# ColinWine/Multi-modal-Multi-label-Facial-Action-Unit-Detection-with-Transformer

Measured on AMD Instinct MI355X. Metric: clips/sec (fwd+bwd) on synthetic (B,T,d) AV sequences, higher is better.
Workload: dtype bf16; 1 GPU; BASELINE.json configs[1]: avformer transformer stack d=512 L=6 H=8x64 mlp=1024, T_v=196+T_a=128 tokens, B=32/GPU; global_batch=32, seq_len=324, parallelism=dp1, step=zero_grad+fwd+AULoss+bwd+adam, optimizer=FusedAdam, residual_stream=bf16

## Files before the change

include/avformer_hip.h:

```cpp
#ifndef AVFORMER_HIP_H
#define AVFORMER_HIP_H

#include <stddef.h>
#include <stdint.h>

#ifdef __cplusplus
extern "C" {
#endif

#define AVF_F32 0
#define AVF_BF16 1

#define AVF_EPI_NONE 0
#define AVF_EPI_BIAS_RES 1
#define AVF_EPI_BIAS_GELU 2
#define AVF_EPI_DGELU 3

typedef struct avf_layer_cfg {
  int32_t batch;
  int32_t tokens;
  int32_t dim;
  int32_t heads;
  int32_t dim_head;
  int32_t mlp_dim;
// ... 240 lines not shown

size_t avf_layer_saved_bytes(const avf_layer_cfg* cfg);
size_t avf_layer_lowp_bytes(const avf_layer_cfg* cfg);
size_t avf_layer_workspace_bytes(const avf_layer_cfg* cfg);
size_t avf_layer_grad_stream_bytes(const avf_layer_cfg* cfg);
int avf_layer_prepare_weights(const avf_layer_cfg* cfg, const avf_layer_params* p, void* lowp, void* stream);

int avf_layer_adam_step(const avf_layer_cfg* cfg, const avf_layer_params* p, const avf_layer_grads* g,
                        const avf_layer_grads* exp_avg, const avf_layer_grads* exp_avg_sq, void* lowp, float lr,
                        float beta1, float beta2, float eps, float weight_decay, const float* step, void* stream);

int avf_stack_adam_step(const avf_layer_cfg* cfg, int layers, const avf_layer_params* p, const avf_layer_grads* g,
                        const avf_layer_grads* exp_avg, const avf_layer_grads* exp_avg_sq, void* const* lowp, float lr,
                        float beta1, float beta2, float eps, float weight_decay, const float* step, void* stream);

int avf_adam_step_tensors(int count, float* const* p, const float* const* g, float* const* exp_avg,
                          float* const* exp_avg_sq, const int64_t* numel, float lr, float beta1, float beta2, float eps,
                          float weight_decay, const float* step, void* stream);

int avf_adam_batch_begin(void);
int avf_adam_batch_end(void);
int avf_adam_batch_abort(void);
int avf_selftest_adam_table(void* stream);

size_t avf_grad_control_workspace_bytes(int count, const int64_t* numel);
int avf_grad_control(int count, const float* const* g, const int64_t* numel, float max_norm, int n_warmup_steps,
                     const float* step, float* ctl, void* ws, void* stream);

int avf_adam_batch_control(const float* ctl);

int avf_layer_fwd(const avf_layer_cfg* cfg, const avf_layer_params* p, const void* lowp, const void* x_in,
                  void* x_out, void* saved, void* workspace, void* stream);

int avf_layer_fwd_embed_ok(const avf_layer_cfg* cfg);
int avf_layernorm_fwd_embed(const float* clip, const float* audio, const float* pos, int batch, int t_video, int t_audio,
                            void* x0_bf16, const float* gamma, const float* beta, void* y_bf16, float* mean, float* rstd, int dim,
                            float eps, void* stream);
int avf_layernorm_bwd_pos_ok(int batch, int tokens, int dim);
size_t avf_layernorm_bwd_pos_workspace_bytes(int batch, int tokens, int dim);
int avf_layernorm_bwd_pos(const void* dy_bf16, const void* x_bf16, const float* gamma, const float* mean, const float* rstd,
                          const void* dres_bf16, float* d_pos, float* dgamma, float* dbeta, void* workspace, int batch, int tokens,
                          int dim, void* stream);
int avf_layer_fwd_embed(const avf_layer_cfg* cfg, const avf_layer_params* p, const void* lowp, const float* clip,
                        const float* audio, const float* pos, int t_video, void* x0, void* x_out, void* saved, void* workspace,
                        void* stream);
int avf_layer_bwd_pos_ok(const avf_layer_cfg* cfg);
int avf_layer_bwd_pos(const avf_layer_cfg* cfg, const avf_layer_params* p, const void* lowp, const void* x_in,
                      const void* saved, const float* dx_out, const void* dx_out_lo, const float* dx_out_colsum, float* d_pos,
                      const avf_layer_grads* g, void* workspace, void* stream);
int avf_layer_bwd_dx_pos(const avf_layer_cfg* cfg, const avf_layer_params* p, const void* lowp, const void* x_in,
                         const void* saved, const float* dx_out, const void* dx_out_lo, const float* dx_out_colsum, float* d_pos,
                         const avf_layer_grads* g, void* workspace, void* dw_block, void* dw_desc, void* stream);

int avf_layer_bwd(const avf_layer_cfg* cfg, const avf_layer_params* p, const void* lowp, const void* x_in,
                  const void* saved, const float* dx_out, const void* dx_out_lo, const float* dx_out_colsum,
                  float* dx_in, void* dx_in_lo, float* dx_in_colsum, const avf_layer_grads* g, void* workspace,
                  void* stream);

int avf_layer_dw_defer_ok(const avf_layer_cfg* cfg, int* tiles_per_layer, int* slots);
int avf_layers_dw_max(void);
size_t avf_layer_dw_block_bytes(const avf_layer_cfg* cfg);
size_t avf_layer_dw_desc_bytes(void);
int avf_layer_bwd_dx(const avf_layer_cfg* cfg, const avf_layer_params* p, const void* lowp, const void* x_in,
                     const void* saved, const float* dx_out, const void* dx_out_lo, const float* dx_out_colsum,
                     float* dx_in, void* dx_in_lo, float* dx_in_colsum, const avf_layer_grads* g, void* workspace,
                     void* dw_block, void* dw_desc, void* stream);
size_t avf_layers_dw_workspace_bytes(const avf_layer_cfg* cfgs, int n_layers);
int avf_layers_dw(const avf_layer_cfg* cfgs, int n_layers, const void* const* descs, void* workspace, size_t workspace_bytes,
                  void* stream);

int avf_conv_pack_weight(const float* w, const float* gamma, const float* beta, const float* running_mean,
                         const float* running_var, double eps, void* w_packed, float* scale, float* shift, int Cout, int Cin,
                         int k, void* stream);
int avf_conv2d_nhwc(const void* x, int x_dtype, const void* w_packed, const float* scale, const float* shift,
                    const void* residual, int res_dtype, int relu, int k, int stride, void* out, int out_dtype, int N, int H,
                    int W, int Cin, int Cout, void* stream);
int avf_conv_plan(int N, int H, int W, int Cin, int Cout, int k, int stride, int* tile, int* tile_m, int* tile_n);
int avf_avgpool_nhwc(const void* x, int x_dtype, float* out, int64_t N, int HW, int C, void* stream);

int avf_dropout_factors(uint32_t seed_lo, uint32_t seed_hi, int layer_index, int site, float p, int64_t rows, int cols,
                        float* out, void* stream);

int avf_set_f32_arith(int mode);
int avf_get_f32_arith(void);

int avf_hip_error_reset(void* stream);

int avf_crash_line_arm(const char* line, int fd);
int avf_crash_line_disarm(void);

int avf_timing_enable(int on);
int avf_timing_read(int cls, double* total_ms, int64_t* launches, double* flops, double* bytes);

int avf_selftest_mfma_bf16(const void* a_bf16_16x32, const void* b_bf16_32x16, float* c_16x16, void* stream);
int avf_selftest_mfma_f32(const float* a_16x4, const float* b_4x16, float* c_16x16, void* stream);
int avf_selftest_tr16(const void* tile_bf16_32x16, void* out_bf16_64x8, void* stream);

#ifdef __cplusplus
}
#endif
#endif
```

multi-modal-multi-label-facial-action-unit-detection-with-transformer_amd/_build.py:

```python
from __future__ import annotations

import concurrent.futures
import os
import shutil
import subprocess

HERE = os.path.dirname(os.path.abspath(__file__))
CSRC = os.path.join(HERE, "csrc")
LIBDIR = os.path.join(HERE, "lib")
LIBNAME = "libavformer_hip.so"
SOURCES = ["api.hip", "norm_elem.hip", "layernorm.hip", "gemm_f32.hip", "attn_f32.hip", "attn_f32_mfma.hip", "attn_f32x3.hip", "gemm_bf16.hip", "gemm_ws.hip", "gemm_mx8.hip", "attn_bf16.hip", "attn_bwd_merged.hip", "layer.hip", "optim.hip", "grad_control.hip", "layer_small.hip", "heads.hip", "task_loss.hip", "eval_metrics.hip", "mel.hip", "clip.hip", "augment.hip", "clip_bank.hip", "mel_bank.hip", "conv.hip"]
HEADERS = [os.path.join(CSRC, "common.hpp"), os.path.join(CSRC, "gemm_nt.hpp"), os.path.join(CSRC, "gemm_dispatch.hpp"), os.path.join(CSRC, "attn_dispatch.hpp"), os.path.join(CSRC, "clip_source.hpp"),
           os.path.join(CSRC, "clip_kernels.hpp"), os.path.join(CSRC, "augment_kernels.hpp"), os.path.join(CSRC, "mel_kernels.hpp"), os.path.join(os.path.dirname(HERE), "include", "avformer_hip.h")]
FLAGS = ["--offload-arch=gfx950", "-O3", "-std=c++17", "-fPIC"]
EXTRA_FLAGS = {"gemm_f32.hip": ["-mllvm", "-amdgpu-mfma-vgpr-form"], "attn_f32_mfma.hip": ["-mllvm", "-amdgpu-mfma-vgpr-form"], "attn_f32x3.hip": ["-mllvm", "-amdgpu-mfma-vgpr-form"],
               "attn_bwd_merged.hip": ["-mllvm", "-amdgpu-mfma-vgpr-form", "-Xclang", "-target-feature", "-Xclang", "-packed-fp32-ops"],
               "augment.hip": ["-ffp-contract=off"],
               "clip_bank.hip": ["-ffp-contract=off"]}


def out_wt() -> int:
    v = os.environ.get("AVF_OUT_WT", "1").strip() or "1"
    if v not in ("0", "1"):
        raise RuntimeError(f"AVF_OUT_WT={v!r}: 0 or 1")
    return int(v)


def _variant() -> str:
    return "" if out_wt() == 1 else "_wt0"


def built_lib_path() -> str:
    return os.path.join(LIBDIR, LIBNAME.replace(".so", _variant() + ".so"))


def lib_path() -> str:
    return os.environ.get("AVF_LIB_PATH") or built_lib_path()


def _hipcc() -> str:
    for cand in (os.environ.get("HIPCC"), "/opt/rocm/bin/hipcc", shutil.which("hipcc")):
        if cand and os.path.exists(cand):
            return cand
    raise RuntimeError("hipcc not found (set HIPCC or install ROCm under /opt/rocm)")


def _stale(target: str, deps) -> bool:
    if not os.path.exists(target):
        return True
    t = os.path.getmtime(target)
    return any(os.path.getmtime(d) > t for d in deps)


def build(force: bool = False, verbose: bool = False) -> str:
    import fcntl
    os.makedirs(LIBDIR, exist_ok=True)
    with open(os.path.join(LIBDIR, ".build.lock"), "w") as lock:
        fcntl.flock(lock, fcntl.LOCK_EX)
        try:
            return _build_locked(force, verbose)
        finally:
            fcntl.flock(lock, fcntl.LOCK_UN)


# ... 40 lines not shown
```

multi-modal-multi-label-facial-action-unit-detection-with-transformer_amd/_lib.py:

```python
from __future__ import annotations

import ctypes as C
import os
import threading

from . import _build

F32, BF16 = 0, 1
EPI_NONE, EPI_BIAS_RES, EPI_BIAS_GELU, EPI_DGELU = 0, 1, 2, 3
CLIP_CTHW, CLIP_TCHW = 0, 1
WAVE_F32, WAVE_I16 = 0, 1

_vp = C.c_void_p
_i64 = C.c_int64
_int = C.c_int
_f = C.c_float
_sz = C.c_size_t


class LayerCfg(C.Structure):
    _fields_ = [("batch", C.c_int32), ("tokens", C.c_int32), ("dim", C.c_int32), ("heads", C.c_int32),
                ("dim_head", C.c_int32), ("mlp_dim", C.c_int32), ("dtype", C.c_int32), ("project_out", C.c_int32),
                ("ln_eps", C.c_float), ("dropout_p", C.c_float), ("seed_lo", C.c_uint32), ("seed_hi", C.c_uint32),
                ("layer_index", C.c_int32), ("seed_dev", C.c_void_p), ("grad_stream_bf16", C.c_int32), ("mx8_fwd", C.c_int32),
# ... 88 lines not shown
    "avf_au_loss_sum": (_int, [_vp, _i64, _vp, _i64, _vp, _f, _int, _int, _vp, _vp, _vp]),
    "avf_au_loss_wide": (_int, [_vp, _i64, _vp, _i64, _vp, _f, _int, _int, _int, _int, _vp, _vp, _vp]),
    "avf_sizeof_task_loss_cfg": (_sz, []),
    "avf_task_loss": (_int, [_vp, _i64, _vp, _vp, _i64, _vp, _i64, _vp, _int, _int, _vp, _vp, _vp, _vp]),
    "avf_task_loss_bwd": (_int, [_vp, _vp, _vp, _vp, _vp, _int, _int, _vp, _vp]),
    "avf_sizeof_eval_cfg": (_sz, []),
    "avf_eval_update": (_int, [_vp, _i64, _vp, _vp, _i64, _vp, _i64, _vp, _vp, _int, _vp, _vp, _vp, _vp, _vp]),
    "avf_eval_scores": (_int, [_vp, _vp, _vp, _vp]),
    "avf_mel_power": (_int, [_vp, _i64, _i64, _vp, _int, _int, _int, _vp, _vp, _vp, _int, _int, _int, _vp, _vp, _vp]),
    "avf_mel_db_norm": (_int, [_vp, _vp, _i64, _int, _i64, _int, C.c_double, C.c_double, C.c_double, _vp]),
    "avf_mel_power_bank": (_int, [_vp, _int, _i64, _vp, _vp, _i64, _vp, _vp, _i64, _vp, _i64, _i64, _i64, _vp, _int, _int, _int, _vp, _vp,
                                  _vp, _int, _int, _vp, _vp, _vp]),
    "avf_wave_gather": (_int, [_vp, _int, _i64, _vp, _vp, _i64, _vp, _vp, _i64, _vp, _i64, _i64, _i64, _i64, _vp, _vp]),
    "avf_clip_normalize": (_int, [_vp, _i64, _i64, _i64, _i64, _int, _int, _vp, _vp, _vp, _int, _int, _vp]),
    "avf_clip_denormalize": (_int, [_vp, _int, _int, _i64, _i64, _i64, _i64, _int, _vp, _vp, _vp, _vp]),
    "avf_clip_autoaugment": (_int, [_vp, _vp, _i64, _i64, _i64, _i64, _int, _vp, _vp]),
    "avf_clip_autoaugment_max_pixels": (_i64, []),
    "avf_clip_autoaugment_normalize": (_int, [_vp, _i64, _i64, _i64, _i64, _int, _vp, _int, _vp, _vp, _vp, _int, _int, _vp]),
    "avf_clip_gather": (_int, [_vp, _vp, _vp, _vp, _i64, _i64, _i64, _i64, _i64, _i64, _int, _vp, _vp]),
    "avf_clip_gather_normalize": (_int, [_vp, _vp, _vp, _vp, _i64, _i64, _i64, _i64, _i64, _i64, _int, _int, _vp, _vp, _vp, _int, _int,
                                         _vp]),
    "avf_clip_gather_autoaugment": (_int, [_vp, _vp, _vp, _vp, _i64, _i64, _i64, _i64, _i64, _i64, _int, _vp, _vp, _vp]),
    "avf_clip_gather_autoaugment_normalize": (_int, [_vp, _vp, _vp, _vp, _i64, _i64, _i64, _i64, _i64, _i64, _int, _vp, _int, _vp, _vp,
                                                     _vp, _int, _int, _vp]),
    "avf_conv_pack_weight": (_int, [_vp, _vp, _vp, _vp, _vp, C.c_double, _vp, _vp, _vp, _int, _int, _int, _vp]),
    "avf_conv2d_nhwc": (_int, [_vp, _int, _vp, _vp, _vp, _vp, _int, _int, _int, _int, _vp, _int, _int, _int, _int, _int, _int, _vp]),
    "avf_conv_plan": (_int, [_int, _int, _int, _int, _int, _int, _int, C.POINTER(C.c_int), C.POINTER(C.c_int), C.POINTER(C.c_int)]),
    "avf_avgpool_nhwc": (_int, [_vp, _int, _vp, _i64, _int, _int, _vp]),
    "avf_layer_saved_bytes": (_sz, [C.POINTER(LayerCfg)]),
    "avf_layer_lowp_bytes": (_sz, [C.POINTER(LayerCfg)]),
    "avf_layernorm_bwd_mx8": (_int, [_vp, _vp, _vp, _vp, _vp, _vp, _vp, _vp, _vp, _vp, _vp, _vp, _vp, _i64, _int, _vp]),
    "avf_attn_fwd_mx8": (_int, [_vp, _vp, _vp, _vp, _vp, _int, _int, _int, _int, _vp]),
    "avf_attn_bwd_emits_mx8": (_int, [_int, _int]),
    "avf_attn_bwd_mx8": (_int, [_vp, _vp, _vp, _vp, _vp, _vp, _vp, _int, _int, _int, _int, _vp]),
    "avf_attn_fwd_masked": (_int, [_int, _vp, _vp, _vp, _vp, _int, _int, _int, _int, _vp]),
    "avf_attn_bwd_masked": (_int, [_int, _vp, _vp, _vp, _vp, _vp, _vp, _vp, _int, _int, _int, _int, _vp]),
    "avf_layer_workspace_bytes": (_sz, [C.POINTER(LayerCfg)]),
    "avf_layer_grad_stream_bytes": (_sz, [C.POINTER(LayerCfg)]),
    "avf_layer_prepare_weights": (_int, [C.POINTER(LayerCfg), C.POINTER(LayerPtrs), _vp, _vp]),
    "avf_layer_fwd": (_int, [C.POINTER(LayerCfg), C.POINTER(LayerPtrs), _vp, _vp, _vp, _vp, _vp, _vp]),
    "avf_layer_bwd": (_int, [C.POINTER(LayerCfg), C.POINTER(LayerPtrs), _vp, _vp, _vp, _vp, _vp, _vp, _vp, _vp, _vp,
                             C.POINTER(LayerPtrs), _vp, _vp]),
    "avf_layernorm_fwd_embed": (_int, [_vp, _vp, _vp, _int, _int, _int, _vp, _vp, _vp, _vp, _vp, _vp, _int, _f, _vp]),
    "avf_layernorm_bwd_pos_ok": (_int, [_int, _int, _int]),
    "avf_layernorm_bwd_pos_workspace_bytes": (_sz, [_int, _int, _int]),
    "avf_layernorm_bwd_pos": (_int, [_vp, _vp, _vp, _vp, _vp, _vp, _vp, _vp, _vp, _vp, _int, _int, _int, _vp]),
    "avf_layer_fwd_embed_ok": (_int, [C.POINTER(LayerCfg)]),
    "avf_layer_fwd_embed": (_int, [C.POINTER(LayerCfg), C.POINTER(LayerPtrs), _vp, _vp, _vp, _vp, _int, _vp, _vp, _vp, _vp, _vp]),
    "avf_layer_bwd_pos_ok": (_int, [C.POINTER(LayerCfg)]),
    "avf_layer_bwd_pos": (_int, [C.POINTER(LayerCfg), C.POINTER(LayerPtrs), _vp, _vp, _vp, _vp, _vp, _vp, _vp,
                                 C.POINTER(LayerPtrs), _vp, _vp]),
    "avf_layer_bwd_dx_pos": (_int, [C.POINTER(LayerCfg), C.POINTER(LayerPtrs), _vp, _vp, _vp, _vp, _vp, _vp, _vp,
                                    C.POINTER(LayerPtrs), _vp, _vp, _vp, _vp]),
    "avf_layer_dw_defer_ok": (_int, [C.POINTER(LayerCfg), C.POINTER(C.c_int), C.POINTER(C.c_int)]),
    "avf_layers_dw_max": (_int, []),
    "avf_layer_dw_block_bytes": (_sz, [C.POINTER(LayerCfg)]),
    "avf_layer_dw_desc_bytes": (_sz, []),
    "avf_layer_bwd_dx": (_int, [C.POINTER(LayerCfg), C.POINTER(LayerPtrs), _vp, _vp, _vp, _vp, _vp, _vp, _vp, _vp, _vp,
                                C.POINTER(LayerPtrs), _vp, _vp, _vp, _vp]),
    "avf_layers_dw_workspace_bytes": (_sz, [C.POINTER(LayerCfg), _int]),
    "avf_layers_dw": (_int, [C.POINTER(LayerCfg), _int, _vp, _vp, _sz, _vp]),
    "avf_layer_adam_step": (_int, [C.POINTER(LayerCfg), C.POINTER(LayerPtrs), C.POINTER(LayerPtrs), C.POINTER(LayerPtrs),
                                   C.POINTER(LayerPtrs), _vp, _f, _f, _f, _f, _f, _vp, _vp]),
    "avf_stack_adam_step": (_int, [C.POINTER(LayerCfg), _int, C.POINTER(LayerPtrs), C.POINTER(LayerPtrs), C.POINTER(LayerPtrs),
                                   C.POINTER(LayerPtrs), _vp, _f, _f, _f, _f, _f, _vp, _vp]),
    "avf_adam_step_tensors": (_int, [_int, _vp, _vp, _vp, _vp, _vp, _f, _f, _f, _f, _f, _vp, _vp]),
    "avf_adam_batch_begin": (_int, []),
    "avf_adam_batch_end": (_int, []),
    "avf_adam_batch_abort": (_int, []),
    "avf_selftest_adam_table": (_int, [_vp]),
    "avf_grad_control_workspace_bytes": (_sz, [_int, _vp]),
    "avf_grad_control": (_int, [_int, _vp, _vp, _f, _int, _vp, _vp, _vp, _vp]),
    "avf_adam_batch_control": (_int, [_vp]),
    "avf_dropout_factors": (_int, [C.c_uint32, C.c_uint32, _int, _int, _f, _i64, _int, _vp, _vp]),
    "avf_timing_enable": (_int, [_int]),
    "avf_timing_read": (_int, [_int, C.POINTER(C.c_double), C.POINTER(C.c_int64), C.POINTER(C.c_double),
                               C.POINTER(C.c_double)]),
    "avf_hip_error_reset": (_int, [_vp]),
    "avf_crash_line_arm": (_int, [C.c_char_p, _int]),
    "avf_crash_line_disarm": (_int, []),
    "avf_set_f32_arith": (_int, [_int]),
    "avf_get_f32_arith": (_int, []),
    "avf_selftest_mfma_bf16": (_int, [_vp, _vp, _vp, _vp]),
    "avf_selftest_mfma_f32": (_int, [_vp, _vp, _vp, _vp]),
    "avf_selftest_tr16": (_int, [_vp, _vp, _vp]),
}

_lock = threading.Lock()
_lib = None


class HipLibraryError(RuntimeError):
    pass


def load(build_if_missing: bool = True):
    global _lib
    if _lib is not None:
        return _lib
    with _lock:
        if _lib is not None:
            return _lib
        path = _build.lib_path()
        if not os.path.exists(path):
            err = None
            if build_if_missing:
# ... 68 lines not shown
```

multi-modal-multi-label-facial-action-unit-detection-with-transformer_amd/csrc/api.hip:

```cpp
#include <stdarg.h>

#include "common.hpp"

namespace avf {

static thread_local char g_err[512] = "";

void set_error(const char* fmt, ...) {
  va_list ap;
  va_start(ap, fmt);
  vsnprintf(g_err, sizeof(g_err), fmt, ap);
  va_end(ap);
}

int check_launch(const char* what) {
  hipError_t e = hipGetLastError();
  if (e != hipSuccess) {
    set_error("%s: %s", what, hipGetErrorString(e));
    return 2;
  }
  return 0;
}

namespace {
// ... 141 lines not shown
  return 1;
}

extern "C" int avf_layernorm_fwd(const float* x, const float* gamma, const float* beta, void* y, int y_dtype,
                                 float* mean, float* rstd, int64_t rows, int dim, float eps, void* stream) {
  AVF_REQUIRE(x && gamma && beta && y && mean && rstd, "layernorm_fwd: null pointer");
  return layernorm_fwd(x, gamma, beta, y, y_dtype, mean, rstd, rows, dim, eps, (hipStream_t)stream);
}
extern "C" size_t avf_layernorm_bwd_workspace_bytes(int64_t rows, int dim) { return layernorm_bwd_ws(rows, dim); }
extern "C" int avf_layernorm_bwd(const void* dy, int dy_dtype, const float* x, const float* gamma, const float* mean,
                                 const float* rstd, const float* dres, float* dx, void* dx_lo, float* dgamma,
                                 float* dbeta, float* dcolsum, void* workspace, int64_t rows, int dim, void* stream) {
  AVF_REQUIRE(dy && x && gamma && mean && rstd && dx && dgamma && dbeta && workspace, "layernorm_bwd: null pointer");
  return layernorm_bwd(dy, dy_dtype, x, gamma, mean, rstd, dres, dx, dx_lo, dgamma, dbeta, dcolsum, workspace, rows,
                       dim, (hipStream_t)stream);
}
extern "C" int avf_layernorm_fwd_ex(const void* x, int x_dtype, const float* gamma, const float* beta, void* y, int y_dtype,
                                    float* mean, float* rstd, int64_t rows, int dim, float eps, void* stream) {
  AVF_REQUIRE(x && gamma && beta && y && mean && rstd, "layernorm_fwd_ex: null pointer");
  AVF_REQUIRE(x_dtype == AVF_F32 || x_dtype == AVF_BF16, "layernorm_fwd_ex: bad x_dtype %d", x_dtype);
  return layernorm_fwd(x, gamma, beta, y, y_dtype, mean, rstd, rows, dim, eps, (hipStream_t)stream, nullptr, nullptr, x_dtype);
}
extern "C" int avf_layernorm_bwd_ex(const void* dy, int dy_dtype, const void* x, int x_dtype, const float* gamma,
                                    const float* mean, const float* rstd, const void* dres, int dres_dtype, float* dx,
                                    void* dx_lo, void* dx_m, float* dgamma, float* dbeta, float* dcolsum, void* workspace,
                                    int64_t rows, int dim, uint32_t seed_lo, uint32_t seed_hi, int layer_index, int site,
                                    float p, void* stream) {
  AVF_REQUIRE(dy && x && gamma && mean && rstd && dgamma && dbeta && workspace, "layernorm_bwd_ex: null pointer");
  AVF_REQUIRE((x_dtype == AVF_F32 || x_dtype == AVF_BF16) && (dres_dtype == AVF_F32 || dres_dtype == AVF_BF16),
              "layernorm_bwd_ex: bad x_dtype %d / dres_dtype %d", x_dtype, dres_dtype);
  AVF_REQUIRE(p >= 0.f && p < 1.f && (p == 0.f || (site >= 0 && site < 3)), "layernorm_bwd_ex: bad dropout site %d / p %g", site,
              (double)p);
  const DropCfg d = p > 0.f ? make_drop(p, ((uint64_t)seed_hi << 32) | seed_lo, layer_index, site) : kNoDrop;
  return layernorm_bwd(dy, dy_dtype, x, gamma, mean, rstd, dres, dx, dx_lo, dgamma, dbeta, dcolsum, workspace, rows, dim,
                       (hipStream_t)stream, d, nullptr, dres ? dres_dtype : AVF_F32, x_dtype, nullptr, nullptr, dx_m);
}
extern "C" int avf_layernorm_fwd_embed(const float* clip, const float* audio, const float* pos, int batch, int t_video, int t_audio,
                                       void* x0_bf16, const float* gamma, const float* beta, void* y_bf16, float* mean, float* rstd,
                                       int dim, float eps, void* stream) {
  AVF_REQUIRE(gamma && beta, "layernorm_fwd_embed: null pointer");
  return layernorm_fwd_embed(clip, audio, pos, batch, t_video, t_audio, x0_bf16, gamma, beta, y_bf16, mean, rstd, dim, eps,
                             (hipStream_t)stream);
}
extern "C" int avf_layernorm_bwd_pos_ok(int batch, int tokens, int dim) { return layernorm_bwd_tok_ok(batch, tokens, dim) ? 1 : 0; }
extern "C" size_t avf_layernorm_bwd_pos_workspace_bytes(int batch, int tokens, int dim) {
  return layernorm_bwd_ws((int64_t)batch * tokens, dim, tokens);
}
extern "C" int avf_layernorm_bwd_pos(const void* dy_bf16, const void* x_bf16, const float* gamma, const float* mean, const float* rstd,
                                     const void* dres_bf16, float* d_pos, float* dgamma, float* dbeta, void* workspace, int batch,
                                     int tokens, int dim, void* stream) {
  AVF_REQUIRE(dgamma && dbeta, "layernorm_bwd_pos: null pointer");
  return layernorm_bwd_tok(dy_bf16, x_bf16, gamma, mean, rstd, dres_bf16, d_pos, dgamma, dbeta, workspace, batch, tokens, dim,
                           (hipStream_t)stream);
}
extern "C" size_t avf_colsum_workspace_bytes(int64_t rows, int cols) { return colsum_ws(rows, cols); }
extern "C" int avf_colsum(const void* in, int in_dtype, int64_t rows, int cols, int64_t ld, float* out,
                          void* workspace, void* stream) {
  return colsum(in, in_dtype, rows, cols, ld, out, workspace, (hipStream_t)stream);
}
extern "C" int avf_cast_f32_to_bf16(const float* in, void* out, int64_t n, void* stream) {
  AVF_REQUIRE(in && out, "cast: null pointer");
  return cast_f32_to_bf16(in, out, n, (hipStream_t)stream);
}
extern "C" int avf_dropout_factors(uint32_t seed_lo, uint32_t seed_hi, int layer_index, int site, float p, int64_t rows,
                                   int cols, float* out, void* stream) {
  AVF_REQUIRE(out && rows > 0 && cols > 0 && cols % 4 == 0 && p > 0.f && p < 1.f && site >= 0 && site < 3,
              "dropout_factors: bad arguments");
  const DropCfg d = make_drop(p, ((uint64_t)seed_hi << 32) | seed_lo, layer_index, site);
  return dropout_factors(d, out, rows * cols, (hipStream_t)stream);
}
extern "C" int avf_prep_weight_bf16(const float* w, void* w_lo, void* w_t_lo, int rows, int cols, void* stream) {
  AVF_REQUIRE(w, "prep_weight: null pointer");
  return prep_weight_bf16(w, w_lo, w_t_lo, rows, cols, (hipStream_t)stream);
}

extern "C" size_t avf_gemm_workspace_bytes(int dtype, int transA, int transB, int64_t M, int64_t N, int64_t K) {
  return gemm_ws(dtype, transA, transB, M, N, K);
}
extern "C" int avf_gemm(int dtype, int transA, int transB, int64_t M, int64_t N, int64_t K, const void* A, int64_t lda,
                        const void* B, int64_t ldb, void* C, int64_t ldc, int c_dtype, int epilogue, const float* bias,
                        const float* residual, int64_t ldres, void* aux, int64_t ldaux, void* workspace, void* stream) {
  AVF_REQUIRE(A && B && C, "gemm: null pointer");
  GemmArgs a;
  a.dtype = dtype; a.transA = transA; a.transB = transB;
  a.M = M; a.N = N; a.K = K;
  a.A = A; a.lda = lda; a.B = B; a.ldb = ldb; a.C = C; a.ldc = ldc;
  a.c_dtype = c_dtype; a.epilogue = epilogue; a.bias = bias; a.residual = residual; a.ldres = ldres;
  a.aux = aux; a.ldaux = ldaux; a.workspace = workspace; a.colsum = nullptr; a.drop = kNoDrop; a.defer_fold = nullptr;
  return gemm(a, (hipStream_t)stream);
}

extern "C" int avf_pack_weight_ws_ok(int64_t rows, int64_t cols) { return pack_ws_ok(rows, cols) ? 1 : 0; }
extern "C" size_t avf_pack_weight_ws_bytes(int64_t rows, int64_t cols) { return pack_ws_ok(rows, cols) ? pack_ws_bytes(rows, cols) : 0; }
extern "C" size_t avf_gemm_nt_ws_workspace_bytes(int64_t M, int64_t N) { return gemm_nt_colsum_ws(M, N); }
extern "C" int avf_gemm_nt_ws_dispatch(int64_t M, int64_t N, int64_t K, int epilogue, int c_dtype) {
  GemmArgs a;
  a.dtype = AVF_BF16; a.transA = 0; a.transB = 1;
  a.M = M; a.N = N; a.K = K;
  void* aligned = (void*)(uintptr_t)256;
  a.A = aligned; a.lda = K; a.B = nullptr; a.ldb = K; a.C = aligned; a.ldc = N;
  a.c_dtype = c_dtype; a.epilogue = epilogue; a.bias = (epilogue == AVF_EPI_BIAS_RES || epilogue == AVF_EPI_BIAS_GELU) ? (const float*)aligned : nullptr;
  a.residual = epilogue == AVF_EPI_BIAS_RES ? aligned : nullptr; a.ldres = N;
  a.aux = (epilogue == AVF_EPI_BIAS_GELU || epilogue == AVF_EPI_DGELU) ? aligned : nullptr; a.ldaux = N;
  a.workspace = nullptr; a.colsum = nullptr; a.drop = kNoDrop; a.defer_fold = nullptr;
  a.Bp = aligned; a.ws_force = 0; a.mx_q = nullptr; a.mx_s = nullptr;
  return gemm_bf16_nt_ws_preferred(a) ? 1 : 0;
// ... 280 lines not shown
```

multi-modal-multi-label-facial-action-unit-detection-with-transformer_amd/csrc/common.hpp:

```cpp
#pragma once
#include <hip/hip_runtime.h>
#include <hip/hip_ext.h>
#include <stdint.h>
#include <stdio.h>
#include <stdlib.h>
#include <string.h>

#include <type_traits>

#include "../../include/avformer_hip.h"

namespace avf {

void set_error(const char* fmt, ...);
int check_launch(const char* what);
bool shape_log_on();
void shape_log(const char* fmt, ...);
inline const char* tuning_env(const char* name) {
  static const bool on = [] {
    const char* t = getenv("AVF_TUNING");
    return t && *t && atoi(t) != 0;
  }();
  return on ? getenv(name) : nullptr;
}
// ... 267 lines not shown
  d.scale = 1.0f / (1.0f - (float)d.thresh16 / 65536.0f);
  d.site_const = 0xD1B54A32D192ED03ULL * (uint64_t)(layer * 4 + site + 1);
  d.key = mix64(seed + d.site_const);
  d.seed_dev = seed_dev;
  return d;
}
static const DropCfg kNoDrop = {0, nullptr, 0, 0, 1.0f};
__device__ __forceinline__ uint64_t drop_key(const DropCfg& d) {
  return d.seed_dev ? mix64(*d.seed_dev + d.site_const) : d.key;
}
__device__ __forceinline__ float4 drop_factor4(const DropCfg& d, uint64_t key, uint64_t idx) {
  const uint64_t h = mix64(key + idx * 0x9E3779B97F4A7C15ULL);
  float4 f;
  f.x = ((uint32_t)(h) & 0xffffu) >= d.thresh16 ? d.scale : 0.f;
  f.y = ((uint32_t)(h >> 16) & 0xffffu) >= d.thresh16 ? d.scale : 0.f;
  f.z = ((uint32_t)(h >> 32) & 0xffffu) >= d.thresh16 ? d.scale : 0.f;
  f.w = ((uint32_t)(h >> 48) & 0xffffu) >= d.thresh16 ? d.scale : 0.f;
  return f;
}

__device__ __forceinline__ float drop_factor1(const DropCfg& d, uint64_t key, uint64_t idx) {
  const uint64_t h = mix64(key + (idx & ~3ULL) * 0x9E3779B97F4A7C15ULL);
  return ((uint32_t)(h >> (16 * (idx & 3))) & 0xffffu) >= d.thresh16 ? d.scale : 0.f;
}

static inline size_t align_up(size_t v, size_t a) { return (v + a - 1) / a * a; }

struct PerDeviceOnce {
  uint64_t done = 0;
  bool need() const {
    int dev = 0;
    (void)hipGetDevice(&dev);
    return ((__atomic_load_n(&done, __ATOMIC_ACQUIRE) >> (dev & 63)) & 1u) == 0;
  }
  void mark() {
    int dev = 0;
    (void)hipGetDevice(&dev);
    __atomic_fetch_or(&done, 1ull << (dev & 63), __ATOMIC_RELEASE);
  }
};

struct FoldJob;
int layernorm_fwd(const void* x, const float* gamma, const float* beta, void* y, int y_dtype, float* mean,
                  float* rstd, int64_t rows, int dim, float eps, hipStream_t s, void* mx_q = nullptr, void* mx_s = nullptr,
                  int x_dtype = AVF_F32);
size_t layernorm_bwd_ws(int64_t rows, int dim, int tokens = 0);
bool layernorm_fwd_embed_ok(int dim);
int layernorm_fwd_embed(const float* clip, const float* audio, const float* pos, int batch, int t_video, int t_audio, void* x0,
                        const float* gamma, const float* beta, void* y, float* mean, float* rstd, int dim, float eps, hipStream_t s);
bool layernorm_bwd_tok_ok(int batch, int tokens, int dim);
int layernorm_bwd_tok(const void* dy, const void* x, const float* gamma, const float* mean, const float* rstd, const void* dres,
                      float* dpos, float* dgamma, float* dbeta, void* ws, int batch, int tokens, int dim, hipStream_t s,
                      FoldJob* defer_fold = nullptr);
int layernorm_bwd(const void* dy, int dy_dtype, const void* x, const float* gamma, const float* mean,
                  const float* rstd, const void* dres, float* dx, void* dx_lo, float* dgamma, float* dbeta,
                  float* dcolsum, void* ws, int64_t rows, int dim, hipStream_t s, const DropCfg& drop = kNoDrop,
                  FoldJob* defer_fold = nullptr, int dres_dtype = AVF_F32, int x_dtype = AVF_F32, void* mx_q = nullptr,
                  void* mx_s = nullptr, void* dx_m = nullptr);
size_t colsum_ws(int64_t rows, int cols);
int colsum(const void* in, int in_dtype, int64_t rows, int cols, int64_t ld, float* out, void* ws, hipStream_t s);
int cast_f32_to_bf16(const float* in, void* out, int64_t n, hipStream_t s, const DropCfg& drop = kNoDrop);
int mask_copy_f32(const float* in, float* out, int64_t n, hipStream_t s, const DropCfg& drop);
int dropout_factors(const DropCfg& drop, float* out, int64_t n, hipStream_t s);
int fold_partials(const float* partial, int nb, int width, float* out, hipStream_t s);
struct FoldJob;
int fold_job(const FoldJob& job, hipStream_t s);

struct FoldJob {
  const float* partial;
  int nb, width, seg;
  float *o0, *o1, *o2;
};
constexpr int kFoldMax = 12;
struct FoldList {
  FoldJob job[kFoldMax];
  int count;
};
int fold_list(const FoldList& fl, hipStream_t s);
constexpr int FOLD_COLS = 16, FOLD_RG = 64;
__device__ __forceinline__ void fold_columns_vec(const FoldJob& j, int colgroup, float4 (*red)[FOLD_COLS / 4]) {
  const int cq = threadIdx.x & (FOLD_COLS / 4 - 1), grp = threadIdx.x / (FOLD_COLS / 4);
  const int col = colgroup * FOLD_COLS + cq * 4;
  float4 a[8];
#pragma unroll
  for (int u = 0; u < 8; ++u) a[u] = make_float4(0.f, 0.f, 0.f, 0.f);
  if (col < j.width) {
    int b = grp;
    for (; b + 7 * FOLD_RG < j.nb; b += 8 * FOLD_RG) {
      float4 t[8];
#pragma unroll
      for (int u = 0; u < 8; ++u) t[u] = *reinterpret_cast<const float4*>(j.partial + (int64_t)(b + FOLD_RG * u) * j.width + col);
#pragma unroll
      for (int u = 0; u < 8; ++u) { a[u].x += t[u].x; a[u].y += t[u].y; a[u].z += t[u].z; a[u].w += t[u].w; }
    }
    for (; b < j.nb; b += FOLD_RG) {
      const float4 t = *reinterpret_cast<const float4*>(j.partial + (int64_t)b * j.width + col);
      a[0].x += t.x; a[0].y += t.y; a[0].z += t.z; a[0].w += t.w;
    }
  }
  red[grp][cq] = make_float4(((a[0].x + a[1].x) + (a[2].x + a[3].x)) + ((a[4].x + a[5].x) + (a[6].x + a[7].x)),
                             ((a[0].y + a[1].y) + (a[2].y + a[3].y)) + ((a[4].y + a[5].y) + (a[6].y + a[7].y)),
                             ((a[0].z + a[1].z) + (a[2].z + a[3].z)) + ((a[4].z + a[5].z) + (a[6].z + a[7].z)),
                             ((a[0].w + a[1].w) + (a[2].w + a[3].w)) + ((a[4].w + a[5].w) + (a[6].w + a[7].w)));
  __syncthreads();
  if (threadIdx.x < FOLD_COLS) {
    const int q = threadIdx.x >> 2, comp = threadIdx.x & 3;
// ... 158 lines not shown
```

multi-modal-multi-label-facial-action-unit-detection-with-transformer_amd/csrc/layer.hip:

```cpp
#include <mutex>
#include <vector>

#include "common.hpp"

namespace avf {

namespace {

struct Dims {
  int64_t R;
  int D, H, dh, I, M, B, N;
  int dt;
  size_t es;
  float p;
  uint64_t seed;
  const uint64_t* seed_dev;
  int layer;
  bool gs16;
  bool gsd;
  bool mx;
  bool rs16;
  int xdt;
  float p0;
  const void* keep;
// ... 101 lines not shown
  }
  Carver c(base);
  LowP t;
  t.wqkv = c.take((size_t)3 * d.I * d.D * 2);
  t.wqkv_t = c.take((size_t)3 * d.I * d.D * 2);
  t.wo = c.take((size_t)d.D * d.I * 2);
  t.wo_t = c.take((size_t)d.D * d.I * 2);
  t.w1 = c.take((size_t)d.M * d.D * 2);
  t.w1_t = c.take((size_t)d.M * d.D * 2);
  t.w2 = c.take((size_t)d.D * d.M * 2);
  t.w2_t = c.take((size_t)d.D * d.M * 2);
  if (d.mx) {
    t.wqkv_q = c.take((size_t)3 * d.I * d.D); t.wqkv_s = c.take((size_t)3 * d.I * d.D / 32);
    t.w1_q = c.take((size_t)d.M * d.D);       t.w1_s = c.take((size_t)d.M * d.D / 32);
    t.w2_q = c.take((size_t)d.D * d.M);       t.w2_s = c.take((size_t)d.D * d.M / 32);
    t.wo_q = c.take((size_t)d.D * d.I);       t.wo_s = c.take((size_t)d.D * d.I / 32);
    t.w2t_q = c.take((size_t)d.D * d.M);      t.w2t_s = c.take((size_t)d.D * d.M / 32);
    t.w1t_q = c.take((size_t)d.D * d.M);      t.w1t_s = c.take((size_t)d.D * d.M / 32);
    t.wot_q = c.take((size_t)d.D * d.I);      t.wot_s = c.take((size_t)d.D * d.I / 32);
    t.wqkvt_q = c.take((size_t)3 * d.I * d.D); t.wqkvt_s = c.take((size_t)3 * d.I * d.D / 32);
  } else {
    t.wqkv_q = t.wqkv_s = t.w1_q = t.w1_s = t.w2_q = t.w2_s = nullptr;
    t.wo_q = t.wo_s = t.w2t_q = t.w2t_s = t.w1t_q = t.w1t_s = t.wot_q = t.wot_s = nullptr;
    t.wqkvt_q = t.wqkvt_s = nullptr;
  }
  t.ws.wqkv_p = pack_ws_ok(3 * d.I, d.D) ? c.take(pack_ws_bytes(3 * d.I, d.D)) : nullptr;
  t.ws.wo_p = pack_ws_ok(d.D, d.I) ? c.take(pack_ws_bytes(d.D, d.I)) : nullptr;
  t.ws.w1_p = pack_ws_ok(d.M, d.D) ? c.take(pack_ws_bytes(d.M, d.D)) : nullptr;
  t.ws.w2t_p = pack_ws_ok(d.M, d.D) ? c.take(pack_ws_bytes(d.M, d.D)) : nullptr;
  t.ws.wot_p = pack_ws_ok(d.I, d.D) ? c.take(pack_ws_bytes(d.I, d.D)) : nullptr;
  if (!base) t.ws = LowpWs{nullptr, nullptr, nullptr, nullptr, nullptr};
  if (l) *l = t;
  return c.off;
}

TnGroupArgs dw_group(const Dims& d, const void* gy, const void* g_act, const void* du, const void* h2, const void* gm,
                     const void* o, const void* dqkv, const void* h1, const avf_layer_grads* g) {
  TnGroupArgs a;
  memset(&a, 0, sizeof(a));
  a.count = 4;
  a.K = d.R;
  a.A[0] = dqkv; a.B[0] = h1; a.C[0] = g ? g->w_qkv : nullptr; a.M[0] = 3 * d.I; a.N[0] = d.D;
  a.A[1] = gm;   a.B[1] = o;  a.C[1] = g ? g->w_out : nullptr; a.M[1] = d.D;     a.N[1] = d.I;
  a.A[2] = du;   a.B[2] = h2; a.C[2] = g ? g->w1 : nullptr;    a.M[2] = d.M;     a.N[2] = d.D;
  a.A[3] = gy;   a.B[3] = g_act; a.C[3] = g ? g->w2 : nullptr; a.M[3] = d.D;     a.N[3] = d.M;
  for (int i = 0; i < 4; ++i) { a.lda[i] = a.M[i]; a.ldb[i] = a.N[i]; }
  return a;
}

size_t work_colsum_bytes(const Dims& d) {
  const int maxc = d.M > d.D ? d.M : d.D;
  size_t csb = colsum_ws(d.R, maxc);
  if (d.dt == AVF_BF16 && gemm_nt_colsum_ws(d.R, d.M) > csb) csb = gemm_nt_colsum_ws(d.R, d.M);
  return csb;
}

struct Work {
  void *du, *dh, *d_o, *dqkv, *dx_mid_lo, *dx_out_lo, *ln_ws, *ln_ws1, *cs_ws, *gemm_ws;
  float *dx_mid, *delta;
  void *hq, *hs, *gq, *gs;
  void *oq, *os;
  void *duq, *dus, *mq, *ms, *gyq, *gys;
  void *dqq, *dqs;
  void *dx_out_s, *dx_mid_m;
  float *gy_m, *gm_m;
  float* small_part;
};
size_t carve_work(const Dims& d, void* base, Work* w) {
  Carver c(base);
  Work t;
  t.du = c.take(d.R * d.M * d.es);
  t.dh = c.take(d.R * d.D * d.es);
  t.d_o = c.take(d.R * d.I * d.es);
  t.dqkv = c.take(d.R * 3 * d.I * d.es);
  t.dx_mid = (float*)c.take(d.R * d.D * 4);
  t.dx_mid_lo = c.take(d.dt == AVF_BF16 ? d.R * d.D * 2 : 0);
  t.dx_out_lo = c.take(d.dt == AVF_BF16 ? d.R * d.D * 2 : 0);
  t.delta = (float*)c.take((size_t)d.B * d.H * d.N * 4 * 2);
  t.ln_ws = c.take(layernorm_bwd_ws(d.R, d.D));
  t.ln_ws1 = c.take(layernorm_bwd_ws(d.R, d.D, d.N));
  t.cs_ws = c.take(work_colsum_bytes(d));
  size_t g = 0;
  if (d.dt == AVF_BF16) {
    size_t a = gemm_bf16_tn_ws(3 * d.I, d.D, d.R), b = gemm_bf16_tn_ws(d.D, d.I, d.R);
    size_t e = gemm_bf16_tn_ws(d.M, d.D, d.R), f = gemm_bf16_tn_ws(d.D, d.M, d.R);
    g = a > b ? a : b;
    g = g > e ? g : e;
    g = g > f ? g : f;
    TnGroupArgs ga = dw_group(d, nullptr, nullptr, nullptr, nullptr, nullptr, nullptr, nullptr, nullptr, nullptr);
    const size_t gg = gemm_bf16_tn_group_ws(ga);
    g = g > gg ? g : gg;
  } else {
    const size_t a = gemm_f32_ws(3 * d.I, d.D, d.R), b = gemm_f32_ws(d.D, d.I, d.R);
    const size_t e = gemm_f32_ws(d.M, d.D, d.R), f = gemm_f32_ws(d.D, d.M, d.R);
    g = a > b ? a : b;
    g = g > e ? g : e;
    g = g > f ? g : f;
    TnGroupArgs ga = dw_group(d, nullptr, nullptr, nullptr, nullptr, nullptr, nullptr, nullptr, nullptr, nullptr);
    const size_t gg = gemm_f32x3_tn_group_ws(ga);
    g = g > gg ? g : gg;
  }
  t.gemm_ws = c.take(g);
  t.small_part = (float*)c.take(small_layer_ok(d.dt, d.N, d.D, d.H, d.dh, d.M) ? small_bwd_partial_floats(d.B, d.D, d.M) * 4 : 0);
  if (d.mx) {
    t.hq = c.take(d.R * d.D); t.hs = c.take(d.R * d.D / 32);
    t.gq = c.take(d.R * d.M); t.gs = c.take(d.R * d.M / 32);
    t.oq = c.take(d.R * d.I); t.os = c.take(d.R * d.I / 32);
  } else {
    t.hq = t.hs = t.gq = t.gs = t.oq = t.os = nullptr;
  }
  if (d.mxb) {
    t.duq = c.take(d.R * d.M); t.dus = c.take(d.R * d.M / 32);
    t.mq = c.take(d.R * d.D);  t.ms = c.take(d.R * d.D / 32);
    t.gyq = c.take(d.R * d.D); t.gys = c.take(d.R * d.D / 32);
    t.dqq = c.take(d.R * 3 * d.I); t.dqs = c.take(d.R * 3 * d.I / 32);
  } else {
    t.duq = t.dus = t.mq = t.ms = t.gyq = t.gys = nullptr;
    t.dqq = t.dqs = nullptr;
  }
  t.dx_out_s = c.take(d.gsd ? d.R * d.D * 2 : 0);
  t.dx_mid_m = c.take(d.gsd ? d.R * d.D * 2 : 0);
  const bool f32_drop = d.dt == AVF_F32 && d.p > 0.f;
  t.gy_m = (float*)c.take(f32_drop ? d.R * d.D * 4 : 0);
  t.gm_m = (float*)c.take(f32_drop ? d.R * d.D * 4 : 0);
  if (w) *w = t;
  return c.off;
}

size_t carve_dw_block(const Dims& d, void* base, Work* w) {
  Carver c(base);
  void* du = c.take(d.R * d.M * 2);
  void* dqkv = c.take(d.R * 3 * d.I * 2);
  void* dx_mid_lo = c.take(d.R * d.D * 2);
  void* dx_out_lo = c.take(d.R * d.D * 2);
  void* ln_ws = c.take(layernorm_bwd_ws(d.R, d.D));
  void* ln_ws1 = c.take(layernorm_bwd_ws(d.R, d.D, d.N));
  void* cs_ws = c.take(work_colsum_bytes(d));
  if (w) {
    w->du = du; w->dqkv = dqkv; w->dx_mid_lo = dx_mid_lo; w->dx_out_lo = dx_out_lo;
    w->ln_ws = ln_ws; w->ln_ws1 = ln_ws1; w->cs_ws = cs_ws;
  }
  return c.off;
}
constexpr uint32_t kDwDescMagic = 0x64574431u;
struct DwDeferred {
  uint32_t magic;
  TnGroupArgs grp;
  FoldJob folds[3];
};
bool dw_defer_mode_ok(const Dims& d) {
  return d.dt == AVF_BF16 && !d.gsd && d.p == 0.f && !d.mx && !d.mxb && !d.keep && !small_layer_ok(d.dt, d.N, d.D, d.H, d.dh, d.M);
}

int linear_fwd(const Dims& d, const void* A, int in, const void* W, int out, void* C, int c_dtype, int epi,
               const float* bias, const void* res, void* aux, hipStream_t s, const DropCfg& drop = kNoDrop,
               const void* Wp = nullptr) {
  GemmArgs a;
  a.dtype = d.dt; a.transA = 0; a.transB = 1;
  a.M = d.R; a.N = out; a.K = in;
  a.A = A; a.lda = in; a.B = W; a.ldb = in;
  a.C = C; a.ldc = out; a.c_dtype = c_dtype; a.epilogue = epi;
  a.bias = bias; a.residual = res; a.ldres = out; a.aux = aux; a.ldaux = out; a.workspace = nullptr; a.colsum = nullptr;
  a.drop = drop; a.defer_fold = nullptr;
  a.Bp = Wp;
  return gemm(a, s);
}

int linear_fwd_mx(const Dims& d, const void* Aq, const void* As, int in, const void* Wq, const void* Ws, int out, void* C,
                  int c_dtype, int epi, const float* bias, const void* res, void* aux, hipStream_t s, const DropCfg& drop,
                  void* mx_q = nullptr, void* mx_s = nullptr) {
  GemmArgs a;
  a.dtype = AVF_BF16; a.transA = 0; a.transB = 1;
  a.M = d.R; a.N = out; a.K = in;
  a.A = Aq; a.lda = in; a.B = Wq; a.ldb = in;
  a.C = C; a.ldc = out; a.c_dtype = c_dtype; a.epilogue = epi;
  a.bias = bias; a.residual = res; a.ldres = out; a.aux = aux; a.ldaux = out; a.workspace = nullptr; a.colsum = nullptr;
  a.drop = drop; a.defer_fold = nullptr;
// ... 98 lines not shown
  AVF_TRY(make_dims(cfg, &d));
  if (d.dt != AVF_BF16) return 0;
  AVF_REQUIRE(p && lowp, "prepare_weights: null pointer");
  hipStream_t s = (hipStream_t)stream;
  LowP l;
  carve_lowp(d, lowp, &l);
  PrepBatch b;
  b.d[0] = PrepDesc{p->w_qkv, (bf16*)l.wqkv, (bf16*)l.wqkv_t, 3 * d.I, d.D, attn_q_prescale(d.dh), d.I, l.ws.wqkv_p, nullptr};
  b.d[1] = PrepDesc{p->w_out, (bf16*)l.wo, (bf16*)l.wo_t, d.D, d.I, 1.0f, 0, l.ws.wo_p, l.ws.wot_p};
  b.d[2] = PrepDesc{p->w1, (bf16*)l.w1, (bf16*)l.w1_t, d.M, d.D, 1.0f, 0, l.ws.w1_p, nullptr};
  b.d[3] = PrepDesc{p->w2, (bf16*)l.w2, (bf16*)l.w2_t, d.D, d.M, 1.0f, 0, nullptr, l.ws.w2t_p};
  AVF_TRY(prep_weights_multi(b, 4, s));
  return 0;
}

extern "C" int avf_stack_quant_weights_mx8(const avf_layer_cfg* cfg, int layers, void* const* lowp, void* stream) {
  Dims d;
  AVF_TRY(make_dims(cfg, &d));
  AVF_REQUIRE(d.mx, "stack_quant_weights_mx8: cfg.mx8_fwd is not set");
  AVF_REQUIRE(layers > 0 && layers <= 64 && lowp, "stack_quant_weights_mx8: bad arguments");
  MxQuantJob jobs[64 * 8];
  int n = 0;
  for (int i = 0; i < layers; ++i) {
    AVF_REQUIRE(lowp[i], "stack_quant_weights_mx8: null image buffer (layer %d)", i);
    LowP l;
    carve_lowp(d, lowp[i], &l);
    jobs[n++] = MxQuantJob{l.wqkv, l.wqkv_q, l.wqkv_s, 3 * d.I, d.D};
    jobs[n++] = MxQuantJob{l.w1, l.w1_q, l.w1_s, d.M, d.D};
    jobs[n++] = MxQuantJob{l.w2, l.w2_q, l.w2_s, d.D, d.M};
    if (d.I % 128 == 0) jobs[n++] = MxQuantJob{l.wo, l.wo_q, l.wo_s, d.D, d.I};
    if (d.mxb) {
      jobs[n++] = MxQuantJob{l.w2_t, l.w2t_q, l.w2t_s, d.M, d.D};
      jobs[n++] = MxQuantJob{l.w1_t, l.w1t_q, l.w1t_s, d.D, d.M};
      jobs[n++] = MxQuantJob{l.wo_t, l.wot_q, l.wot_s, d.I, d.D};
      if ((3 * d.I) % 128 == 0) jobs[n++] = MxQuantJob{l.wqkv_t, l.wqkvt_q, l.wqkvt_s, d.D, 3 * d.I};
    }
  }
  return quant_mx8_multi(jobs, n, (hipStream_t)stream);
}

static bool stack_ends_mode_ok(const Dims& d) {
  return d.dt == AVF_BF16 && d.rs16 && d.gs16 && !d.gsd && d.p == 0.f && !d.mx && !d.mxb &&
         !d.keep && d.D % 8 == 0 && d.D <= 1536;
}
extern "C" int avf_layer_fwd_embed_ok(const avf_layer_cfg* cfg) {
  Dims d;
  return !make_dims(cfg, &d) && stack_ends_mode_ok(d) && layernorm_fwd_embed_ok(d.D);
}
extern "C" int avf_layer_bwd_pos_ok(const avf_layer_cfg* cfg) {
  Dims d;
  return !make_dims(cfg, &d) && stack_ends_mode_ok(d) && layernorm_bwd_tok_ok(d.B, d.N, d.D);
}

struct EmbedSrc {
  const float *clip, *audio, *pos;
  int t_video;
  void* x0;
};
static int layer_fwd_impl(const avf_layer_cfg* cfg, const avf_layer_params* p, const void* lowp, const void* x_in, void* x_out,
                          void* saved, void* workspace, void* stream, const EmbedSrc* emb) {
  Dims d;
  AVF_TRY(make_dims(cfg, &d));
  if (emb) {
    AVF_REQUIRE(stack_ends_mode_ok(d) && layernorm_fwd_embed_ok(d.D) && emb->x0 && emb->t_video > 0 && emb->t_video < d.N,
                "layer_fwd_embed: needs the all-bf16 streams without dropout, fp8 or mask, and both token groups (ask "
                "avf_layer_fwd_embed_ok first)");
    x_in = emb->x0;
  }
  AVF_REQUIRE(p && x_in && x_out && saved, "layer_fwd: null pointer");
  AVF_REQUIRE(d.dt == AVF_F32 || lowp, "layer_fwd(bf16): lowp weights missing");
  hipStream_t s = (hipStream_t)stream;
  Saved sv;
  carve_saved(d, saved, &sv);
  LowP l;
  carve_lowp(d, (void*)lowp, &l);
  const bool lo = d.dt == AVF_BF16;
  const void* wqkv = lo ? l.wqkv : (const void*)p->w_qkv;
  const void* wo = lo ? l.wo : (const void*)p->w_out;
  const void* w1 = lo ? l.w1 : (const void*)p->w1;
  const void* w2 = lo ? l.w2 : (const void*)p->w2;

  if (d.mx) {
    AVF_REQUIRE(workspace, "layer_fwd(mx8): workspace missing");
    Work w;
    carve_work(d, workspace, &w);
    const DropCfg dr0 = make_drop(d.p0, d.seed, d.layer, 0, d.seed_dev), dr1 = make_drop(d.p, d.seed, d.layer, 1, d.seed_dev),
                  dr2 = make_drop(d.p, d.seed, d.layer, 2, d.seed_dev);
    AVF_TRY(layernorm_fwd(x_in, p->ln1_w, p->ln1_b, sv.h1, d.dt, sv.mean1, sv.rstd1, d.R, d.D, cfg->ln_eps, s, w.hq, w.hs, d.xdt));
    AVF_TRY(linear_fwd_mx(d, w.hq, w.hs, d.D, l.wqkv_q, l.wqkv_s, 3 * d.I, sv.qkv, d.dt, AVF_EPI_NONE, nullptr, nullptr,
                          nullptr, s, kNoDrop));
    static const int o_mx_on = tuning_int("AVF_MX8_OUTPROJ", 1);
    const bool o_mx = o_mx_on && !d.keep && attn_fwd_emits_mx8(d.N, d.dh) && d.I % 128 == 0;
    if (d.keep)
      AVF_TRY(attn_fwd_vec(AVF_BF16, sv.qkv, sv.o, sv.lse2, d.B, d.N, d.H, d.dh, s, d.keep, attn_q_prescale_on()));
    else
      AVF_TRY(attn_fwd_bf16((const bf16*)sv.qkv, (bf16*)sv.o, sv.lse2, d.B, d.N, d.H, d.dh, s, attn_q_prescale_on(),
                            o_mx ? w.oq : nullptr, o_mx ? w.os : nullptr));
    if (o_mx)
      AVF_TRY(linear_fwd_mx(d, w.oq, w.os, d.I, l.wo_q, l.wo_s, d.D, sv.x_mid, d.xdt, AVF_EPI_BIAS_RES, p->b_out, x_in, nullptr,
                            s, dr0));
    else
      AVF_TRY(linear_fwd(d, sv.o, d.I, wo, d.D, sv.x_mid, d.xdt, AVF_EPI_BIAS_RES, p->b_out, x_in, nullptr, s, dr0, l.ws.wo_p));
    AVF_TRY(layernorm_fwd(sv.x_mid, p->ln2_w, p->ln2_b, sv.h2, d.dt, sv.mean2, sv.rstd2, d.R, d.D, cfg->ln_eps, s, w.hq, w.hs, d.xdt));
    AVF_TRY(linear_fwd_mx(d, w.hq, w.hs, d.D, l.w1_q, l.w1_s, d.M, sv.g, d.dt, AVF_EPI_BIAS_GELU, p->b1, nullptr, sv.u, s, dr1,
                          w.gq, w.gs));
    AVF_TRY(linear_fwd_mx(d, w.gq, w.gs, d.M, l.w2_q, l.w2_s, d.D, x_out, d.xdt, AVF_EPI_BIAS_RES, p->b2, sv.x_mid, nullptr,
                          s, dr2));
    return 0;
  }
  if (!d.rs16 && !d.keep && small_layer_ok(d.dt, d.N, d.D, d.H, d.dh, d.M)) {
    const float sc = attn_q_prescale_on() ? 1.0f : 1.4426950408889634f / sqrtf((float)d.dh);
    return layer_fwd_small(d.B, d.N, d.D, d.H, d.M, cfg->ln_eps, sc, p, wqkv, wo, w1, w2, (const float*)x_in, (float*)x_out, sv.h1,
                           sv.mean1, sv.rstd1, sv.qkv, sv.o, sv.lse2, (float*)sv.x_mid, sv.h2, sv.mean2, sv.rstd2, sv.u, sv.g,
                           make_drop(d.p0, d.seed, d.layer, 0, d.seed_dev), make_drop(d.p, d.seed, d.layer, 1, d.seed_dev),
                           make_drop(d.p, d.seed, d.layer, 2, d.seed_dev), s);
  }
  if (emb)
    AVF_TRY(layernorm_fwd_embed(emb->clip, emb->audio, emb->pos, d.B, emb->t_video, d.N - emb->t_video, emb->x0, p->ln1_w, p->ln1_b,
                                sv.h1, sv.mean1, sv.rstd1, d.D, cfg->ln_eps, s));
  else
    AVF_TRY(layernorm_fwd(x_in, p->ln1_w, p->ln1_b, sv.h1, d.dt, sv.mean1, sv.rstd1, d.R, d.D, cfg->ln_eps, s, nullptr, nullptr, d.xdt));
  AVF_TRY(linear_fwd(d, sv.h1, d.D, wqkv, 3 * d.I, sv.qkv, d.dt, AVF_EPI_NONE, nullptr, nullptr, nullptr, s, kNoDrop, l.ws.wqkv_p));
  if (d.keep && lo) AVF_TRY(attn_fwd_masked_bf16(sv.qkv, sv.o, sv.lse2, d.keep, d.B, d.N, d.H, d.dh, s, attn_q_prescale_on()));
  else if (d.keep) AVF_TRY(attn_fwd_vec(d.dt, sv.qkv, sv.o, sv.lse2, d.B, d.N, d.H, d.dh, s, d.keep, false));
  else if (lo) AVF_TRY(attn_fwd_bf16((const bf16*)sv.qkv, (bf16*)sv.o, sv.lse2, d.B, d.N, d.H, d.dh, s, attn_q_prescale_on()));
  else AVF_TRY(attn_fwd_f32((const float*)sv.qkv, (float*)sv.o, sv.lse2, d.B, d.N, d.H, d.dh, s));
  const DropCfg dr0 = make_drop(d.p0, d.seed, d.layer, 0, d.seed_dev), dr1 = make_drop(d.p, d.seed, d.layer, 1, d.seed_dev),
                dr2 = make_drop(d.p, d.seed, d.layer, 2, d.seed_dev);
  AVF_TRY(linear_fwd(d, sv.o, d.I, wo, d.D, sv.x_mid, d.xdt, AVF_EPI_BIAS_RES, p->b_out, x_in, nullptr, s, dr0, l.ws.wo_p));
  AVF_TRY(layernorm_fwd(sv.x_mid, p->ln2_w, p->ln2_b, sv.h2, d.dt, sv.mean2, sv.rstd2, d.R, d.D, cfg->ln_eps, s, nullptr, nullptr, d.xdt));
  AVF_TRY(linear_fwd(d, sv.h2, d.D, w1, d.M, sv.g, d.dt, AVF_EPI_BIAS_GELU, p->b1, nullptr, sv.u, s, dr1, l.ws.w1_p));
  AVF_TRY(linear_fwd(d, sv.g, d.M, w2, d.D, x_out, d.xdt, AVF_EPI_BIAS_RES, p->b2, sv.x_mid, nullptr, s, dr2));
  return 0;
}

extern "C" int avf_layer_fwd(const avf_layer_cfg* cfg, const avf_layer_params* p, const void* lowp, const void* x_in,
                             void* x_out, void* saved, void* workspace, void* stream) {
  return layer_fwd_impl(cfg, p, lowp, x_in, x_out, saved, workspace, stream, nullptr);
}

extern "C" int avf_layer_fwd_embed(const avf_layer_cfg* cfg, const avf_layer_params* p, const void* lowp, const float* clip,
                                   const float* audio, const float* pos, int t_video, void* x0, void* x_out, void* saved,
                                   void* workspace, void* stream) {
  const EmbedSrc emb{clip, audio, pos, t_video, x0};
  return layer_fwd_impl(cfg, p, lowp, nullptr, x_out, saved, workspace, stream, &emb);
}

static int layer_bwd_impl(const avf_layer_cfg* cfg, const avf_layer_params* p, const void* lowp, const void* x_in,
                          const void* saved, const float* dx_out, const void* dx_out_lo,
                          const float* dx_out_colsum, float* dx_in, void* dx_in_lo, float* dx_in_colsum,
                          const avf_layer_grads* g, void* workspace, void* stream, void* dw_block, DwDeferred* dw_desc,
                          float* d_pos = nullptr) {
  Dims d;
  AVF_TRY(make_dims(cfg, &d));
  AVF_REQUIRE(!d_pos || (stack_ends_mode_ok(d) && layernorm_bwd_tok_ok(d.B, d.N, d.D) && !dx_in && !dx_in_lo && !dx_in_colsum),
              "layer_bwd_pos: needs the all-bf16 streams without dropout, fp8 or mask, a batch within the token-major rule (ask "
              "avf_layer_bwd_pos_ok first) and no dx_in outputs");
  AVF_REQUIRE(!dw_desc || (dw_block && dw_defer_mode_ok(d) && ((uintptr_t)dw_block & 255) == 0),
              "layer_bwd_dx: this mode keeps its weight gradients in the layer (ask avf_layer_dw_defer_ok first), or the "
              "operand block is missing / not 256-byte aligned");
  AVF_REQUIRE(p && x_in && saved && g && workspace, "layer_bwd: null pointer");
  AVF_REQUIRE(d.gs16 ? (dx_out || dx_out_lo) && (dx_in || dx_in_lo || d_pos) : (dx_out && dx_in), "layer_bwd: null gradient pointer");
  AVF_REQUIRE(!d.gs16 || dx_in_lo || d_pos, "layer_bwd(grad_stream_bf16): dx_in_lo missing");
  AVF_REQUIRE(d.dt == AVF_F32 || lowp, "layer_bwd(bf16): lowp weights missing");
  hipStream_t s = (hipStream_t)stream;
  Saved sv;
  carve_saved(d, (void*)saved, &sv);
  LowP l;
  carve_lowp(d, (void*)lowp, &l);
  const bool lo = d.dt == AVF_BF16;
  Work w;
  carve_work(d, workspace, &w);
  if (dw_desc) carve_dw_block(d, dw_block, &w);

  const DropCfg dr0 = make_drop(d.p0, d.seed, d.layer, 0, d.seed_dev), dr1 = make_drop(d.p, d.seed, d.layer, 1, d.seed_dev),
                dr2 = make_drop(d.p, d.seed, d.layer, 2, d.seed_dev);
  const DropCfg dr_prev2 = d.layer > 0 ? make_drop(d.p, d.seed, d.layer - 1, 2, d.seed_dev) : kNoDrop;
  static const int small_bwd_on = tuning_int("AVF_LAYER_SMALL_BWD", 1);
  const bool small_bwd = lo && !d.rs16 && !d.mx && !d.keep && small_bwd_on && small_layer_ok(d.dt, d.N, d.D, d.H, d.dh, d.M);
  const void* gy = dx_out;
  const void* gy_stream = nullptr;
  bool own_copy = false;
  if (lo) {
    if (dx_out_lo && d.gsd) {
      gy_stream = dx_out_lo;
      gy = (const char*)dx_out_lo + grad_q_off(d.R, d.D);
    } else if (dx_out_lo) gy = dx_out_lo;
    else if (small_bwd) gy = w.dx_out_lo;
    else {
      AVF_TRY(cast_f32_to_bf16(dx_out, w.dx_out_lo, d.R * d.D, s, dr2));
      gy = w.dx_out_lo;
      own_copy = true;
      if (d.gsd) {
        AVF_TRY(cast_f32_to_bf16(dx_out, w.dx_out_s, d.R * d.D, s, kNoDrop));
        gy_stream = w.dx_out_s;
      }
    }
  }
  AVF_REQUIRE(!d.gsd || !small_bwd, "layer_bwd: grad_stream_bf16 with dropout on a short-sequence layer (internal error)");
  const bool gm_masked = d.gsd && d.p0 > 0.f;
  const bool f32_drop = !lo && d.p > 0.f;
  if (f32_drop) {
    AVF_TRY(mask_copy_f32(dx_out, w.gy_m, d.R * d.D, s, dr2));
    gy = w.gy_m;
    own_copy = true;
  }
  const bool f32_drop0 = f32_drop && d.p0 > 0.f;
  const void* gm = lo ? (gm_masked ? (const void*)w.dx_mid_m : (const void*)w.dx_mid_lo)
                      : (f32_drop0 ? (const void*)w.gm_m : (const void*)w.dx_mid);
  TnGroupArgs grp = dw_group(d, gy, sv.g, w.du, sv.h2, gm, sv.o, w.dqkv, sv.h1, g);
  grp.workspace = w.gemm_ws;
  const bool grouped32 = !lo && !small_bwd && gemm_f32x3_tn_group_ok(grp);
  const bool grouped = lo && gemm_bf16_tn_group_ok(grp);
  FoldList folds;
  memset(&folds, 0, sizeof(folds));
  folds.count = 3;
  AVF_REQUIRE(!dw_desc || (grouped && !small_bwd), "layer_bwd_dx: the layer's weight gradients do not form a grouped launch "
              "(rows %% 64, widths %% 8, 16-byte aligned operands)");

  if (small_bwd) {
    float* pb1 = w.small_part;
    float* pln2 = pb1 + (size_t)d.B * d.M;
    float* pln1 = pln2 + (size_t)d.B * 3 * d.D;
    SmallBwdAHost ha;
    ha.dx_out = dx_out; ha.dx_out_lo = dx_out_lo; ha.gy_store = dx_out_lo ? nullptr : w.dx_out_lo; ha.x_mid = (const float*)sv.x_mid;
    ha.u = sv.u; ha.ln2_w = p->ln2_w; ha.mean2 = sv.mean2; ha.rstd2 = sv.rstd2;
    ha.w2_t = l.w2_t; ha.w1_t = l.w1_t; ha.wo_t = l.wo_t; ha.du = w.du; ha.dx_mid = d.gs16 ? nullptr : w.dx_mid;
    ha.dx_mid_lo = w.dx_mid_lo; ha.d_o = w.d_o; ha.pb1 = pb1; ha.pln2 = pln2; ha.gs16 = d.gs16 ? 1 : 0;
    ha.dr0 = dr0; ha.dr1 = dr1; ha.dr2 = dr2;
    AVF_TRY(layer_bwd_small_a(d.B, d.N, d.D, d.I, d.M, ha, s));
    if (dx_out_colsum && dx_out_colsum != g->b2)
      AVF_REQUIRE(hipMemcpyAsync(g->b2, dx_out_colsum, (size_t)d.D * 4, hipMemcpyDeviceToDevice, s) == hipSuccess,
                  "layer_bwd: memcpy failed");
    else if (!dx_out_colsum) {
      if (d.p > 0.f || !dx_out) AVF_TRY(colsum(gy, AVF_BF16, d.R, d.D, d.D, g->b2, w.cs_ws, s));
      else AVF_TRY(colsum(dx_out, AVF_F32, d.R, d.D, d.D, g->b2, w.cs_ws, s));
    }
    static const int small_att_on = tuning_int("AVF_LAYER_SMALL_ATT", 1);
    const bool fuse_att = small_att_on && d.H <= 16;
    if (!fuse_att)
      AVF_TRY(attn_bwd_bf16((const bf16*)sv.qkv, (const bf16*)sv.o, (const bf16*)w.d_o, sv.lse2, (bf16*)w.dqkv, w.delta,
                            d.B, d.N, d.H, d.dh, s, attn_q_prescale_on(), w.delta + (size_t)d.B * d.H * d.N));
    SmallBwdBHost hb;
    hb.attention = fuse_att ? 1 : 0;
    hb.qkv = sv.qkv; hb.o = sv.o; hb.d_o = w.d_o; hb.lse2 = sv.lse2; hb.H = d.H;
    {
      const float scale = 1.0f / sqrtf((float)d.dh), log2e = 1.4426950408889634f;
      hb.score_scale = attn_q_prescale_on() ? 1.0f : log2e * scale;
      hb.dq_scale = scale;
      hb.dk_scale = attn_q_prescale_on() ? 1.0f / log2e : scale;
    }
    hb.dqkv = w.dqkv; hb.wqkv_t = l.wqkv_t; hb.x_in = (const float*)x_in; hb.ln1_w = p->ln1_w; hb.mean1 = sv.mean1; hb.rstd1 = sv.rstd1;
    hb.dx_mid = d.gs16 ? nullptr : w.dx_mid; hb.dx_mid_lo = w.dx_mid_lo; hb.dx_in = dx_in; hb.dx_in_lo = dx_in_lo; hb.pln1 = pln1;
    hb.gs16 = d.gs16 ? 1 : 0; hb.dr_prev2 = dr_prev2;
    AVF_TRY(layer_bwd_small_b(d.B, d.N, d.D, d.I, hb, s));
    folds.job[0] = FoldJob{pb1, d.B, d.M, d.M, g->b1, nullptr, nullptr};
    folds.job[1] = FoldJob{pln2, d.B, 3 * d.D, d.D, g->ln2_w, g->ln2_b, g->b_out};
    folds.job[2] = FoldJob{pln1, d.B, 3 * d.D, d.D, g->ln1_w, g->ln1_b, dx_in_colsum};
    if (grouped) return gemm_bf16_tn_group(grp, s, &folds);
    AVF_TRY(linear_dw(d, gy, d.D, sv.g, d.M, g->w2, w.gemm_ws, s));
    AVF_TRY(linear_dw(d, w.du, d.M, sv.h2, d.D, g->w1, w.gemm_ws, s));
    AVF_TRY(linear_dw(d, gm, d.D, sv.o, d.I, g->w_out, w.gemm_ws, s));
    AVF_TRY(linear_dw(d, w.dqkv, 3 * d.I, sv.h1, d.D, g->w_qkv, w.gemm_ws, s));
    for (int j = 0; j < 3; ++j) AVF_TRY(fold_job(folds.job[j], s));
    return 0;
  }

  if (dx_out_colsum && dx_out_colsum != g->b2)
    AVF_REQUIRE(hipMemcpyAsync(g->b2, dx_out_colsum, (size_t)d.D * 4, hipMemcpyDeviceToDevice, s) == hipSuccess,
                "layer_bwd: memcpy failed");
  else if (!dx_out_colsum) {
    if (d.p > 0.f) {
      AVF_REQUIRE(own_copy, "layer_bwd: with dropout pass dx_out_colsum together with dx_out_lo");
      AVF_TRY(colsum(gy, d.dt, d.R, d.D, d.D, g->b2, w.cs_ws, s));
    } else if (dx_out) {
      AVF_TRY(colsum(dx_out, AVF_F32, d.R, d.D, d.D, g->b2, w.cs_ws, s));
    } else {
      AVF_TRY(colsum(gy, AVF_BF16, d.R, d.D, d.D, g->b2, w.cs_ws, s));
    }
  }
  if (!grouped && !grouped32) AVF_TRY(linear_dw(d, gy, d.D, sv.g, d.M, g->w2, w.gemm_ws, s));
  const void *gyq = nullptr, *gys = nullptr;
  void *inq = nullptr, *ins = nullptr;
  if (d.mxb) {
    if (d.gy_mx && dx_out_lo) {
      gyq = (const char*)dx_out_lo + grad_q_off(d.R, d.D);
      gys = (const char*)dx_out_lo + grad_s_off(d.R, d.D);
    } else {
      AVF_TRY(quant_mx8(gy, AVF_BF16, d.D, d.R, d.D, w.gyq, d.D, w.gys, s));
      gyq = w.gyq; gys = w.gys;
    }
    if (dx_in_lo) {
      inq = (char*)dx_in_lo + grad_q_off(d.R, d.D);
      ins = (char*)dx_in_lo + grad_s_off(d.R, d.D);
    }
  }
  if (d.mxb) {
    GemmArgs a;
    a.dtype = AVF_BF16; a.transA = 0; a.transB = 1;
    a.M = d.R; a.N = d.M; a.K = d.D;
    a.A = gy; a.lda = d.D; a.B = l.w2_t; a.ldb = d.D;
    a.C = w.du; a.ldc = d.M; a.c_dtype = AVF_BF16; a.epilogue = AVF_EPI_DGELU;
    a.bias = nullptr; a.residual = nullptr; a.ldres = 0; a.aux = (void*)sv.u; a.ldaux = d.M; a.workspace = w.cs_ws; a.colsum = g->b1;
    a.drop = dr1; a.defer_fold = grouped ? &folds.job[0] : nullptr;
    a.Bp = l.ws.w2t_p; a.mx_q = w.duq; a.mx_s = w.dus;
    static const int dgelu_ws = tuning_int("AVF_MX8_DGELU_WS", 1);
    if (dgelu_ws && gemm_bf16_nt_ws_ok(a)) AVF_TRY(gemm(a, s));
    else
      AVF_TRY(linear_dx_mx(d, gyq, gys, d.D, l.w2t_q, l.w2t_s, d.M, w.du, AVF_EPI_DGELU, sv.u, s, g->b1, w.cs_ws, dr1,
                           grouped ? &folds.job[0] : nullptr, w.duq, w.dus));
  } else if (lo) {
    AVF_TRY(linear_dx(d, gy, d.D, p->w2, l.w2_t, d.M, w.du, AVF_EPI_DGELU, sv.u, s, g->b1, w.cs_ws, dr1,
                      grouped ? &folds.job[0] : nullptr, l.ws.w2t_p));
  } else {
    AVF_TRY(linear_dx(d, gy, d.D, p->w2, l.w2_t, d.M, w.du, AVF_EPI_DGELU, sv.u, s, nullptr, nullptr, dr1));
    AVF_TRY(colsum(w.du, d.dt, d.R, d.M, d.M, g->b1, w.cs_ws, s));
  }
  if (d.mxb)
    AVF_TRY(linear_dx_mx(d, w.duq, w.dus, d.M, l.w1t_q, l.w1t_s, d.D, w.dh, AVF_EPI_NONE, nullptr, s, nullptr, nullptr, kNoDrop,
                         nullptr));
  else
    AVF_TRY(linear_dx(d, w.du, d.M, p->w1, l.w1_t, d.D, w.dh, AVF_EPI_NONE, nullptr, s));
  if (d.gs16)
    AVF_TRY(layernorm_bwd(w.dh, d.dt, sv.x_mid, p->ln2_w, sv.mean2, sv.rstd2, d.gsd ? gy_stream : gy, nullptr, w.dx_mid_lo,
                          g->ln2_w, g->ln2_b, g->b_out, w.ln_ws, d.R, d.D, s, dr0, grouped ? &folds.job[1] : nullptr, AVF_BF16,
                          d.xdt, w.mq, w.ms, gm_masked ? w.dx_mid_m : nullptr));
  else
    AVF_TRY(layernorm_bwd(w.dh, d.dt, sv.x_mid, p->ln2_w, sv.mean2, sv.rstd2, dx_out, w.dx_mid,
                          lo ? w.dx_mid_lo : nullptr, g->ln2_w, g->ln2_b, g->b_out, w.ln_ws, d.R, d.D, s, dr0,
                          (grouped || grouped32) ? &folds.job[1] : nullptr, AVF_F32, d.xdt, w.mq, w.ms));
  if (!grouped && !grouped32) AVF_TRY(linear_dw(d, w.du, d.M, sv.h2, d.D, g->w1, w.gemm_ws, s));
  if (f32_drop0) AVF_TRY(mask_copy_f32(w.dx_mid, w.gm_m, d.R * d.D, s, dr0));
  if (!grouped && !grouped32) AVF_TRY(linear_dw(d, gm, d.D, sv.o, d.I, g->w_out, w.gemm_ws, s));
  if (d.mxb)
    AVF_TRY(linear_dx_mx(d, w.mq, w.ms, d.D, l.wot_q, l.wot_s, d.I, w.d_o, AVF_EPI_NONE, nullptr, s, nullptr, nullptr, kNoDrop,
                         nullptr));
  else
    AVF_TRY(linear_dx(d, gm, d.D, p->w_out, l.wo_t, d.I, w.d_o, AVF_EPI_NONE, nullptr, s, nullptr, nullptr, kNoDrop, nullptr,
                      l.ws.wot_p));
  const int dq_mx_on = tuning_int("AVF_MX8_DQKV", 0);
  const bool dq_mx = d.mxb && dq_mx_on && !d.keep && (3 * d.I) % 128 == 0 && d.D % 128 == 0 &&
                     attn_bwd_emits_mx8(d.N, d.dh, attn_q_prescale_on());
  if (d.keep && lo && !d.mx)
    AVF_TRY(attn_bwd_masked_bf16(sv.qkv, sv.o, w.d_o, sv.lse2, w.dqkv, w.delta, w.delta + (size_t)d.B * d.H * d.N, d.keep, d.B,
                                 d.N, d.H, d.dh, s, attn_q_prescale_on()));
  else if (d.keep)
    AVF_TRY(attn_bwd_vec(d.dt, sv.qkv, sv.o, w.d_o, sv.lse2, w.dqkv, w.delta, d.B, d.N, d.H, d.dh, s, d.keep,
                         lo && attn_q_prescale_on()));
  else if (lo)
    AVF_TRY(attn_bwd_bf16((const bf16*)sv.qkv, (const bf16*)sv.o, (const bf16*)w.d_o, sv.lse2, (bf16*)w.dqkv, w.delta,
                          d.B, d.N, d.H, d.dh, s, attn_q_prescale_on(), w.delta + (size_t)d.B * d.H * d.N, nullptr,
                          dq_mx ? w.dqq : nullptr, dq_mx ? w.dqs : nullptr));
  else
    AVF_TRY(attn_bwd_f32((const float*)sv.qkv, (const float*)sv.o, (const float*)w.d_o, sv.lse2, (float*)w.dqkv,
                         w.delta, d.B, d.N, d.H, d.dh, s));
  if (grouped32) AVF_TRY(gemm_f32x3_tn_group(grp, s));
  if (dq_mx)
    AVF_TRY(linear_dx_mx(d, w.dqq, w.dqs, 3 * d.I, l.wqkvt_q, l.wqkvt_s, d.D, w.dh, AVF_EPI_NONE, nullptr, s, nullptr, nullptr,
                         kNoDrop, nullptr));
  else
    AVF_TRY(linear_dx(d, w.dqkv, 3 * d.I, p->w_qkv, l.wqkv_t, d.D, w.dh, AVF_EPI_NONE, nullptr, s));
  if (d_pos)
    AVF_TRY(layernorm_bwd_tok(w.dh, x_in, p->ln1_w, sv.mean1, sv.rstd1, w.dx_mid_lo, d_pos, g->ln1_w, g->ln1_b, w.ln_ws1, d.B, d.N,
                              d.D, s, grouped ? &folds.job[2] : nullptr));
  else if (d.gs16)
    AVF_TRY(layernorm_bwd(w.dh, d.dt, x_in, p->ln1_w, sv.mean1, sv.rstd1, w.dx_mid_lo, dx_in, dx_in_lo, g->ln1_w, g->ln1_b,
                          dx_in_colsum, w.ln_ws1, d.R, d.D, s, dr_prev2, grouped ? &folds.job[2] : nullptr, AVF_BF16, d.xdt,
                          inq, ins, (d.gsd && dr_prev2.thresh16) ? (char*)dx_in_lo + grad_q_off(d.R, d.D) : nullptr));
  else
    AVF_TRY(layernorm_bwd(w.dh, d.dt, x_in, p->ln1_w, sv.mean1, sv.rstd1, w.dx_mid, dx_in, lo ? dx_in_lo : nullptr,
                          g->ln1_w, g->ln1_b, dx_in_colsum, w.ln_ws1, d.R, d.D, s, dr_prev2,
                          (grouped || grouped32) ? &folds.job[2] : nullptr, AVF_F32, d.xdt, inq, ins));
  if (!grouped && !grouped32) AVF_TRY(linear_dw(d, w.dqkv, 3 * d.I, sv.h1, d.D, g->w_qkv, w.gemm_ws, s));
  if (dw_desc) {
    dw_desc->magic = kDwDescMagic;
    dw_desc->grp = grp;
// ... 1 lines not shown
    for (int j = 0; j < 3; ++j) dw_desc->folds[j] = folds.job[j];
    return 0;
  }
  if (grouped) {
    AVF_TRY(gemm_bf16_tn_group(grp, s, &folds));
  }
  if (grouped32) AVF_TRY(fold_list(folds, s));
  return 0;
}

extern "C" int avf_layer_bwd(const avf_layer_cfg* cfg, const avf_layer_params* p, const void* lowp, const void* x_in,
                             const void* saved, const float* dx_out, const void* dx_out_lo,
                             const float* dx_out_colsum, float* dx_in, void* dx_in_lo, float* dx_in_colsum,
                             const avf_layer_grads* g, void* workspace, void* stream) {
  return layer_bwd_impl(cfg, p, lowp, x_in, saved, dx_out, dx_out_lo, dx_out_colsum, dx_in, dx_in_lo, dx_in_colsum, g, workspace,
                        stream, nullptr, nullptr);
}

extern "C" int avf_layer_dw_defer_ok(const avf_layer_cfg* cfg, int* tiles_per_layer, int* slots) {
  Dims d;
  if (make_dims(cfg, &d) || !dw_defer_mode_ok(d) || d.R % 64 != 0) return 0;
  TnGroupArgs ga = dw_group(d, nullptr, nullptr, nullptr, nullptr, nullptr, nullptr, nullptr, nullptr, nullptr);
  if (!gemm_bf16_tn_group_ok(ga)) return 0;
  int t = 0, sl = 0;
  gemm_bf16_tn_group_plan(ga, &t, &sl);
  if (tiles_per_layer) *tiles_per_layer = t;
  if (slots) *slots = sl;
  return 1;
}
extern "C" int avf_layers_dw_max(void) { return kTnGroupMax / 4; }
extern "C" size_t avf_layer_dw_block_bytes(const avf_layer_cfg* cfg) {
  Dims d;
  if (make_dims(cfg, &d) || !dw_defer_mode_ok(d)) return 0;
  return align_up(carve_dw_block(d, nullptr, nullptr), 256);
}
extern "C" size_t avf_layer_dw_desc_bytes(void) { return sizeof(DwDeferred); }

extern "C" int avf_layer_bwd_pos(const avf_layer_cfg* cfg, const avf_layer_params* p, const void* lowp, const void* x_in,
                                 const void* saved, const float* dx_out, const void* dx_out_lo, const float* dx_out_colsum,
                                 float* d_pos, const avf_layer_grads* g, void* workspace, void* stream) {
  AVF_REQUIRE(d_pos, "layer_bwd_pos: null d_pos");
  return layer_bwd_impl(cfg, p, lowp, x_in, saved, dx_out, dx_out_lo, dx_out_colsum, nullptr, nullptr, nullptr, g, workspace, stream,
                        nullptr, nullptr, d_pos);
}
extern "C" int avf_layer_bwd_dx_pos(const avf_layer_cfg* cfg, const avf_layer_params* p, const void* lowp, const void* x_in,
                                    const void* saved, const float* dx_out, const void* dx_out_lo, const float* dx_out_colsum,
                                    float* d_pos, const avf_layer_grads* g, void* workspace, void* dw_block, void* dw_desc,
                                    void* stream) {
  AVF_REQUIRE(d_pos && dw_block && dw_desc, "layer_bwd_dx_pos: null d_pos / operand block / descriptor");
  return layer_bwd_impl(cfg, p, lowp, x_in, saved, dx_out, dx_out_lo, dx_out_colsum, nullptr, nullptr, nullptr, g, workspace, stream,
                        dw_block, (DwDeferred*)dw_desc, d_pos);
}

extern "C" int avf_layer_bwd_dx(const avf_layer_cfg* cfg, const avf_layer_params* p, const void* lowp, const void* x_in,
                                const void* saved, const float* dx_out, const void* dx_out_lo,
                                const float* dx_out_colsum, float* dx_in, void* dx_in_lo, float* dx_in_colsum,
                                const avf_layer_grads* g, void* workspace, void* dw_block, void* dw_desc, void* stream) {
  AVF_REQUIRE(dw_block && dw_desc, "layer_bwd_dx: null operand block / descriptor");
  return layer_bwd_impl(cfg, p, lowp, x_in, saved, dx_out, dx_out_lo, dx_out_colsum, dx_in, dx_in_lo, dx_in_colsum, g, workspace,
                        stream, dw_block, (DwDeferred*)dw_desc);
}

static int layers_dw_group(const avf_layer_cfg* cfgs, int n_layers, const void* const* descs, TnGroupArgs* grp, FoldList* fl) {
  AVF_REQUIRE(cfgs && n_layers >= 1 && n_layers <= kTnGroupMax / 4, "layers_dw: 1..%d layers per group", kTnGroupMax / 4);
  memset(grp, 0, sizeof(*grp));
  if (fl) memset(fl, 0, sizeof(*fl));
  for (int l = 0; l < n_layers; ++l) {
    Dims d;
    AVF_TRY(make_dims(&cfgs[l], &d));
    AVF_REQUIRE(dw_defer_mode_ok(d), "layers_dw: layer %d is in a mode that keeps its weight gradients in the layer", l);
    TnGroupArgs one;
    if (descs) {
      const DwDeferred* dd = (const DwDeferred*)descs[l];
      AVF_REQUIRE(dd && dd->magic == kDwDescMagic, "layers_dw: descriptor %d was not written by avf_layer_bwd_dx", l);
      one = dd->grp;
      AVF_REQUIRE(one.K == d.R, "layers_dw: descriptor %d belongs to another configuration", l);
      for (int j = 0; j < 3; ++j) fl->job[3 * l + j] = dd->folds[j];
    } else {
      one = dw_group(d, nullptr, nullptr, nullptr, nullptr, nullptr, nullptr, nullptr, nullptr, nullptr);
    }
    AVF_REQUIRE(l == 0 || one.K == grp->K, "layers_dw: the layers of a group share their token rows");
    grp->K = one.K;
    for (int i = 0; i < 4; ++i) {
      const int q = 4 * l + i;
      grp->A[q] = one.A[i]; grp->B[q] = one.B[i]; grp->C[q] = one.C[i];
      grp->M[q] = one.M[i]; grp->N[q] = one.N[i]; grp->lda[q] = one.lda[i]; grp->ldb[q] = one.ldb[i];
    }
  }
  grp->count = 4 * n_layers;
  if (fl) fl->count = 3 * n_layers;
  return 0;
}
extern "C" size_t avf_layers_dw_workspace_bytes(const avf_layer_cfg* cfgs, int n_layers) {
  TnGroupArgs grp;
  if (layers_dw_group(cfgs, n_layers, nullptr, &grp, nullptr)) return 0;
  return gemm_bf16_tn_group_ws(grp);
}
extern "C" int avf_layers_dw(const avf_layer_cfg* cfgs, int n_layers, const void* const* descs, void* workspace,
                             size_t workspace_bytes, void* stream) {
  AVF_REQUIRE(descs, "layers_dw: null descriptors");
  TnGroupArgs grp;
  FoldList fl;
  AVF_TRY(layers_dw_group(cfgs, n_layers, descs, &grp, &fl));
  AVF_REQUIRE(gemm_bf16_tn_group_ok(grp), "layers_dw: the group does not fit the grouped launch");
  const size_t need = gemm_bf16_tn_group_ws(grp);
  AVF_REQUIRE(need == 0 || (workspace && ((uintptr_t)workspace & 15) == 0 && workspace_bytes >= need),
              "layers_dw: split-K workspace missing or too small (%zu bytes given, %zu needed)", workspace_bytes, need);
  grp.workspace = workspace;
  return gemm_bf16_tn_group(grp, (hipStream_t)stream, &fl);
}
```

multi-modal-multi-label-facial-action-unit-detection-with-transformer_amd/csrc/layernorm.hip:

```cpp
#include <algorithm>
#include <type_traits>

#include "common.hpp"

namespace avf {

template <typename F>
static int ln_nv(int dim, F&& f) {
  switch ((dim + 255) / 256) {
    case 1: return f(int_c<1>{});
    case 2: return f(int_c<2>{});
    case 3: return f(int_c<3>{});
    case 4: return f(int_c<4>{});
    default: return f(int_c<6>{});
  }
}
template <typename F>
static int ln_nv8(int dim, F&& f) {
  switch ((dim + 511) / 512) {
    case 1: return f(int_c<1>{}, int_c<4>{});
    case 2: return f(int_c<2>{}, int_c<2>{});
    default: return f(int_c<3>{}, int_c<1>{});
  }
}
// ... 446 lines not shown
        xh[i] = make_float4((v.x - mu) * rs, (v.y - mu) * rs, (v.z - mu) * rs, (v.w - mu) * rs);
      }
      const float g0 = d[i].x * g[i].x, g1 = d[i].y * g[i].y, g2 = d[i].z * g[i].z, g3 = d[i].w * g[i].w;
      s1 += (g0 + g1) + (g2 + g3);
      s2 += (g0 * xh[i].x + g1 * xh[i].y) + (g2 * xh[i].z + g3 * xh[i].w);
    }
    s1 = wave_sum(s1) * invD;
    s2 = wave_sum(s2) * invD;
#pragma unroll
    for (int i = 0; i < NV; ++i) {
      if (!act[i]) continue;
      const int c = lane * 4 + 256 * i;
      float4 r = make_float4(0.f, 0.f, 0.f, 0.f);
      if (dres) r = load4<ResT>(dres + row * D + c);
      float4 o;
      o.x = rs * (d[i].x * g[i].x - s1 - xh[i].x * s2) + r.x;
      o.y = rs * (d[i].y * g[i].y - s1 - xh[i].y * s2) + r.y;
      o.z = rs * (d[i].z * g[i].z - s1 - xh[i].z * s2) + r.z;
      o.w = rs * (d[i].w * g[i].w - s1 - xh[i].w * s2) + r.w;
      if (dx) *reinterpret_cast<float4*>(dx + row * D + c) = o;
      if (drop.thresh16) {
        const float4 f = drop_factor4(drop, dkey, (uint64_t)row * D + c);
        o.x *= f.x; o.y *= f.y; o.z *= f.z; o.w *= f.w;
      }
      if (dx_lo) store4<bf16>(dx_lo + row * D + c, o);
      if (dxq) {
        const float ov[4] = {o.x, o.y, o.z, o.w};
        uint32_t sb;
        const uint32_t qw = mx8_encode4(ov, &sb);
        *reinterpret_cast<uint32_t*>(dxq + row * D + c) = qw;
        if ((lane & 7) == 0) dxs[row * (D >> 5) + (c >> 5)] = (uint8_t)sb;
      }
      adg[i].x += d[i].x * xh[i].x; adg[i].y += d[i].y * xh[i].y; adg[i].z += d[i].z * xh[i].z; adg[i].w += d[i].w * xh[i].w;
      adb[i].x += d[i].x; adb[i].y += d[i].y; adb[i].z += d[i].z; adb[i].w += d[i].w;
      acs[i].x += o.x; acs[i].y += o.y; acs[i].z += o.z; acs[i].w += o.w;
    }
  }
  float* mine = lds + wave * 3 * D;
#pragma unroll
  for (int i = 0; i < NV; ++i) {
    if (!act[i]) continue;
    const int c = lane * 4 + 256 * i;
    *reinterpret_cast<float4*>(mine + c) = adg[i];
    *reinterpret_cast<float4*>(mine + D + c) = adb[i];
    *reinterpret_cast<float4*>(mine + 2 * D + c) = acs[i];
  }
  __syncthreads();
  float* out = partial + (int64_t)blockIdx.x * 3 * D;
  const int n = want_colsum ? 3 * D : 2 * D;
  for (int i = threadIdx.x; i < n; i += 256)
    out[i] = (lds[i] + lds[3 * D + i]) + (lds[6 * D + i] + lds[9 * D + i]);
}

template <int NV8, int RU, bool DROP = false, bool TOK = false>
__global__ __launch_bounds__(256) void ln_bwd_row8_kernel(const bf16* __restrict__ dy, const bf16* __restrict__ x,
                                                          const float* __restrict__ gamma, const float* __restrict__ mean,
                                                          const float* __restrict__ rstd, const bf16* __restrict__ dres,
                                                          bf16* __restrict__ dx_lo, float* __restrict__ partial, int64_t rows,
                                                          int D, int want_colsum, uint8_t* __restrict__ dxq = nullptr,
                                                          uint8_t* __restrict__ dxs = nullptr, float* __restrict__ dx = nullptr,
                                                          DropCfg drop = kNoDrop, bf16* __restrict__ dx_m = nullptr,
                                                          int rpb = LNR_ROWS_PER_BLOCK, int tokN = 0,
                                                          float* __restrict__ dpos = nullptr) {
  uint64_t dkey = 0;
  if constexpr (DROP) dkey = drop_key(drop);
  extern __shared__ __attribute__((aligned(16))) float lds[];
  const int lane = threadIdx.x & 63, wave = threadIdx.x >> 6;
  float gm[NV8][8];
#pragma unroll
  for (int i = 0; i < NV8; ++i) {
    const int c = lane * 8 + 512 * i;
#pragma unroll
    for (int k = 0; k < 8; ++k) gm[i][k] = 0.f;
    if (c < D) load8f(gamma + c, gm[i]);
  }
  float adg[NV8][8], adb[NV8][8], acs[NV8][8];
#pragma unroll
  for (int i = 0; i < NV8; ++i)
#pragma unroll
    for (int k = 0; k < 8; ++k) adg[i][k] = adb[i][k] = acs[i][k] = 0.f;
  const float invD = 1.0f / (float)D;
#pragma unroll 1
  for (int batch = 0; batch < rpb / 4 / RU; ++batch) {
  const int64_t i0 = TOK ? (int64_t)(batch * 4 + wave) * RU : (int64_t)blockIdx.x * rpb + wave * (rpb / 4) + batch * RU;
  const int64_t iend = TOK ? rows / tokN : rows;
  const auto row_of = [&](int64_t i) { return TOK ? i * tokN + blockIdx.x : i; };
  uint4 rd[RU][NV8], rx[RU][NV8], rr[RU][NV8];
  float mu[RU], rs[RU];
#pragma unroll
  for (int r = 0; r < RU; ++r) {
    const int64_t row = row_of(i0 + r < iend ? i0 + r : iend - 1);
#pragma unroll
    for (int i = 0; i < NV8; ++i) {
      const int c = lane * 8 + 512 * i;
      const bool ok = c < D;
      rd[r][i] = ok ? *reinterpret_cast<const uint4*>(dy + row * D + c) : make_uint4(0u, 0u, 0u, 0u);
      typedef uint32_t u32x4_nt __attribute__((ext_vector_type(4)));
      u32x4_nt xv = {0u, 0u, 0u, 0u};
      if (ok) xv = __builtin_nontemporal_load(reinterpret_cast<const u32x4_nt*>(x + row * D + c));
      rx[r][i] = make_uint4(xv[0], xv[1], xv[2], xv[3]);
      rr[r][i] = (ok && dres) ? *reinterpret_cast<const uint4*>(dres + row * D + c) : make_uint4(0u, 0u, 0u, 0u);
    }
    mu[r] = mean[row];
    rs[r] = rstd[row];
  }
  float s1[RU], s2[RU];
#pragma unroll
  for (int r = 0; r < RU; ++r) {
    float a = 0.f, b = 0.f;
#pragma unroll
    for (int i = 0; i < NV8; ++i) {
      float d[8], v[8];
      unpack8(rd[r][i], d);
      unpack8(rx[r][i], v);
#pragma unroll
      for (int k = 0; k < 8; ++k) {
        const float g = d[k] * gm[i][k];
        a += g;
        b = fmaf(g, (v[k] - mu[r]) * rs[r], b);
      }
    }
    s1[r] = a;
    s2[r] = b;
  }
#pragma unroll
  for (int r = 0; r < RU; ++r) {
    s1[r] = wave_sum(s1[r]) * invD;
    s2[r] = wave_sum(s2[r]) * invD;
  }
#pragma unroll
  for (int r = 0; r < RU; ++r) {
    if (i0 + r >= iend) break;
    const int64_t row = row_of(i0 + r);
#pragma unroll
    for (int i = 0; i < NV8; ++i) {
      const int c = lane * 8 + 512 * i;
      if (c >= D) continue;
      float d[8], v[8], e[8], o[8];
      unpack8(rd[r][i], d);
      unpack8(rx[r][i], v);
      unpack8(rr[r][i], e);
#pragma unroll
      for (int k = 0; k < 8; ++k) {
        const float xh = (v[k] - mu[r]) * rs[r];
        o[k] = rs[r] * (d[k] * gm[i][k] - s1[r] - xh * s2[r]) + e[k];
        adg[i][k] = fmaf(d[k], xh, adg[i][k]);
        adb[i][k] += d[k];
        if constexpr (!DROP) acs[i][k] += o[k];
      }
      if constexpr (TOK) continue;
      *reinterpret_cast<uint4*>(dx_lo + row * D + c) = pack8(o);
      if (dx) {
        *reinterpret_cast<float4*>(dx + row * D + c) = make_float4(o[0], o[1], o[2], o[3]);
        *reinterpret_cast<float4*>(dx + row * D + c + 4) = make_float4(o[4], o[5], o[6], o[7]);
      }
      if constexpr (DROP) {
        const uint64_t e0 = (uint64_t)row * D + c;
        const float4 f0 = drop_factor4(drop, dkey, e0), f1 = drop_factor4(drop, dkey, e0 + 4);
        o[0] *= f0.x; o[1] *= f0.y; o[2] *= f0.z; o[3] *= f0.w;
        o[4] *= f1.x; o[5] *= f1.y; o[6] *= f1.z; o[7] *= f1.w;
#pragma unroll
        for (int k = 0; k < 8; ++k) acs[i][k] += o[k];
        *reinterpret_cast<uint4*>(dx_m + row * D + c) = pack8(o);
      }
      if (dxq) {
        const MxBlock mb = mx8_encode(o);
        *reinterpret_cast<uint2*>(dxq + row * D + c) = mb.q;
        if ((lane & 3) == 0) dxs[row * (D >> 5) + (c >> 5)] = (uint8_t)mb.scale;
      }
    }
  }
  }
  float* mine = lds + wave * 3 * D;
#pragma unroll
  for (int i = 0; i < NV8; ++i) {
    const int c = lane * 8 + 512 * i;
    if (c >= D) continue;
#pragma unroll
    for (int h = 0; h < 2; ++h) {
      *reinterpret_cast<float4*>(mine + c + 4 * h) = make_float4(adg[i][4 * h], adg[i][4 * h + 1], adg[i][4 * h + 2], adg[i][4 * h + 3]);
      *reinterpret_cast<float4*>(mine + D + c + 4 * h) = make_float4(adb[i][4 * h], adb[i][4 * h + 1], adb[i][4 * h + 2], adb[i][4 * h + 3]);
      *reinterpret_cast<float4*>(mine + 2 * D + c + 4 * h) = make_float4(acs[i][4 * h], acs[i][4 * h + 1], acs[i][4 * h + 2], acs[i][4 * h + 3]);
    }
  }
  __syncthreads();
  float4* out = reinterpret_cast<float4*>(partial + (int64_t)blockIdx.x * 3 * D);
  const float4* l4 = reinterpret_cast<const float4*>(lds);
  const int n4 = (want_colsum ? 3 * D : 2 * D) >> 2, w4 = (3 * D) >> 2;
  for (int i = threadIdx.x; i < n4; i += 256) {
    const float4 a = l4[i], b = l4[w4 + i], c = l4[2 * w4 + i], d = l4[3 * w4 + i];
    const float4 v = make_float4((a.x + b.x) + (c.x + d.x), (a.y + b.y) + (c.y + d.y), (a.z + b.z) + (c.z + d.z), (a.w + b.w) + (c.w + d.w));
    if (TOK && i >= (2 * D) >> 2) reinterpret_cast<float4*>(dpos + (int64_t)blockIdx.x * D)[i - ((2 * D) >> 2)] = v;
    else out[i] = v;
  }
// ... 10 lines not shown
}
static inline int64_t ln_bwd_blocks(LnBwdFamily f, int64_t rows) { return ceil_div(rows, ln_bwd_rows_per_block(f, rows)); }

constexpr int LNR8_TOK_MAX_BATCH = 256;
bool layernorm_bwd_tok_ok(int batch, int tokens, int dim) {
  return batch > 0 && tokens > 0 && dim % 8 == 0 && dim <= 1536 && ln_row8_on() && batch <= LNR8_TOK_MAX_BATCH;
}

size_t layernorm_bwd_ws(int64_t rows, int dim, int tokens) {
  const int64_t nb = std::max({ln_bwd_blocks(LN_BWD_GENERAL, rows), ln_bwd_blocks(LN_BWD_REG, rows), ln_bwd_blocks(LN_BWD_ROW8, rows),
                               (int64_t)tokens});
  return (size_t)nb * 3 * dim * sizeof(float);
}

template <bool VEC, typename DyT>
static int launch_ln_bwd(const TimingScope* ts, hipStream_t s, const DyT* dy, const float* x, const float* gamma, const float* mean,
                         const float* rstd, const float* dres, float* dx, bf16* dx_lo, float* partial, int64_t rows, int D, int wc) {
  const size_t lds = (size_t)3 * D * sizeof(float);
  launch_in_scope(ts, ln_bwd_kernel<DyT, VEC>, dim3((unsigned)ln_bwd_blocks(LN_BWD_GENERAL, rows)), dim3(256), (uint32_t)lds, s, dy, x,
                  gamma, mean, rstd, dres, dx, dx_lo, partial, rows, D, wc);
  return check_launch("ln_bwd_kernel");
}

template <int NV, typename DyT, typename XT, typename ResT>
static int launch_ln_bwd_reg(const TimingScope* ts, hipStream_t s, const DyT* dy, const XT* x, const float* gamma, const float* mean,
                             const float* rstd, const ResT* dres, float* dx, bf16* dx_lo, float* partial, int64_t rows, int D, int wc,
                             const DropCfg& drop, uint8_t* dxq, uint8_t* dxs) {
  const size_t lds = (size_t)4 * 3 * D * sizeof(float);
  static PerDeviceOnce raised;
  if (lds > 64 * 1024 && raised.need()) {
    hipError_t e = hipFuncSetAttribute((const void*)ln_bwd_reg_kernel<DyT, NV, ResT, XT>, hipFuncAttributeMaxDynamicSharedMemorySize,
                                       4 * 3 * 256 * NV * (int)sizeof(float));
    AVF_REQUIRE(e == hipSuccess, "layernorm_bwd: cannot raise dynamic LDS limit");
    raised.mark();
  }
  launch_in_scope(ts, ln_bwd_reg_kernel<DyT, NV, ResT, XT>, dim3((unsigned)ln_bwd_blocks(LN_BWD_REG, rows)), dim3(256), (uint32_t)lds, s,
                  dy, x, gamma, mean, rstd, dres, dx, dx_lo, partial, rows, D, wc, drop, dxq, dxs, ln_bwd_rows_per_block(LN_BWD_REG, rows));
  return check_launch("ln_bwd_reg_kernel");
}

template <int NV8, int RU, bool DROP>
static int launch_ln_bwd_row8(const TimingScope* ts, hipStream_t s, const bf16* dy, const bf16* x, const float* gamma,
                              const float* mean, const float* rstd, const bf16* dres, bf16* dx_lo, float* partial, int64_t rows, int D,
                              int wc, uint8_t* dxq, uint8_t* dxs, float* dx, const DropCfg& drop, bf16* dx_m) {
  const size_t lds = (size_t)4 * 3 * D * sizeof(float);
  static PerDeviceOnce raised;
  if (lds > 64 * 1024 && raised.need()) {
    hipError_t e = hipFuncSetAttribute((const void*)ln_bwd_row8_kernel<NV8, RU, DROP>, hipFuncAttributeMaxDynamicSharedMemorySize,
                                       4 * 3 * 512 * NV8 * (int)sizeof(float));
    AVF_REQUIRE(e == hipSuccess, "layernorm_bwd: cannot raise dynamic LDS limit");
    raised.mark();
  }
  launch_in_scope(ts, ln_bwd_row8_kernel<NV8, RU, DROP>, dim3((unsigned)ln_bwd_blocks(LN_BWD_ROW8, rows)), dim3(256), (uint32_t)lds, s,
                  dy, x, gamma, mean, rstd, dres, dx_lo, partial, rows, D, wc, dxq, dxs, dx, drop, dx_m,
                  ln_bwd_rows_per_block(LN_BWD_ROW8, rows), 0, (float*)nullptr);
  return check_launch("ln_bwd_row8_kernel");
}

template <int NV8, int RU>
static int launch_ln_bwd_row8_tok(const TimingScope* ts, hipStream_t s, const bf16* dy, const bf16* x, const float* gamma,
                                  const float* mean, const float* rstd, const bf16* dres, float* dpos, float* partial, int batch,
                                  int tokens, int D) {
  const size_t lds = (size_t)4 * 3 * D * sizeof(float);
  static PerDeviceOnce raised;
  if (lds > 64 * 1024 && raised.need()) {
    hipError_t e = hipFuncSetAttribute((const void*)ln_bwd_row8_kernel<NV8, RU, false, true>, hipFuncAttributeMaxDynamicSharedMemorySize,
                                       4 * 3 * 512 * NV8 * (int)sizeof(float));
    AVF_REQUIRE(e == hipSuccess, "layernorm_bwd_tok: cannot raise dynamic LDS limit");
    raised.mark();
  }
  const int nbatch = (int)ceil_div((int64_t)batch, 4 * RU);
  launch_in_scope(ts, ln_bwd_row8_kernel<NV8, RU, false, true>, dim3((unsigned)tokens), dim3(256), (uint32_t)lds, s, dy, x, gamma, mean,
                  rstd, dres, (bf16*)nullptr, partial, (int64_t)batch * tokens, D, 1, (uint8_t*)nullptr, (uint8_t*)nullptr,
                  (float*)nullptr, kNoDrop, (bf16*)nullptr, nbatch * 4 * RU, tokens, dpos);
  return check_launch("ln_bwd_row8_kernel(tok)");
}

int layernorm_bwd_tok(const void* dy, const void* x, const float* gamma, const float* mean, const float* rstd, const void* dres,
                      float* dpos, float* dgamma, float* dbeta, void* ws, int batch, int tokens, int dim, hipStream_t s,
                      FoldJob* defer_fold) {
  AVF_REQUIRE(dy && x && gamma && mean && rstd && dpos && ws, "layernorm_bwd_tok: null pointer");
  AVF_REQUIRE(layernorm_bwd_tok_ok(batch, tokens, dim), "layernorm_bwd_tok: shape outside the token-major rule (batch=%d dim=%d)", batch, dim);
  AVF_REQUIRE((((uintptr_t)dy | (uintptr_t)x | (uintptr_t)dres | (uintptr_t)dpos | (uintptr_t)ws) & 15) == 0,
              "layernorm_bwd_tok: pointers must be 16-byte aligned");
  const int64_t rows = (int64_t)batch * tokens;
  TimingScope ts(KC_LAYERNORM, 0.0, (double)rows * dim * (2.0 + 2.0 + (dres ? 2.0 : 0.0)) + (double)tokens * dim * 4.0, s, true);
  float* partial = (float*)ws;
  AVF_TRY(ln_nv8(dim, [&](auto nv8, auto ru) {
    return launch_ln_bwd_row8_tok<decltype(nv8)::value, decltype(ru)::value>(&ts, s, (const bf16*)dy, (const bf16*)x, gamma, mean, rstd,
                                                                             (const bf16*)dres, dpos, partial, batch, tokens, dim);
  }));
  const FoldJob job{partial, tokens, 3 * dim, dim, dgamma, dbeta, nullptr};
  if (defer_fold) {
    *defer_fold = job;
    return 0;
  }
  return fold_job(job, s);
}

int layernorm_bwd(const void* dy, int dy_dtype, const void* xv, const float* gamma, const float* mean,
                  const float* rstd, const void* dres, float* dx, void* dx_lo, float* dgamma, float* dbeta,
                  float* dcolsum, void* ws, int64_t rows, int dim, hipStream_t s, const DropCfg& drop,
                  FoldJob* defer_fold, int dres_dtype, int x_dtype, void* mx_q, void* mx_s, void* dx_m) {
  AVF_REQUIRE(!dx_m || (drop.thresh16 && dx_lo && dy_dtype == AVF_BF16 && x_dtype == AVF_BF16 && (!dres || dres_dtype == AVF_BF16) &&
                        dim % 8 == 0 && dim <= 1536 && !mx_q),
              "layernorm_bwd: a separate masked image needs live dropout on the all-bf16 streams (dim %% 8 == 0, no MX-FP8 image)");
  AVF_REQUIRE(rows > 0 && dim > 0 && ws, "layernorm_bwd: bad arguments");
  AVF_REQUIRE(!mx_q || (mx_s && dy_dtype == AVF_BF16 && dim % 32 == 0 && dim <= 1536 && ((uintptr_t)mx_q & 3) == 0),
              "layernorm_bwd: the MX-FP8 image of dx needs bf16 dy, dim %% 32 == 0 and dim <= 1536 (dim=%d)", dim);
  AVF_REQUIRE(x_dtype == AVF_F32 || (x_dtype == AVF_BF16 && dy_dtype == AVF_BF16 && dim % 4 == 0 && dim <= 1536),
              "layernorm_bwd: a bf16 LayerNorm input needs bf16 dy, dim %% 4 == 0 and dim <= 1536");
  AVF_REQUIRE(dres_dtype == AVF_F32 || (dres_dtype == AVF_BF16 && dy_dtype == AVF_BF16 && dim % 4 == 0 && dim <= 1536 &&
                                         (!drop.thresh16 || dx_m) && dx_lo),
              "layernorm_bwd: a bf16 residual gradient needs bf16 dy, a bf16 output, dim %% 4 == 0, dim <= 1536, and with dropout a "
              "separate masked image");
  AVF_REQUIRE(dx || dx_lo, "layernorm_bwd: no output");
  AVF_REQUIRE(dx || (dim % 4 == 0 && dim <= 1536), "layernorm_bwd: dim %d runs the general kernel, which needs the fp32 dx", dim);
  AVF_REQUIRE(!drop.thresh16 || (dim % 4 == 0 && dim <= 1536), "layernorm_bwd: dropout needs dim %% 4 == 0 and dim <= 1536");
  AVF_REQUIRE((size_t)3 * dim * sizeof(float) <= 64 * 1024, "layernorm_bwd: dim %d too large", dim);
  TimingScope ts(KC_LAYERNORM, 0.0,
                 (double)rows * dim * ((dy_dtype == AVF_BF16 ? 2.0 : 4.0) + (x_dtype == AVF_BF16 ? 2.0 : 4.0) + (dres ? (dres_dtype == AVF_BF16 ? 2.0 : 4.0) : 0.0) +
                                       (dx ? 4.0 : 0.0) + (dx_lo ? 2.0 : 0.0)), s, true);
  float* partial = (float*)ws;
  const int wc = dcolsum ? 1 : 0;
  const float *x = (const float*)xv, *drf = (const float*)dres;
  const bf16 *dyb = (const bf16*)dy, *xb = (const bf16*)xv, *drb = (const bf16*)dres;
  uint8_t *dxq = (uint8_t*)mx_q, *dxs = (uint8_t*)mx_s;
  const bool fast = (dim % 4 == 0) && dim <= 1536 && (dy_dtype == AVF_F32 || dy_dtype == AVF_BF16);
  const bool row8 = fast && x_dtype == AVF_BF16 && dy_dtype == AVF_BF16 && (!dres || dres_dtype == AVF_BF16) && dx_lo &&
                    (!drop.thresh16 || dx_m) && (!mx_q || dim % 32 == 0) && dim % 8 == 0 && (ln_row8_on() || dx_m);
  const int nb = (int)ln_bwd_blocks(row8 ? LN_BWD_ROW8 : fast ? LN_BWD_REG : LN_BWD_GENERAL, rows);
  if (row8) {
    AVF_TRY(ln_nv8(dim, [&](auto nv8, auto ru) {
      constexpr int NV8 = decltype(nv8)::value, RU = decltype(ru)::value;
      if (dx_m)
        return launch_ln_bwd_row8<NV8, RU, true>(&ts, s, dyb, xb, gamma, mean, rstd, drb, (bf16*)dx_lo, partial, rows, dim, wc, nullptr,
                                                 nullptr, dx, drop, (bf16*)dx_m);
      return launch_ln_bwd_row8<NV8, RU, false>(&ts, s, dyb, xb, gamma, mean, rstd, drb, (bf16*)dx_lo, partial, rows, dim, wc, dxq, dxs,
                                                dx, kNoDrop, nullptr);
    }));
  } else if (fast) {
    auto reg = [&](auto* dyp, auto* xp, auto* drp) {
      return ln_nv(dim, [&](auto nv) {
        return launch_ln_bwd_reg<decltype(nv)::value>(&ts, s, dyp, xp, gamma, mean, rstd, drp, dx, (bf16*)dx_lo, partial, rows, dim, wc,
                                                      drop, dxq, dxs);
// ... 28 lines not shown
```

multi-modal-multi-label-facial-action-unit-detection-with-transformer_amd/ops.py:

```python
from __future__ import annotations

import ctypes as C
from typing import Optional, Tuple

import torch

from . import _lib
from ._lib import BF16, EPI_BIAS_GELU, EPI_BIAS_RES, EPI_DGELU, EPI_NONE, F32

_TORCH2AVF = {torch.float32: F32, torch.bfloat16: BF16}
_AVF2TORCH = {F32: torch.float32, BF16: torch.bfloat16}


def avf_dtype(dt) -> int:
    if isinstance(dt, int):
        return dt
    if isinstance(dt, str):
        return {"f32": F32, "fp32": F32, "float32": F32, "bf16": BF16, "bfloat16": BF16}[dt.lower()]
    return _TORCH2AVF[dt]


def torch_dtype(dt) -> torch.dtype:
    return _AVF2TORCH[avf_dtype(dt)]

# ... 941 lines not shown
def clip_gather_autoaugment_normalize(bank: torch.Tensor, video_db_nr: torch.Tensor, present: Optional[torch.Tensor],
                                      index: torch.Tensor, T: int, d: int, plan: torch.Tensor, lut: torch.Tensor,
                                      k: Optional[int] = None, flip: Optional[torch.Tensor] = None, layout: str = "cthw",
                                      out_dtype=torch.float32) -> torch.Tensor:
    F, B = _bank_args(bank, video_db_nr, present, index)
    _need_cuda(plan, lut, flip)
    _, H, W, Cn = bank.shape
    T = int(T)
    assert plan.dtype == torch.int32 and plan.is_contiguous() and tuple(plan.shape) == (B, T, 2, 8)
    k, dt, lay, out = _planes_out(B, T, H, W, Cn, lut, k, flip, layout, out_dtype, bank.device)
    _lib.check(_lib.load().avf_clip_gather_autoaugment_normalize(_ptr(bank), _ptr(video_db_nr), _ptr(present), _ptr(index), F, B, T,
                                                                 int(d), H, W, Cn, _ptr(plan), k, _ptr(lut), _ptr(flip), _ptr(out),
                                                                 dt, lay, _stream()), "clip_gather_autoaugment_normalize")
    return out


def fuse_tokens(clip: torch.Tensor, audio: torch.Tensor, pos: Optional[torch.Tensor], out_bf16: bool = False) -> torch.Tensor:
    _need_cuda(clip, audio)
    clip, audio = clip.contiguous(), audio.contiguous()
    B, Tv, D = clip.shape
    Ta = audio.shape[1]
    assert audio.shape[0] == B and audio.shape[2] == D and clip.dtype == audio.dtype == torch.float32
    if pos is not None:
        pos = pos.contiguous()
        assert pos.numel() == (Tv + Ta) * D and pos.dtype == torch.float32
    out = torch.empty((B, Tv + Ta, D), dtype=torch.bfloat16 if out_bf16 else torch.float32, device=clip.device)
    fn = _lib.load().avf_fuse_tokens_bf16 if out_bf16 else _lib.load().avf_fuse_tokens
    _lib.check(fn(_ptr(clip), _ptr(audio), _ptr(pos), _ptr(out), B, Tv, Ta, D, _stream()), "fuse_tokens")
    return out


def token_mean_fwd(y: torch.Tensor) -> torch.Tensor:
    _need_cuda(y)
    y = y.contiguous()
    B, T, D = y.shape
    out = torch.empty((B, D), dtype=torch.float32, device=y.device)
    fn = _lib.load().avf_token_mean_fwd_bf16 if y.dtype == torch.bfloat16 else _lib.load().avf_token_mean_fwd
    _lib.check(fn(_ptr(y), _ptr(out), B, T, D, _stream()), "token_mean_fwd")
    return out


def token_mean_bwd(g: torch.Tensor, tokens: int, want_bf16: bool = False, want_colsum: bool = False):
    _need_cuda(g)
    g = g.contiguous().to(torch.float32)
    B, D = g.shape
    dy = torch.empty((B, tokens, D), dtype=torch.float32, device=g.device)
    lo = torch.empty((B, tokens, D), dtype=torch.bfloat16, device=g.device) if want_bf16 else None
    cs = torch.empty(D, dtype=torch.float32, device=g.device) if want_colsum else None
    _lib.check(_lib.load().avf_token_mean_bwd(_ptr(g), _ptr(dy), _ptr(lo), _ptr(cs), B, tokens, D, _stream()),
               "token_mean_bwd")
    return dy, lo, cs


def conv_pack_weight(w: torch.Tensor, gamma: torch.Tensor, beta: torch.Tensor, running_mean: torch.Tensor,
                     running_var: torch.Tensor, eps: float = 1e-5):
    _need_cuda(w, gamma, beta, running_mean, running_var)
    ts = [t.detach().contiguous() for t in (w, gamma, beta, running_mean, running_var)]
    assert all(t.dtype == torch.float32 for t in ts) and ts[0].dim() == 4 and ts[0].shape[2] == ts[0].shape[3]
    Cout, Cin, k, _ = ts[0].shape
    assert all(t.numel() == Cout for t in ts[1:])
    wp = torch.empty((Cout, k * k * Cin), dtype=torch.bfloat16, device=w.device)
    scale = torch.empty(Cout, dtype=torch.float32, device=w.device)
    shift = torch.empty(Cout, dtype=torch.float32, device=w.device)
    _lib.check(_lib.load().avf_conv_pack_weight(*[_ptr(t) for t in ts], float(eps), _ptr(wp), _ptr(scale), _ptr(shift), Cout, Cin, k,
                                                _stream()), "conv_pack_weight")
    return wp, scale, shift


def conv_out_hw(H: int, W: int, k: int, stride: int) -> Tuple[int, int]:
    pad = 1 if k == 3 else 0
    return (H + 2 * pad - k) // stride + 1, (W + 2 * pad - k) // stride + 1


def conv_plan(N: int, H: int, W: int, Cin: int, Cout: int, k: int, stride: int = 1) -> dict:
    out = [C.c_int(-1) for _ in range(3)]
    _lib.check(_lib.load().avf_conv_plan(int(N), int(H), int(W), int(Cin), int(Cout), int(k), int(stride), *[C.byref(o) for o in out]),
               "conv_plan")
    return dict(tile=out[0].value, tile_m=out[1].value, tile_n=out[2].value)


def conv2d_nhwc(x: torch.Tensor, w_packed: torch.Tensor, scale: torch.Tensor, shift: torch.Tensor, k: int, stride: int = 1,
                residual: Optional[torch.Tensor] = None, relu: bool = False, out: Optional[torch.Tensor] = None,
                out_dtype=torch.bfloat16) -> torch.Tensor:
    _need_cuda(x, w_packed, scale, shift, residual, out)
    N, H, W, Cin = x.shape
    Cout = w_packed.shape[0]
    Ho, Wo = conv_out_hw(H, W, k, stride)
    if out is None:
        out = torch.empty((N, Ho, Wo, Cout), dtype=torch_dtype(out_dtype), device=x.device)
    for name, t, shape in (("x", x, (N, H, W, Cin)), ("w_packed", w_packed, (Cout, k * k * Cin)), ("scale", scale, (Cout,)),
                           ("shift", shift, (Cout,)), ("residual", residual, (N, Ho, Wo, Cout)), ("out", out, (N, Ho, Wo, Cout))):
        if t is not None and (tuple(t.shape) != shape or not t.is_contiguous()):
            raise ValueError(f"conv2d_nhwc: {name} must be a contiguous {shape} tensor (got {tuple(t.shape)}, strides {t.stride()})")
    assert w_packed.dtype == torch.bfloat16 and scale.dtype == shift.dtype == torch.float32
    _lib.check(_lib.load().avf_conv2d_nhwc(_ptr(x), avf_dtype(x.dtype), _ptr(w_packed), _ptr(scale), _ptr(shift), _ptr(residual),
                                           avf_dtype(residual.dtype) if residual is not None else F32, int(bool(relu)), int(k),
                                           int(stride), _ptr(out), avf_dtype(out.dtype), N, H, W, Cin, Cout, _stream()), "conv2d_nhwc")
    return out


def avgpool_nhwc(x: torch.Tensor, out: Optional[torch.Tensor] = None) -> torch.Tensor:
    _need_cuda(x, out)
    if not x.is_contiguous():
        raise ValueError("avgpool_nhwc: x must be contiguous")
    N, Cn = x.shape[0], x.shape[-1]
    HW = x.numel() // (N * Cn)
# ... 31 lines not shown
```

multi-modal-multi-label-facial-action-unit-detection-with-transformer_amd/transformer.py:

```python
from __future__ import annotations

import ctypes as C
import os
from typing import Callable, List, Optional

import torch
from torch import nn

from . import _lib, ops
from .ops import avf_dtype

PARAMS_PER_LAYER = 11

import os as _os

_CANARY = 4096 if _os.environ.get("AVF_DEBUG_CANARY") == "1" else 0
_guarded: list = []


def _alloc_bytes(nbytes: int, dev) -> torch.Tensor:
    t = torch.empty(max(int(nbytes), 16) + _CANARY, dtype=torch.uint8, device=dev)
    if _CANARY:
        import weakref
        t[-_CANARY:].fill_(0xA5)
# ... 16 lines not shown
    _guarded[:] = alive


class _Holder(nn.Module):

    def forward(self, *a, **k):
        raise RuntimeError("parameter holder: the computation runs in the enclosing Transformer")


def _make_layer(dim: int, heads: int, dim_head: int, mlp_dim: int, dropout: float) -> nn.ModuleList:
    inner = heads * dim_head
    project_out = not (heads == 1 and dim_head == dim)
    attn = _Holder()
    attn.to_qkv = nn.Linear(dim, inner * 3, bias=False)
    attn.to_out = nn.Sequential(nn.Linear(inner, dim), nn.Dropout(dropout)) if project_out else nn.Identity()
    pre_a = _Holder()
    pre_a.norm = nn.LayerNorm(dim)
    pre_a.fn = attn
    res_a = _Holder()
    res_a.fn = pre_a
    ff = _Holder()
    ff.net = nn.Sequential(nn.Linear(dim, mlp_dim), nn.Identity(), nn.Dropout(dropout), nn.Linear(mlp_dim, dim),
                           nn.Dropout(dropout))
    pre_f = _Holder()
    pre_f.norm = nn.LayerNorm(dim)
    pre_f.fn = ff
    res_f = _Holder()
    res_f.fn = pre_f
    return nn.ModuleList([res_a, res_f])


def _ptr(t):
    return None if t is None else C.c_void_p(t.data_ptr())


def plan_dw_groups(n_layers: int, tiles_per_layer: int, slots: int, max_group: int = 4, force: int = 0) -> List[int]:
    if n_layers <= 0:
        return []
    g = force if force > 0 else slots // max(1, tiles_per_layer)
    g = max(1, min(g, max_group, n_layers))
    out = [g] * (n_layers // g)
    if n_layers % g:
        out.append(n_layers % g)
    return out


class _DwGroup:
    __slots__ = ("cfgs", "ws_bytes", "blocks", "descs", "desc_ptrs", "ws")


def _stack_ends_on(part: str) -> bool:
    v = os.environ.get("AVF_STACK_ENDS", "1").strip()
    return v != "0" and (v in ("", "1") or part in v.split(","))


class _StackFn(torch.autograd.Function):

    @staticmethod
    def forward(ctx, x, audio, pos, mod, pool, keep, *params):
        lib = _lib.load()
        ctx.fused = audio is not None
        embed = None
        if ctx.fused:
            T = x.shape[1] + audio.shape[1]
            if pos.shape[-2] < T or pos.shape[-1] != x.shape[-1]:
                raise ValueError(f"pos_embedding {tuple(pos.shape)} does not cover {T} tokens of width {x.shape[-1]}")
            ctx.tv, ctx.shape_pos = x.shape[1], pos.shape
            pos_rows = pos.detach().reshape(pos.shape[-2], pos.shape[-1])[:T]
            if (mod.resid_bf16 and keep is None and x.shape[1] > 0 and audio.shape[1] > 0 and _stack_ends_on("embed")
                    and lib.avf_layer_fwd_embed_ok(C.byref(mod._cfg(x.shape[0], T, 0, None, None)))):
                embed = (x.detach().float().contiguous(), audio.detach().float().contiguous(), pos_rows.float().contiguous())
                x = torch.empty((x.shape[0], T, x.shape[2]), dtype=torch.bfloat16, device=x.device)
            else:
                x = ops.fuse_tokens(x.detach().float(), audio.detach().float(), pos_rows, out_bf16=mod.resid_bf16)
        B, N, D = x.shape
        dev = x.device
        stream = C.c_void_p(torch.cuda.current_stream().cuda_stream)
        L = mod.depth
        seed_t = mod._advance_seed(dev)
        if keep is not None and keep.shape != (B, N):
            raise ValueError(f"mask has incorrect dimensions: {tuple(keep.shape)} after the leading True, tokens {(B, N)}")
        ctx.keep = keep
        ckey = (B, N, mod.training, mod.dropout, None if seed_t is None else seed_t.data_ptr(),
                None if keep is None else keep.data_ptr(), mod.compute_dtype, mod.mx8, mod.mx8_bwd, mod.resid_bf16)
        chit = mod.__dict__.get("_cfg_cache")
        if chit is not None and chit[0] == ckey:
            cfgs = chit[1]
        else:
            cfgs = [mod._cfg(B, N, l, seed_t, keep) for l in range(L)]
            mod.__dict__["_cfg_cache"] = (ckey, cfgs)
        cfg = cfgs[0]
        params = list(params)
        need_grad = any(ctx.needs_input_grad)
        ctx.grad_in = ctx.needs_input_grad[:3]
        saved_bytes = lib.avf_layer_saved_bytes(C.byref(cfg))
        if saved_bytes == 0:
            _lib.check(1, "layer configuration")
        ws = mod._workspace(lib, cfg, dev)
        lowps = mod._lowp(lib, cfg, params, dev, stream)
        rs16 = bool(cfg.resid_bf16)
        x0 = x.detach().contiguous().view(B * N, D)
        if rs16 and x0.dtype != torch.bfloat16:
            xb = torch.empty((B * N, D), dtype=torch.bfloat16, device=dev)
            _lib.check(lib.avf_cast_f32_to_bf16(_ptr(x0), _ptr(xb), B * N * D, stream), "cast")
            x0 = xb
        xs = [x0]
        saved = []
        shared = None
        for l in range(L):
            pp = mod._param_struct(params, l)
            if need_grad:
                sv = _alloc_bytes(saved_bytes, dev)
            else:
                shared = shared if shared is not None else _alloc_bytes(saved_bytes, dev)
                sv = shared
            x_out = torch.empty((B * N, D), dtype=torch.bfloat16 if rs16 else torch.float32, device=dev)
            if l == 0 and embed is not None:
                _lib.check(lib.avf_layer_fwd_embed(C.byref(cfgs[0]), C.byref(pp), _ptr(lowps[0]), _ptr(embed[0]), _ptr(embed[1]),
                                                   _ptr(embed[2]), ctx.tv, _ptr(x0), _ptr(x_out), _ptr(sv), _ptr(ws), stream),
                           "layer_fwd_embed[0]")
            else:
                _lib.check(lib.avf_layer_fwd(C.byref(cfgs[l]), C.byref(pp), _ptr(lowps[l]), _ptr(xs[-1]), _ptr(x_out), _ptr(sv),
                                             _ptr(ws), stream), f"layer_fwd[{l}]")
            saved.append(sv)
            xs.append(x_out)
        ctx.mod = mod
        ctx.cfgs = cfgs
        ctx.seed_t = seed_t
        ctx.shape = (B, N, D)
        ctx.xs = xs[:-1] if need_grad else None
        ctx.saved_bufs = saved if need_grad else None
        ctx.params = params
        ctx.lowps = lowps
        ctx.pool = pool
        _check_canaries()
        if pool:
            pooled = torch.empty((B, D), dtype=torch.float32, device=dev)
            fn = lib.avf_token_mean_fwd_bf16 if rs16 else lib.avf_token_mean_fwd
            _lib.check(fn(_ptr(xs[-1]), _ptr(pooled), B, N, D, stream), "token_mean_fwd")
            return pooled
        out = xs[-1].view(B, N, D)
        return out.float() if rs16 else out

    @staticmethod
    def backward(ctx, dy):
        with torch.cuda.device(dy.device):
            return _StackFn._backward(ctx, dy)

    @staticmethod
    def _backward(ctx, dy):
        if ctx.saved_bufs is None:
            raise RuntimeError("Transformer (HIP): backward through the stack a second time - its saved activations are released "
                               "after the first backward (retain_graph=True is not supported; run the forward again)")
        lib = _lib.load()
        mod = ctx.mod
        cfgs = ctx.cfgs
        cfg = cfgs[0]
        B, N, D = ctx.shape
        dev = dy.device
        stream = C.c_void_p(torch.cuda.current_stream().cuda_stream)
        L = mod.depth
        ws = mod._workspace(lib, cfg, dev)
        bf16 = cfg.dtype == _lib.BF16
        lo_bytes = lib.avf_layer_grad_stream_bytes(C.byref(cfg)) if bf16 else 0
        lo_a = torch.empty(lo_bytes, dtype=torch.uint8, device=dev) if bf16 else None
        lo_b = torch.empty(lo_bytes, dtype=torch.uint8, device=dev) if bf16 else None
        have_lo = False
        top_colsum = False
        d_pos = None
        if (ctx.fused and ctx.grad_in[2] and not ctx.grad_in[0] and not ctx.grad_in[1] and cfg.grad_stream_bf16
                and _stack_ends_on("pos") and lib.avf_layer_bwd_pos_ok(C.byref(cfg))):
            d_pos = torch.empty((N, D), dtype=torch.float32, device=dev)
        if ctx.pool:
            g = dy.contiguous().to(torch.float32)
            have_lo = top_colsum = bf16 and cfg.dropout_p == 0.0
            dx = None if (have_lo and d_pos is not None) else torch.empty((B * N, D), dtype=torch.float32, device=dev)
        else:
            dx = dy.contiguous().view(B * N, D).to(torch.float32)
            if dx.data_ptr() == dy.data_ptr():
                dx = dx.clone()
        live = mod.flat_parameters()
        sizes = [p.numel() for p in ctx.params[:PARAMS_PER_LAYER]]
        hook = mod._grad_hook
        groups = mod._dw_plan(lib, cfgs) if (bf16 and hook is None and L > 1) else [1] * L
        per_layer = sum(sizes)
        flat_all = torch.empty(L * per_layer, dtype=torch.float32, device=dev)
        shapes = [p.shape for p in ctx.params[:PARAMS_PER_LAYER]]
        parts = flat_all.split_with_sizes(sizes * L)
        views = [[parts[l * PARAMS_PER_LAYER + i] if len(shapes[i]) == 1 else parts[l * PARAMS_PER_LAYER + i].view(shapes[i])
                  for i in range(PARAMS_PER_LAYER)] for l in range(L)]
        flats = list(flat_all.split(per_layer))
        offs, acc = [], 0
        for n in sizes:
            offs.append(4 * acc)
            acc += n
        base = flat_all.data_ptr()
        B2 = PARAMS_PER_LAYER - 1
        gs16 = bool(cfg.grad_stream_bf16)
        if ctx.pool:
            _lib.check(lib.avf_token_mean_bwd(_ptr(g), None if (gs16 and have_lo) else _ptr(dx),
                                              _ptr(lo_a) if have_lo else None,
                                              _ptr(views[L - 1][B2]) if top_colsum else None, B, N, D, stream),
                       "token_mean_bwd")
        def hand_over(l):
            waiter = hook(l, flats[l]) if hook is not None else None
            for p, v in zip(live[l * PARAMS_PER_LAYER:(l + 1) * PARAMS_PER_LAYER], views[l]):
                if not p.requires_grad:
                    continue
                if p.grad is None:
                    p.grad = v
                else:
                    if waiter is not None:
                        waiter()
                    p.grad.add_(v)

        top = L
        for gsize in groups:
            dw = mod._dw_buffers(lib, cfgs, top, gsize, dev) if gsize > 1 else None
            held = []
            for k, l in enumerate(range(top - 1, top - 1 - gsize, -1)):
                gp = _lib.LayerPtrs(*[base + 4 * l * per_layer + o for o in offs])
                pp = mod._param_struct(ctx.params, l)
                dx_out_p = None if (gs16 and have_lo) else _ptr(dx)
                dx_in_p = None if (gs16 and l > 0) else _ptr(dx)
                lead = (C.byref(cfgs[l]), C.byref(pp), _ptr(ctx.lowps[l]), _ptr(ctx.xs[l]),
                        _ptr(ctx.saved_bufs[l]), dx_out_p, _ptr(lo_a) if have_lo else None,
                        _ptr(views[l][B2]) if (l < L - 1 or top_colsum) else None)
                if l == 0 and d_pos is not None:
                    args = lead + (_ptr(d_pos), C.byref(gp), _ptr(ws))
                    fn, fn_dx, what = lib.avf_layer_bwd_pos, lib.avf_layer_bwd_dx_pos, "layer_bwd_pos"
                else:
                    args = lead + (dx_in_p, _ptr(lo_b), _ptr(views[l - 1][B2]) if l > 0 else None, C.byref(gp), _ptr(ws))
                    fn, fn_dx, what = lib.avf_layer_bwd, lib.avf_layer_bwd_dx, "layer_bwd"
                if dw is None:
                    _lib.check(fn(*args, stream), f"{what}[{l}]")
                    lo_a, lo_b = lo_b, lo_a
                else:
                    _lib.check(fn_dx(*args, _ptr(dw.blocks[k]), dw.descs[k], stream), f"{what}_dx[{l}]")
                    held.append(lo_a)
                    lo_a, lo_b = lo_b, torch.empty(lo_bytes, dtype=torch.uint8, device=dev)
                have_lo = bf16
            if dw is not None:
                _lib.check(lib.avf_layers_dw(dw.cfgs, gsize, dw.desc_ptrs, _ptr(dw.ws), dw.ws_bytes, stream), f"layers_dw[{top - gsize}:{top}]")
            del held
            for l in range(top - 1, top - 1 - gsize, -1):
                hand_over(l)
            top -= gsize
        _check_canaries()
        ctx.saved_bufs = None
        ctx.xs = None
        tail = (None, None, None, *([None] * (L * PARAMS_PER_LAYER)))
        dx = None if dx is None else dx.view(B, N, D)
        if not ctx.fused:
            return (dx, None, None) + tail
        d_clip = dx[:, :ctx.tv] if ctx.grad_in[0] else None
        d_audio = dx[:, ctx.tv:] if ctx.grad_in[1] else None
        if ctx.grad_in[2]:
            if d_pos is None:
                d_pos = ops.colsum(dx.view(B, N * D)).view(N, D)
            if ctx.shape_pos[-2] > N:
                d_pos = torch.nn.functional.pad(d_pos, (0, 0, 0, ctx.shape_pos[-2] - N))
            d_pos = d_pos.view(ctx.shape_pos)
        return (d_clip, d_audio, d_pos) + tail


class Transformer(nn.Module):
    _instances = 0

    def __init__(self, dim, depth, heads, dim_head, mlp_dim, dropout=0., compute_dtype="bf16", residual_dtype="f32"):
        super().__init__()
        self.dim, self.depth, self.heads, self.dim_head, self.mlp_dim = dim, depth, heads, dim_head, mlp_dim
        self.dropout = float(dropout)
        cd = compute_dtype.lower().replace("_", "-") if isinstance(compute_dtype, str) else ""
        self.mx8 = cd in ("mx8", "fp8", "mxfp8", "mx8-fwd")
        self.mx8_bwd = self.mx8 and cd != "mx8-fwd"
        if self.mx8 and (dim % 128 or mlp_dim % 128 or dim > 1536):
            raise ValueError(f"compute_dtype='mx8' needs dim and mlp_dim to be multiples of 128 and dim <= 1536 "
                             f"(dim={dim}, mlp_dim={mlp_dim})")
        self.compute_dtype = _lib.BF16 if self.mx8 else avf_dtype(compute_dtype)
        rd = str(residual_dtype).lower()
        if rd not in ("f32", "fp32", "float32", "bf16", "bfloat16"):
# ... 224 lines not shown
```

Baseline: 19100 clips/s.

## Fold final token-mean pool into top layer's second MLP linear, fwd and bwd

The last transformer layer's output is only consumed through a token mean. So the forward pass now sums GELU activations and residuals over tokens and applies W2 to the per-batch sums, instead of running the full W2 GEMM and a separate pooling pass. The backward pass mirrors this. It computes dW2/db2 from pooled sums, builds the dGELU input by broadcasting W2^T·d_pooled across tokens, and uses a layernorm backward that adds the broadcast pooled gradient as the residual. This removes one large (B·T × M × D) GEMM in each direction plus the pooled-output materialisation, at the cost of new reduction kernels and more top-layer-specific code paths.

Result: no change. 19110 clips/s (median of 5 runs) (+0.1%).

```diff
diff --git a/include/avformer_hip.h b/include/avformer_hip.h
--- a/include/avformer_hip.h
+++ b/include/avformer_hip.h
@@ -316,6 +316,29 @@
                          const void* saved, const float* dx_out, const void* dx_out_lo, const float* dx_out_colsum, float* d_pos,
                          const avf_layer_grads* g, void* workspace, void* dw_block, void* dw_desc, void* stream);
 
+int avf_layer_top_ok(const avf_layer_cfg* cfg);
+int avf_top_pooled(const void* g_bf16, const void* x_mid_bf16, const void* w2_bf16, const float* b2, float* pooled, float* gsum,
+                   float* xsum, int batch, int tokens, int dim, int mlp_dim, void* stream);
+size_t avf_top_dgelu_workspace_bytes(int64_t rows, int mlp_dim);
+int avf_top_dgelu(const float* d_pooled, const void* w2t_bf16, const void* u_bf16, float* r, void* du_bf16, float* db1,
+                  void* workspace, int batch, int tokens, int dim, int mlp_dim, void* stream);
+int avf_top_dw2(const float* d_pooled, const float* gsum, float* dw2, float* db2, int batch, int tokens, int dim, int mlp_dim,
+                void* stream);
+int avf_layernorm_bwd_clipres_ok(int dim);
+int avf_layernorm_bwd_clipres(const void* dy_bf16, const void* x_bf16, const float* gamma, const float* mean, const float* rstd,
+                              const float* d_pooled, int tokens, void* dx_bf16, float* dgamma, float* dbeta, float* dcolsum,
+                              void* workspace, int64_t rows, int dim, void* stream);
+int avf_layer_fwd_top(const avf_layer_cfg* cfg, const avf_layer_params* p, const void* lowp, const void* x_in, float* pooled,
+                      float* gsum, void* saved, void* workspace, void* stream);
+int avf_layer_top_gsum(const avf_layer_cfg* cfg, const void* saved, float* gsum, void* stream);
+int avf_layer_bwd_top(const avf_layer_cfg* cfg, const avf_layer_params* p, const void* lowp, const void* x_in, const void* saved,
+                      const float* d_pooled, const float* gsum, float* dx_in, void* dx_in_lo, float* dx_in_colsum,
+                      const avf_layer_grads* g, void* workspace, void* stream);
+int avf_layer_bwd_dx_top(const avf_layer_cfg* cfg, const avf_layer_params* p, const void* lowp, const void* x_in,
+                         const void* saved, const float* d_pooled, const float* gsum, float* dx_in, void* dx_in_lo,
+                         float* dx_in_colsum, const avf_layer_grads* g, void* workspace, void* dw_block, void* dw_desc,
+                         void* stream);
+
 int avf_layer_bwd(const avf_layer_cfg* cfg, const avf_layer_params* p, const void* lowp, const void* x_in,
                   const void* saved, const float* dx_out, const void* dx_out_lo, const float* dx_out_colsum,
                   float* dx_in, void* dx_in_lo, float* dx_in_colsum, const avf_layer_grads* g, void* workspace,
diff --git a/multi-modal-multi-label-facial-action-unit-detection-with-transformer_amd/_build.py b/multi-modal-multi-label-facial-action-unit-detection-with-transformer_amd/_build.py
--- a/multi-modal-multi-label-facial-action-unit-detection-with-transformer_amd/_build.py
+++ b/multi-modal-multi-label-facial-action-unit-detection-with-transformer_amd/_build.py
@@ -9,7 +9,7 @@
 CSRC = os.path.join(HERE, "csrc")
 LIBDIR = os.path.join(HERE, "lib")
 LIBNAME = "libavformer_hip.so"
-SOURCES = ["api.hip", "norm_elem.hip", "layernorm.hip", "gemm_f32.hip", "attn_f32.hip", "attn_f32_mfma.hip", "attn_f32x3.hip", "gemm_bf16.hip", "gemm_ws.hip", "gemm_mx8.hip", "attn_bf16.hip", "attn_bwd_merged.hip", "layer.hip", "optim.hip", "grad_control.hip", "layer_small.hip", "heads.hip", "task_loss.hip", "eval_metrics.hip", "mel.hip", "clip.hip", "augment.hip", "clip_bank.hip", "mel_bank.hip", "conv.hip"]
+SOURCES = ["api.hip", "norm_elem.hip", "layernorm.hip", "gemm_f32.hip", "attn_f32.hip", "attn_f32_mfma.hip", "attn_f32x3.hip", "gemm_bf16.hip", "gemm_ws.hip", "gemm_mx8.hip", "attn_bf16.hip", "attn_bwd_merged.hip", "layer.hip", "stack_top.hip", "optim.hip", "grad_control.hip", "layer_small.hip", "heads.hip", "task_loss.hip", "eval_metrics.hip", "mel.hip", "clip.hip", "augment.hip", "clip_bank.hip", "mel_bank.hip", "conv.hip"]
 HEADERS = [os.path.join(CSRC, "common.hpp"), os.path.join(CSRC, "gemm_nt.hpp"), os.path.join(CSRC, "gemm_dispatch.hpp"), os.path.join(CSRC, "attn_dispatch.hpp"), os.path.join(CSRC, "clip_source.hpp"),
            os.path.join(CSRC, "clip_kernels.hpp"), os.path.join(CSRC, "augment_kernels.hpp"), os.path.join(CSRC, "mel_kernels.hpp"), os.path.join(os.path.dirname(HERE), "include", "avformer_hip.h")]
 FLAGS = ["--offload-arch=gfx950", "-O3", "-std=c++17", "-fPIC"]
diff --git a/multi-modal-multi-label-facial-action-unit-detection-with-transformer_amd/_lib.py b/multi-modal-multi-label-facial-action-unit-detection-with-transformer_amd/_lib.py
--- a/multi-modal-multi-label-facial-action-unit-detection-with-transformer_amd/_lib.py
+++ b/multi-modal-multi-label-facial-action-unit-detection-with-transformer_amd/_lib.py
@@ -164,6 +164,19 @@
                                  C.POINTER(LayerPtrs), _vp, _vp]),
     "avf_layer_bwd_dx_pos": (_int, [C.POINTER(LayerCfg), C.POINTER(LayerPtrs), _vp, _vp, _vp, _vp, _vp, _vp, _vp,
                                     C.POINTER(LayerPtrs), _vp, _vp, _vp, _vp]),
+    "avf_top_pooled": (_int, [_vp, _vp, _vp, _vp, _vp, _vp, _vp, _int, _int, _int, _int, _vp]),
+    "avf_top_dgelu_workspace_bytes": (_sz, [_i64, _int]),
+    "avf_top_dgelu": (_int, [_vp, _vp, _vp, _vp, _vp, _vp, _vp, _int, _int, _int, _int, _vp]),
+    "avf_top_dw2": (_int, [_vp, _vp, _vp, _vp, _int, _int, _int, _int, _vp]),
+    "avf_layernorm_bwd_clipres_ok": (_int, [_int]),
+    "avf_layernorm_bwd_clipres": (_int, [_vp, _vp, _vp, _vp, _vp, _vp, _int, _vp, _vp, _vp, _vp, _vp, _i64, _int, _vp]),
+    "avf_layer_top_ok": (_int, [C.POINTER(LayerCfg)]),
+    "avf_layer_fwd_top": (_int, [C.POINTER(LayerCfg), C.POINTER(LayerPtrs), _vp, _vp, _vp, _vp, _vp, _vp, _vp]),
+    "avf_layer_top_gsum": (_int, [C.POINTER(LayerCfg), _vp, _vp, _vp]),
+    "avf_layer_bwd_top": (_int, [C.POINTER(LayerCfg), C.POINTER(LayerPtrs), _vp, _vp, _vp, _vp, _vp, _vp, _vp, _vp,
+                                 C.POINTER(LayerPtrs), _vp, _vp]),
+    "avf_layer_bwd_dx_top": (_int, [C.POINTER(LayerCfg), C.POINTER(LayerPtrs), _vp, _vp, _vp, _vp, _vp, _vp, _vp, _vp,
+                                    C.POINTER(LayerPtrs), _vp, _vp, _vp, _vp]),
     "avf_layer_dw_defer_ok": (_int, [C.POINTER(LayerCfg), C.POINTER(C.c_int), C.POINTER(C.c_int)]),
     "avf_layers_dw_max": (_int, []),
     "avf_layer_dw_block_bytes": (_sz, [C.POINTER(LayerCfg)]),
diff --git a/multi-modal-multi-label-facial-action-unit-detection-with-transformer_amd/csrc/api.hip b/multi-modal-multi-label-facial-action-unit-detection-with-transformer_amd/csrc/api.hip
--- a/multi-modal-multi-label-facial-action-unit-detection-with-transformer_amd/csrc/api.hip
+++ b/multi-modal-multi-label-facial-action-unit-detection-with-transformer_amd/csrc/api.hip
@@ -217,6 +217,35 @@
   AVF_REQUIRE(dgamma && dbeta, "layernorm_bwd_pos: null pointer");
   return layernorm_bwd_tok(dy_bf16, x_bf16, gamma, mean, rstd, dres_bf16, d_pos, dgamma, dbeta, workspace, batch, tokens, dim,
                            (hipStream_t)stream);
+}
+extern "C" int avf_top_pooled(const void* g_bf16, const void* x_mid_bf16, const void* w2_bf16, const float* b2, float* pooled,
+                              float* gsum, float* xsum, int batch, int tokens, int dim, int mlp_dim, void* stream) {
+  AVF_REQUIRE(pooled && gsum && xsum && x_mid_bf16, "top_pooled: null pointer");
+  AVF_TRY(token_sums_bf16(g_bf16, gsum, mlp_dim, x_mid_bf16, xsum, dim, batch, tokens, (hipStream_t)stream));
+  return rows_linear_bf16w(gsum, w2_bf16, xsum, b2, pooled, batch, dim, mlp_dim, 1.0f / (float)tokens, (hipStream_t)stream);
+}
+extern "C" size_t avf_top_dgelu_workspace_bytes(int64_t rows, int mlp_dim) { return top_dgelu_ws(rows, mlp_dim); }
+extern "C" int avf_top_dgelu(const float* d_pooled, const void* w2t_bf16, const void* u_bf16, float* r, void* du_bf16, float* db1,
+                             void* workspace, int batch, int tokens, int dim, int mlp_dim, void* stream) {
+  AVF_REQUIRE(r && db1, "top_dgelu: null pointer");
+  AVF_TRY(rows_linear_bf16w(d_pooled, w2t_bf16, nullptr, nullptr, r, batch, mlp_dim, dim, 1.0f, (hipStream_t)stream, 1.0f / (float)tokens,
+                            true));
+  FoldJob fj;
+  AVF_TRY(top_dgelu(r, u_bf16, du_bf16, workspace, (int64_t)batch * tokens, tokens, mlp_dim, db1, &fj, (hipStream_t)stream));
+  return fold_job(fj, (hipStream_t)stream);
+}
+extern "C" int avf_top_dw2(const float* d_pooled, const float* gsum, float* dw2, float* db2, int batch, int tokens, int dim,
+                           int mlp_dim, void* stream) {
+  AVF_REQUIRE(tokens > 0, "top_dw2: bad arguments");
+  return top_dw2(d_pooled, gsum, dw2, db2, batch, dim, mlp_dim, 1.0f / (float)tokens, (hipStream_t)stream);
+}
+extern "C" int avf_layernorm_bwd_clipres_ok(int dim) { return layernorm_bwd_clipres_ok(dim) ? 1 : 0; }
+extern "C" int avf_layernorm_bwd_clipres(const void* dy_bf16, const void* x_bf16, const float* gamma, const float* mean,
+                                         const float* rstd, const float* d_pooled, int tokens, void* dx_bf16, float* dgamma,
+                                         float* dbeta, float* dcolsum, void* workspace, int64_t rows, int dim, void* stream) {
+  AVF_REQUIRE(dgamma && dbeta && tokens > 0, "layernorm_bwd_clipres: null pointer");
+  return layernorm_bwd_clipres(dy_bf16, x_bf16, gamma, mean, rstd, d_pooled, 1.0f / (float)tokens, tokens, dx_bf16, dgamma, dbeta,
+                               dcolsum, workspace, rows, dim, (hipStream_t)stream);
 }
 extern "C" size_t avf_colsum_workspace_bytes(int64_t rows, int cols) { return colsum_ws(rows, cols); }
 extern "C" int avf_colsum(const void* in, int in_dtype, int64_t rows, int cols, int64_t ld, float* out,
diff --git a/multi-modal-multi-label-facial-action-unit-detection-with-transformer_amd/csrc/common.hpp b/multi-modal-multi-label-facial-action-unit-detection-with-transformer_amd/csrc/common.hpp
--- a/multi-modal-multi-label-facial-action-unit-detection-with-transformer_amd/csrc/common.hpp
+++ b/multi-modal-multi-label-facial-action-unit-detection-with-transformer_amd/csrc/common.hpp
@@ -343,6 +343,16 @@
 int layernorm_bwd_tok(const void* dy, const void* x, const float* gamma, const float* mean, const float* rstd, const void* dres,
                       float* dpos, float* dgamma, float* dbeta, void* ws, int batch, int tokens, int dim, hipStream_t s,
                       FoldJob* defer_fold = nullptr);
+int token_sums_bf16(const void* src0, float* out0, int W0, const void* src1, float* out1, int W1, int batch, int tokens, hipStream_t s);
+int rows_linear_bf16w(const float* a, const void* W, const float* add, const float* bias, float* out, int B, int J, int K, float scale,
+                      hipStream_t s, float a_scale = 1.0f, bool round_a = false);
+size_t top_dgelu_ws(int64_t rows, int M);
+int top_dgelu(const float* r, const void* u, void* du, void* ws, int64_t rows, int tokens, int M, float* db1, FoldJob* fold, hipStream_t s);
+int top_dw2(const float* dp, const float* gsum, float* dW2, float* db2, int B, int D, int M, float inv, hipStream_t s);
+bool layernorm_bwd_clipres_ok(int dim);
+int layernorm_bwd_clipres(const void* dy, const void* x, const float* gamma, const float* mean, const float* rstd, const float* dp,
+                          float inv, int tokens, void* dx_lo, float* dgamma, float* dbeta, float* dcolsum, void* ws, int64_t rows,
+                          int dim, hipStream_t s, FoldJob* defer_fold = nullptr);
 int layernorm_bwd(const void* dy, int dy_dtype, const void* x, const float* gamma, const float* mean,
                   const float* rstd, const void* dres, float* dx, void* dx_lo, float* dgamma, float* dbeta,
                   float* dcolsum, void* ws, int64_t rows, int dim, hipStream_t s, const DropCfg& drop = kNoDrop,
diff --git a/multi-modal-multi-label-facial-action-unit-detection-with-transformer_amd/csrc/layer.hip b/multi-modal-multi-label-facial-action-unit-detection-with-transformer_amd/csrc/layer.hip
--- a/multi-modal-multi-label-facial-action-unit-detection-with-transformer_amd/csrc/layer.hip
+++ b/multi-modal-multi-label-facial-action-unit-detection-with-transformer_amd/csrc/layer.hip
@@ -177,6 +177,7 @@
   const int maxc = d.M > d.D ? d.M : d.D;
   size_t csb = colsum_ws(d.R, maxc);
   if (d.dt == AVF_BF16 && gemm_nt_colsum_ws(d.R, d.M) > csb) csb = gemm_nt_colsum_ws(d.R, d.M);
+  if (d.dt == AVF_BF16 && top_dgelu_ws(d.R, d.M) > csb) csb = top_dgelu_ws(d.R, d.M);
   return csb;
 }
 
@@ -190,6 +191,7 @@
   void *dx_out_s, *dx_mid_m;
   float *gy_m, *gm_m;
   float* small_part;
+  float *top_xsum, *top_r;
 };
 size_t carve_work(const Dims& d, void* base, Work* w) {
   Carver c(base);
@@ -215,6 +217,9 @@
     TnGroupArgs ga = dw_group(d, nullptr, nullptr, nullptr, nullptr, nullptr, nullptr, nullptr, nullptr, nullptr);
     const size_t gg = gemm_bf16_tn_group_ws(ga);
     g = g > gg ? g : gg;
+    ga.count = 3;
+    const size_t g3 = gemm_bf16_tn_group_ws(ga);
+    g = g > g3 ? g : g3;
   } else {
     const size_t a = gemm_f32_ws(3 * d.I, d.D, d.R), b = gemm_f32_ws(d.D, d.I, d.R);
     const size_t e = gemm_f32_ws(d.M, d.D, d.R), f = gemm_f32_ws(d.D, d.M, d.R);
@@ -248,6 +253,8 @@
   const bool f32_drop = d.dt == AVF_F32 && d.p > 0.f;
   t.gy_m = (float*)c.take(f32_drop ? d.R * d.D * 4 : 0);
   t.gm_m = (float*)c.take(f32_drop ? d.R * d.D * 4 : 0);
+  t.top_xsum = (float*)c.take(d.dt == AVF_BF16 ? (size_t)d.B * d.D * 4 : 0);
+  t.top_r = (float*)c.take(d.dt == AVF_BF16 ? (size_t)d.B * d.M * 4 : 0);
   if (w) *w = t;
   return c.off;
 }
@@ -452,22 +459,37 @@
   return !make_dims(cfg, &d) && stack_ends_mode_ok(d) && layernorm_bwd_tok_ok(d.B, d.N, d.D);
 }
 
+static bool stack_top_mode_ok(const Dims& d) { return stack_ends_mode_ok(d) && layernorm_bwd_clipres_ok(d.D); }
+extern "C" int avf_layer_top_ok(const avf_layer_cfg* cfg) {
+  Dims d;
+  return !make_dims(cfg, &d) && stack_top_mode_ok(d);
+}
+struct TopOut {
+  float *pooled, *gsum;
+};
+struct TopGrad {
+  const float *d_pooled, *gsum;
+};
+
 struct EmbedSrc {
   const float *clip, *audio, *pos;
   int t_video;
   void* x0;
 };
 static int layer_fwd_impl(const avf_layer_cfg* cfg, const avf_layer_params* p, const void* lowp, const void* x_in, void* x_out,
-                          void* saved, void* workspace, void* stream, const EmbedSrc* emb) {
+                          void* saved, void* workspace, void* stream, const EmbedSrc* emb, const TopOut* top = nullptr) {
   Dims d;
   AVF_TRY(make_dims(cfg, &d));
+  AVF_REQUIRE(!top || (stack_top_mode_ok(d) && top->pooled && top->gsum && workspace && !emb && !x_out),
+              "layer_fwd_top: needs the all-bf16 streams without dropout, fp8 or mask (ask avf_layer_top_ok first), the two outputs "
+              "and the workspace");
   if (emb) {
     AVF_REQUIRE(stack_ends_mode_ok(d) && layernorm_fwd_embed_ok(d.D) && emb->x0 && emb->t_video > 0 && emb->t_video < d.N,
                 "layer_fwd_embed: needs the all-bf16 streams without dropout, fp8 or mask, and both token groups (ask "
                 "avf_layer_fwd_embed_ok first)");
     x_in = emb->x0;
   }
-  AVF_REQUIRE(p && x_in && x_out && saved, "layer_fwd: null pointer");
+  AVF_REQUIRE(p && x_in && (x_out || top) && saved, "layer_fwd: null pointer");
   AVF_REQUIRE(d.dt == AVF_F32 || lowp, "layer_fwd(bf16): lowp weights missing");
   hipStream_t s = (hipStream_t)stream;
   Saved sv;
@@ -530,6 +552,12 @@
   AVF_TRY(linear_fwd(d, sv.o, d.I, wo, d.D, sv.x_mid, d.xdt, AVF_EPI_BIAS_RES, p->b_out, x_in, nullptr, s, dr0, l.ws.wo_p));
   AVF_TRY(layernorm_fwd(sv.x_mid, p->ln2_w, p->ln2_b, sv.h2, d.dt, sv.mean2, sv.rstd2, d.R, d.D, cfg->ln_eps, s, nullptr, nullptr, d.xdt));
   AVF_TRY(linear_fwd(d, sv.h2, d.D, w1, d.M, sv.g, d.dt, AVF_EPI_BIAS_GELU, p->b1, nullptr, sv.u, s, dr1, l.ws.w1_p));
+  if (top) {
+    Work w;
+    carve_work(d, workspace, &w);
+    AVF_TRY(token_sums_bf16(sv.g, top->gsum, d.M, sv.x_mid, w.top_xsum, d.D, d.B, d.N, s));
+    return rows_linear_bf16w(top->gsum, w2, w.top_xsum, p->b2, top->pooled, d.B, d.D, d.M, 1.0f / (float)d.N, s);
+  }
   AVF_TRY(linear_fwd(d, sv.g, d.M, w2, d.D, x_out, d.xdt, AVF_EPI_BIAS_RES, p->b2, sv.x_mid, nullptr, s, dr2));
   return 0;
 }
@@ -546,11 +574,25 @@
   return layer_fwd_impl(cfg, p, lowp, nullptr, x_out, saved, workspace, stream, &emb);
 }
 
+extern "C" int avf_layer_fwd_top(const avf_layer_cfg* cfg, const avf_layer_params* p, const void* lowp, const void* x_in,
+                                 float* pooled, float* gsum, void* saved, void* workspace, void* stream) {
+  const TopOut top{pooled, gsum};
+  return layer_fwd_impl(cfg, p, lowp, x_in, nullptr, saved, workspace, stream, nullptr, &top);
+}
+extern "C" int avf_layer_top_gsum(const avf_layer_cfg* cfg, const void* saved, float* gsum, void* stream) {
+  Dims d;
+  AVF_TRY(make_dims(cfg, &d));
+  AVF_REQUIRE(stack_top_mode_ok(d) && saved && gsum, "layer_top_gsum: bad arguments (ask avf_layer_top_ok first)");
+  Saved sv;
+  carve_saved(d, (void*)saved, &sv);
+  return token_sums_bf16(sv.g, gsum, d.M, nullptr, nullptr, 0, d.B, d.N, (hipStream_t)stream);
+}
+
 static int layer_bwd_impl(const avf_layer_cfg* cfg, const avf_layer_params* p, const void* lowp, const void* x_in,
                           const void* saved, const float* dx_out, const void* dx_out_lo,
                           const float* dx_out_colsum, float* dx_in, void* dx_in_lo, float* dx_in_colsum,
                           const avf_layer_grads* g, void* workspace, void* stream, void* dw_block, DwDeferred* dw_desc,
-                          float* d_pos = nullptr) {
+                          float* d_pos = nullptr, const TopGrad* top = nullptr) {
   Dims d;
   AVF_TRY(make_dims(cfg, &d));
   AVF_REQUIRE(!d_pos || (stack_ends_mode_ok(d) && layernorm_bwd_tok_ok(d.B, d.N, d.D) && !dx_in && !dx_in_lo && !dx_in_colsum),
@@ -560,7 +602,9 @@
               "layer_bwd_dx: this mode keeps its weight gradients in the layer (ask avf_layer_dw_defer_ok first), or the "
               "operand block is missing / not 256-byte aligned");
   AVF_REQUIRE(p && x_in && saved && g && workspace, "layer_bwd: null pointer");
-  AVF_REQUIRE(d.gs16 ? (dx_out || dx_out_lo) && (dx_in || dx_in_lo || d_pos) : (dx_out && dx_in), "layer_bwd: null gradient pointer");
+  AVF_REQUIRE(!top || (stack_top_mode_ok(d) && top->d_pooled && top->gsum && !dx_out && !dx_out_lo && !dx_out_colsum && !d_pos),
+              "layer_bwd_top: needs the all-bf16 streams without dropout, fp8 or mask (ask avf_layer_top_ok first), d_pooled and gsum");
+  AVF_REQUIRE(d.gs16 ? (dx_out || dx_out_lo || top) && (dx_in || dx_in_lo || d_pos) : (dx_out && dx_in), "layer_bwd: null gradient pointer");
   AVF_REQUIRE(!d.gs16 || dx_in_lo || d_pos, "layer_bwd(grad_stream_bf16): dx_in_lo missing");
   AVF_REQUIRE(d.dt == AVF_F32 || lowp, "layer_bwd(bf16): lowp weights missing");
   hipStream_t s = (hipStream_t)stream;
@@ -581,7 +625,8 @@
   const void* gy = dx_out;
   const void* gy_stream = nullptr;
   bool own_copy = false;
-  if (lo) {
+  if (top) gy = nullptr;
+  else if (lo) {
     if (dx_out_lo && d.gsd) {
       gy_stream = dx_out_lo;
       gy = (const char*)dx_out_lo + grad_q_off(d.R, d.D);
@@ -609,6 +654,7 @@
   const void* gm = lo ? (gm_masked ? (const void*)w.dx_mid_m : (const void*)w.dx_mid_lo)
                       : (f32_drop0 ? (const void*)w.gm_m : (const void*)w.dx_mid);
   TnGroupArgs grp = dw_group(d, gy, sv.g, w.du, sv.h2, gm, sv.o, w.dqkv, sv.h1, g);
+  if (top) grp.count = 3;
   grp.workspace = w.gemm_ws;
   const bool grouped32 = !lo && !small_bwd && gemm_f32x3_tn_group_ok(grp);
   const bool grouped = lo && gemm_bf16_tn_group_ok(grp);
@@ -666,7 +712,10 @@
     return 0;
   }
 
-  if (dx_out_colsum && dx_out_colsum != g->b2)
+  const float top_inv = 1.0f / (float)d.N;
+  if (top)
+    AVF_TRY(top_dw2(top->d_pooled, top->gsum, g->w2, g->b2, d.B, d.D, d.M, top_inv, s));
+  else if (dx_out_colsum && dx_out_colsum != g->b2)
     AVF_REQUIRE(hipMemcpyAsync(g->b2, dx_out_colsum, (size_t)d.D * 4, hipMemcpyDeviceToDevice, s) == hipSuccess,
                 "layer_bwd: memcpy failed");
   else if (!dx_out_colsum) {
@@ -679,7 +728,7 @@
       AVF_TRY(colsum(gy, AVF_BF16, d.R, d.D, d.D, g->b2, w.cs_ws, s));
     }
   }
-  if (!grouped && !grouped32) AVF_TRY(linear_dw(d, gy, d.D, sv.g, d.M, g->w2, w.gemm_ws, s));
+  if (!grouped && !grouped32 && !top) AVF_TRY(linear_dw(d, gy, d.D, sv.g, d.M, g->w2, w.gemm_ws, s));
   const void *gyq = nullptr, *gys = nullptr;
   void *inq = nullptr, *ins = nullptr;
   if (d.mxb) {
@@ -709,6 +758,12 @@
     else
       AVF_TRY(linear_dx_mx(d, gyq, gys, d.D, l.w2t_q, l.w2t_s, d.M, w.du, AVF_EPI_DGELU, sv.u, s, g->b1, w.cs_ws, dr1,
                            grouped ? &folds.job[0] : nullptr, w.duq, w.dus));
+  } else if (top) {
+    AVF_TRY(rows_linear_bf16w(top->d_pooled, l.w2_t, nullptr, nullptr, w.top_r, d.B, d.M, d.D, 1.0f, s, top_inv, true));
+    FoldJob fj;
+    AVF_TRY(top_dgelu(w.top_r, sv.u, w.du, w.cs_ws, d.R, d.N, d.M, g->b1, &fj, s));
+    if (grouped) folds.job[0] = fj;
+    else AVF_TRY(fold_job(fj, s));
   } else if (lo) {
     AVF_TRY(linear_dx(d, gy, d.D, p->w2, l.w2_t, d.M, w.du, AVF_EPI_DGELU, sv.u, s, g->b1, w.cs_ws, dr1,
                       grouped ? &folds.job[0] : nullptr, l.ws.w2t_p));
@@ -721,7 +776,10 @@
                          nullptr));
   else
     AVF_TRY(linear_dx(d, w.du, d.M, p->w1, l.w1_t, d.D, w.dh, AVF_EPI_NONE, nullptr, s));
-  if (d.gs16)
+  if (top)
+    AVF_TRY(layernorm_bwd_clipres(w.dh, sv.x_mid, p->ln2_w, sv.mean2, sv.rstd2, top->d_pooled, top_inv, d.N, w.dx_mid_lo, g->ln2_w,
+                                  g->ln2_b, g->b_out, w.ln_ws, d.R, d.D, s, grouped ? &folds.job[1] : nullptr));
+  else if (d.gs16)
     AVF_TRY(layernorm_bwd(w.dh, d.dt, sv.x_mid, p->ln2_w, sv.mean2, sv.rstd2, d.gsd ? gy_stream : gy, nullptr, w.dx_mid_lo,
                           g->ln2_w, g->ln2_b, g->b_out, w.ln_ws, d.R, d.D, s, dr0, grouped ? &folds.job[1] : nullptr, AVF_BF16,
                           d.xdt, w.mq, w.ms, gm_masked ? w.dx_mid_m : nullptr));
@@ -829,6 +887,23 @@
                         dw_block, (DwDeferred*)dw_desc, d_pos);
 }
 
+extern "C" int avf_layer_bwd_top(const avf_layer_cfg* cfg, const avf_layer_params* p, const void* lowp, const void* x_in,
+                                 const void* saved, const float* d_pooled, const float* gsum, float* dx_in, void* dx_in_lo,
+                                 float* dx_in_colsum, const avf_layer_grads* g, void* workspace, void* stream) {
+  const TopGrad top{d_pooled, gsum};
+  return layer_bwd_impl(cfg, p, lowp, x_in, saved, nullptr, nullptr, nullptr, dx_in, dx_in_lo, dx_in_colsum, g, workspace, stream,
+                        nullptr, nullptr, nullptr, &top);
+}
+extern "C" int avf_layer_bwd_dx_top(const avf_layer_cfg* cfg, const avf_layer_params* p, const void* lowp, const void* x_in,
+                                    const void* saved, const float* d_pooled, const float* gsum, float* dx_in, void* dx_in_lo,
+                                    float* dx_in_colsum, const avf_layer_grads* g, void* workspace, void* dw_block, void* dw_desc,
+                                    void* stream) {
+  AVF_REQUIRE(dw_block && dw_desc, "layer_bwd_dx_top: null operand block / descriptor");
+  const TopGrad top{d_pooled, gsum};
+  return layer_bwd_impl(cfg, p, lowp, x_in, saved, nullptr, nullptr, nullptr, dx_in, dx_in_lo, dx_in_colsum, g, workspace, stream,
+                        dw_block, (DwDeferred*)dw_desc, nullptr, &top);
+}
+
 extern "C" int avf_layer_bwd_dx(const avf_layer_cfg* cfg, const avf_layer_params* p, const void* lowp, const void* x_in,
                                 const void* saved, const float* dx_out, const void* dx_out_lo,
                                 const float* dx_out_colsum, float* dx_in, void* dx_in_lo, float* dx_in_colsum,
@@ -838,10 +913,12 @@
                         stream, dw_block, (DwDeferred*)dw_desc);
 }
 
-static int layers_dw_group(const avf_layer_cfg* cfgs, int n_layers, const void* const* descs, TnGroupArgs* grp, FoldList* fl) {
+static int layers_dw_group(const avf_layer_cfg* cfgs, int n_layers, const void* const* descs, TnGroupArgs* grp, FoldList* fl,
+                           bool top_first = false) {
   AVF_REQUIRE(cfgs && n_layers >= 1 && n_layers <= kTnGroupMax / 4, "layers_dw: 1..%d layers per group", kTnGroupMax / 4);
   memset(grp, 0, sizeof(*grp));
   if (fl) memset(fl, 0, sizeof(*fl));
+  int q = 0;
   for (int l = 0; l < n_layers; ++l) {
     Dims d;
     AVF_TRY(make_dims(&cfgs[l], &d));
@@ -851,27 +928,30 @@
       const DwDeferred* dd = (const DwDeferred*)descs[l];
       AVF_REQUIRE(dd && dd->magic == kDwDescMagic, "layers_dw: descriptor %d was not written by avf_layer_bwd_dx", l);
       one = dd->grp;
-      AVF_REQUIRE(one.K == d.R, "layers_dw: descriptor %d belongs to another configuration", l);
+      AVF_REQUIRE(one.K == d.R && (one.count == 4 || one.count == 3), "layers_dw: descriptor %d belongs to another configuration", l);
       for (int j = 0; j < 3; ++j) fl->job[3 * l + j] = dd->folds[j];
     } else {
       one = dw_group(d, nullptr, nullptr, nullptr, nullptr, nullptr, nullptr, nullptr, nullptr, nullptr);
+      if (l == 0 && top_first) one.count = 3;
     }
     AVF_REQUIRE(l == 0 || one.K == grp->K, "layers_dw: the layers of a group share their token rows");
     grp->K = one.K;
-    for (int i = 0; i < 4; ++i) {
-      const int q = 4 * l + i;
+    for (int i = 0; i < one.count; ++i, ++q) {
       grp->A[q] = one.A[i]; grp->B[q] = one.B[i]; grp->C[q] = one.C[i];
       grp->M[q] = one.M[i]; grp->N[q] = one.N[i]; grp->lda[q] = one.lda[i]; grp->ldb[q] = one.ldb[i];
     }
   }
-  grp->count = 4 * n_layers;
+  grp->count = q;
   if (fl) fl->count = 3 * n_layers;
   return 0;
 }
 extern "C" size_t avf_layers_dw_workspace_bytes(const avf_layer_cfg* cfgs, int n_layers) {
   TnGroupArgs grp;
   if (layers_dw_group(cfgs, n_layers, nullptr, &grp, nullptr)) return 0;
-  return gemm_bf16_tn_group_ws(grp);
+  const size_t full = gemm_bf16_tn_group_ws(grp);
+  if (layers_dw_group(cfgs, n_layers, nullptr, &grp, nullptr, true)) return 0;
+  const size_t top = gemm_bf16_tn_group_ws(grp);
+  return full > top ? full : top;
 }
 extern "C" int avf_layers_dw(const avf_layer_cfg* cfgs, int n_layers, const void* const* descs, void* workspace,
                              size_t workspace_bytes, void* stream) {
diff --git a/multi-modal-multi-label-facial-action-unit-detection-with-transformer_amd/csrc/layernorm.hip b/multi-modal-multi-label-facial-action-unit-detection-with-transformer_amd/csrc/layernorm.hip
--- a/multi-modal-multi-label-facial-action-unit-detection-with-transformer_amd/csrc/layernorm.hip
+++ b/multi-modal-multi-label-facial-action-unit-detection-with-transformer_amd/csrc/layernorm.hip
@@ -522,10 +522,33 @@
     out[i] = (lds[i] + lds[3 * D + i]) + (lds[6 * D + i] + lds[9 * D + i]);
 }
 
-template <int NV8, int RU, bool DROP = false, bool TOK = false>
+struct LnResStream {
+  const bf16* __restrict__ p;
+  typedef uint4 Raw;
+  __device__ __forceinline__ Raw fetch(int64_t row, int D, int c, bool ok) const {
+    return (ok && p) ? *reinterpret_cast<const uint4*>(p + row * D + c) : make_uint4(0u, 0u, 0u, 0u);
+  }
+  __device__ __forceinline__ void unpack(const Raw& r, float (&e)[8]) const { unpack8(r, e); }
+};
+struct LnResClip {
+  const float* __restrict__ dp;
+  float inv;
+  int T;
+  struct Raw { float4 a, b; };
+  __device__ __forceinline__ Raw fetch(int64_t row, int D, int c, bool ok) const {
+    if (!ok) return Raw{make_float4(0.f, 0.f, 0.f, 0.f), make_float4(0.f, 0.f, 0.f, 0.f)};
+    const float* q = dp + (row / T) * D + c;
+    return Raw{*reinterpret_cast<const float4*>(q), *reinterpret_cast<const float4*>(q + 4)};
+  }
+  __device__ __forceinline__ void unpack(const Raw& r, float (&e)[8]) const {
+    const float o[8] = {r.a.x * inv, r.a.y * inv, r.a.z * inv, r.a.w * inv, r.b.x * inv, r.b.y * inv, r.b.z * inv, r.b.w * inv};
+    unpack8(pack8(o), e);
+  }
+};
+template <int NV8, int RU, bool DROP = false, bool TOK = false, typename Res = LnResStream>
 __global__ __launch_bounds__(256) void ln_bwd_row8_kernel(const bf16* __restrict__ dy, const bf16* __restrict__ x,
                                                           const float* __restrict__ gamma, const float* __restrict__ mean,
-                                                          const float* __restrict__ rstd, const bf16* __restrict__ dres,
+                                                          const float* __restrict__ rstd, const Res res,
                                                           bf16* __restrict__ dx_lo, float* __restrict__ partial, int64_t rows,
                                                           int D, int want_colsum, uint8_t* __restrict__ dxq = nullptr,
                                                           uint8_t* __restrict__ dxs = nullptr, float* __restrict__ dx = nullptr,
@@ -555,7 +578,8 @@
   const int64_t i0 = TOK ? (int64_t)(batch * 4 + wave) * RU : (int64_t)blockIdx.x * rpb + wave * (rpb / 4) + batch * RU;
   const int64_t iend = TOK ? rows / tokN : rows;
   const auto row_of = [&](int64_t i) { return TOK ? i * tokN + blockIdx.x : i; };
-  uint4 rd[RU][NV8], rx[RU][NV8], rr[RU][NV8];
+  uint4 rd[RU][NV8], rx[RU][NV8];
+  typename Res::Raw rr[RU][NV8];
   float mu[RU], rs[RU];
 #pragma unroll
   for (int r = 0; r < RU; ++r) {
@@ -569,7 +593,7 @@
       u32x4_nt xv = {0u, 0u, 0u, 0u};
       if (ok) xv = __builtin_nontemporal_load(reinterpret_cast<const u32x4_nt*>(x + row * D + c));
       rx[r][i] = make_uint4(xv[0], xv[1], xv[2], xv[3]);
-      rr[r][i] = (ok && dres) ? *reinterpret_cast<const uint4*>(dres + row * D + c) : make_uint4(0u, 0u, 0u, 0u);
+      rr[r][i] = res.fetch(row, D, c, ok);
     }
     mu[r] = mean[row];
     rs[r] = rstd[row];
@@ -609,7 +633,7 @@
       float d[8], v[8], e[8], o[8];
       unpack8(rd[r][i], d);
       unpack8(rx[r][i], v);
-      unpack8(rr[r][i], e);
+      res.unpack(rr[r][i], e);
 #pragma unroll
       for (int k = 0; k < 8; ++k) {
         const float xh = (v[k] - mu[r]) * rs[r];
@@ -726,9 +750,27 @@
     raised.mark();
   }
   launch_in_scope(ts, ln_bwd_row8_kernel<NV8, RU, DROP>, dim3((unsigned)ln_bwd_blocks(LN_BWD_ROW8, rows)), dim3(256), (uint32_t)lds, s,
-                  dy, x, gamma, mean, rstd, dres, dx_lo, partial, rows, D, wc, dxq, dxs, dx, drop, dx_m,
+                  dy, x, gamma, mean, rstd, LnResStream{dres}, dx_lo, partial, rows, D, wc, dxq, dxs, dx, drop, dx_m,
                   ln_bwd_rows_per_block(LN_BWD_ROW8, rows), 0, (float*)nullptr);
   return check_launch("ln_bwd_row8_kernel");
+}
+
+template <int NV8, int RU>
+static int launch_ln_bwd_row8_clip(const TimingScope* ts, hipStream_t s, const bf16* dy, const bf16* x, const float* gamma,
+                                   const float* mean, const float* rstd, const LnResClip& res, bf16* dx_lo, float* partial,
+                                   int64_t rows, int D, int wc) {
+  const size_t lds = (size_t)4 * 3 * D * sizeof(float);
+  static PerDeviceOnce raised;
+  if (lds > 64 * 1024 && raised.need()) {
+    hipError_t e = hipFuncSetAttribute((const void*)ln_bwd_row8_kernel<NV8, RU, false, false, LnResClip>,
+                                       hipFuncAttributeMaxDynamicSharedMemorySize, 4 * 3 * 512 * NV8 * (int)sizeof(float));
+    AVF_REQUIRE(e == hipSuccess, "layernorm_bwd_clipres: cannot raise dynamic LDS limit");
+    raised.mark();
+  }
+  launch_in_scope(ts, ln_bwd_row8_kernel<NV8, RU, false, false, LnResClip>, dim3((unsigned)ln_bwd_blocks(LN_BWD_ROW8, rows)), dim3(256),
+                  (uint32_t)lds, s, dy, x, gamma, mean, rstd, res, dx_lo, partial, rows, D, wc, (uint8_t*)nullptr, (uint8_t*)nullptr,
+                  (float*)nullptr, kNoDrop, (bf16*)nullptr, ln_bwd_rows_per_block(LN_BWD_ROW8, rows), 0, (float*)nullptr);
+  return check_launch("ln_bwd_row8_kernel(clip)");
 }
 
 template <int NV8, int RU>
@@ -745,7 +787,7 @@
   }
   const int nbatch = (int)ceil_div((int64_t)batch, 4 * RU);
   launch_in_scope(ts, ln_bwd_row8_kernel<NV8, RU, false, true>, dim3((unsigned)tokens), dim3(256), (uint32_t)lds, s, dy, x, gamma, mean,
-                  rstd, dres, (bf16*)nullptr, partial, (int64_t)batch * tokens, D, 1, (uint8_t*)nullptr, (uint8_t*)nullptr,
+                  rstd, LnResStream{dres}, (bf16*)nullptr, partial, (int64_t)batch * tokens, D, 1, (uint8_t*)nullptr, (uint8_t*)nullptr,
                   (float*)nullptr, kNoDrop, (bf16*)nullptr, nbatch * 4 * RU, tokens, dpos);
   return check_launch("ln_bwd_row8_kernel(tok)");
 }
@@ -765,6 +807,30 @@
                                                                              (const bf16*)dres, dpos, partial, batch, tokens, dim);
   }));
   const FoldJob job{partial, tokens, 3 * dim, dim, dgamma, dbeta, nullptr};
+  if (defer_fold) {
+    *defer_fold = job;
+    return 0;
+  }
+  return fold_job(job, s);
+}
+
+bool layernorm_bwd_clipres_ok(int dim) { return dim > 0 && dim % 8 == 0 && dim <= 1536 && ln_row8_on(); }
+int layernorm_bwd_clipres(const void* dy, const void* x, const float* gamma, const float* mean, const float* rstd, const float* dp,
+                          float inv, int tokens, void* dx_lo, float* dgamma, float* dbeta, float* dcolsum, void* ws, int64_t rows,
+                          int dim, hipStream_t s, FoldJob* defer_fold) {
+  AVF_REQUIRE(dy && x && gamma && mean && rstd && dp && dx_lo && ws && rows > 0 && tokens > 0 && rows % tokens == 0,
+              "layernorm_bwd_clipres: bad arguments");
+  AVF_REQUIRE(layernorm_bwd_clipres_ok(dim), "layernorm_bwd_clipres: needs dim %% 8 == 0 and dim <= 1536 (dim=%d)", dim);
+  AVF_REQUIRE((((uintptr_t)dy | (uintptr_t)x | (uintptr_t)dp | (uintptr_t)dx_lo | (uintptr_t)ws) & 15) == 0,
+              "layernorm_bwd_clipres: pointers must be 16-byte aligned");
+  TimingScope ts(KC_LAYERNORM, 0.0, (double)rows * dim * 6.0, s, true);
+  float* partial = (float*)ws;
+  const LnResClip res{dp, inv, tokens};
+  AVF_TRY(ln_nv8(dim, [&](auto nv8, auto ru) {
+    return launch_ln_bwd_row8_clip<decltype(nv8)::value, decltype(ru)::value>(&ts, s, (const bf16*)dy, (const bf16*)x, gamma, mean, rstd,
+                                                                              res, (bf16*)dx_lo, partial, rows, dim, dcolsum ? 1 : 0);
+  }));
+  const FoldJob job{partial, (int)ln_bwd_blocks(LN_BWD_ROW8, rows), 3 * dim, dim, dgamma, dbeta, dcolsum};
   if (defer_fold) {
     *defer_fold = job;
     return 0;
diff --git a/multi-modal-multi-label-facial-action-unit-detection-with-transformer_amd/csrc/stack_top.hip b/multi-modal-multi-label-facial-action-unit-detection-with-transformer_amd/csrc/stack_top.hip
--- /dev/null
+++ b/multi-modal-multi-label-facial-action-unit-detection-with-transformer_amd/csrc/stack_top.hip
@@ -0,0 +1,225 @@
+#include "common.hpp"
+
+namespace avf {
+
+struct TokSumJob {
+  const bf16* src;
+  float* out;
+  int W, blocks;
+};
+__global__ __launch_bounds__(256) void token_sum_kernel(TokSumJob j0, TokSumJob j1, int T) {
+  __shared__ float red[16][16][8];
+  const bool second = (int)blockIdx.x >= j0.blocks;
+  const bf16* src = second ? j1.src : j0.src;
+  float* out = second ? j1.out : j0.out;
+  const int W = second ? j1.W : j0.W;
+  const int bx = second ? (int)blockIdx.x - j0.blocks : (int)blockIdx.x;
+  const int cg = threadIdx.x & 15, tl = threadIdx.x >> 4;
+  const int c = (bx * 16 + cg) * 8;
+  const int64_t b = blockIdx.y;
+  float acc[8];
+#pragma unroll
+  for (int k = 0; k < 8; ++k) acc[k] = 0.f;
+  if (c < W) {
+    const bf16* base = src + b * T * W + c;
+    for (int t0 = tl; t0 < T; t0 += 128) {
+      uint4 v[8];
+#pragma unroll
+      for (int u = 0; u < 8; ++u) {
+        const int t = t0 + 16 * u;
+        v[u] = t < T ? *reinterpret_cast<const uint4*>(base + (int64_t)t * W) : make_uint4(0u, 0u, 0u, 0u);
+      }
+#pragma unroll
+      for (int u = 0; u < 8; ++u) {
+        float f[8];
+        unpack8(v[u], f);
+#pragma unroll
+        for (int k = 0; k < 8; ++k) acc[k] += f[k];
+      }
+    }
+  }
+#pragma unroll
+  for (int k = 0; k < 8; ++k) red[tl][cg][k] = acc[k];
+  __syncthreads();
+  if (tl < 8 && c < W) {
+    float r = red[0][cg][tl];
+#pragma unroll
+    for (int j = 1; j < 16; ++j) r += red[j][cg][tl];
+    out[b * W + c + tl] = r;
+  }
+}
+
+int token_sums_bf16(const void* src0, float* out0, int W0, const void* src1, float* out1, int W1, int batch, int tokens,
+                    hipStream_t s) {
+  AVF_REQUIRE(src0 && out0 && W0 > 0 && W0 % 8 == 0 && (!src1 || (out1 && W1 > 0 && W1 % 8 == 0)) && batch > 0 && batch <= 65535 &&
+                  tokens > 0, "token_sums: bad arguments (widths must be multiples of 8)");
+  AVF_REQUIRE((((uintptr_t)src0 | (uintptr_t)src1) & 15) == 0, "token_sums: sources must be 16-byte aligned");
+  const TokSumJob j0{(const bf16*)src0, out0, W0, (W0 + 127) / 128};
+  const TokSumJob j1{(const bf16*)src1, out1, src1 ? W1 : 0, src1 ? (W1 + 127) / 128 : 0};
+  TimingScope ts(KC_OTHER, 0.0, (double)batch * tokens * (W0 + j1.W) * 2.0, s, true);
+  launch_in_scope(&ts, token_sum_kernel, dim3((unsigned)(j0.blocks + j1.blocks), (unsigned)batch), dim3(256), 0, s, j0, j1, tokens);
+  return check_launch("token_sum_kernel");
+}
+
+constexpr int RL_ROWS = 16;
+__device__ __forceinline__ float bf16_round(float x) { return __uint_as_float(pack_bf16x2(x, 0.f) << 16); }
+__global__ __launch_bounds__(256) void rows_linear_kernel(const float* __restrict__ a, const bf16* __restrict__ W,
+                                                          const float* __restrict__ add, const float* __restrict__ bias,
+                                                          float* __restrict__ out, int B, int J, int K, float scale, float a_scale,
+                                                          int round_a) {
+  const int lane = threadIdx.x & 63, wave = threadIdx.x >> 6;
+  const int j = (int)blockIdx.x * 4 + wave;
+  const int b0 = (int)blockIdx.y * RL_ROWS;
+  if (j >= J) return;
+  float acc[RL_ROWS];
+#pragma unroll
+  for (int r = 0; r < RL_ROWS; ++r) acc[r] = 0.f;
+  for (int c = lane * 8; c < K; c += 512) {
+    float w[8];
+    unpack8(*reinterpret_cast<const uint4*>(W + (int64_t)j * K + c), w);
+    float av[RL_ROWS][8];
+#pragma unroll
+    for (int r = 0; r < RL_ROWS; ++r) {
+      const int b = b0 + r < B ? b0 + r : B - 1;
+      load8f(a + (int64_t)b * K + c, av[r]);
+    }
+#pragma unroll
+    for (int r = 0; r < RL_ROWS; ++r)
+#pragma unroll
+      for (int k = 0; k < 8; ++k) acc[r] = fmaf(round_a ? bf16_round(av[r][k] * a_scale) : av[r][k], w[k], acc[r]);
+  }
+  float mine = 0.f;
+#pragma unroll
+  for (int r = 0; r < RL_ROWS; ++r) {
+    const float sum = wave_sum(acc[r]);
+    if (lane == r) mine = sum;
+  }
+  const int b = b0 + lane;
+  if (lane < RL_ROWS && b < B) {
+    float v = mine;
+    if (add) v += add[(int64_t)b * J + j];
+    v *= scale;
+    if (bias) v += bias[j];
+    out[(int64_t)b * J + j] = v;
+  }
+}
+
+int rows_linear_bf16w(const float* a, const void* W, const float* add, const float* bias, float* out, int B, int J, int K,
+                      float scale, hipStream_t s, float a_scale, bool round_a) {
+  AVF_REQUIRE(a && W && out && B > 0 && J > 0 && K > 0 && K % 8 == 0, "rows_linear: bad arguments (K must be a multiple of 8)");
+  AVF_REQUIRE((((uintptr_t)a | (uintptr_t)W) & 15) == 0, "rows_linear: operands must be 16-byte aligned");
+  AVF_REQUIRE(ceil_div(B, RL_ROWS) <= 65535, "rows_linear: too many rows");
+  TimingScope ts(KC_OTHER, 2.0 * B * J * K, (double)J * K * 2.0 + (double)B * (K + J) * 4.0, s, true);
+  launch_in_scope(&ts, rows_linear_kernel, dim3((unsigned)ceil_div(J, 4), (unsigned)ceil_div(B, RL_ROWS)), dim3(256), 0, s, a,
+                  (const bf16*)W, add, bias, out, B, J, K, scale, a_scale, round_a ? 1 : 0);
+  return check_launch("rows_linear_kernel");
+}
+
+constexpr int TOP_DGELU_ROWS = 32;
+__global__ __launch_bounds__(256) void top_dgelu_kernel(const float* __restrict__ r, const bf16* __restrict__ u,
+                                                        bf16* __restrict__ du, float* __restrict__ partial, int64_t rows, int T,
+                                                        int M) {
+  __shared__ float red[4][512];
+  const int lane = threadIdx.x & 63, wave = threadIdx.x >> 6;
+  const int c = (int)blockIdx.x * 512 + lane * 8;
+  const bool ok = c < M;
+  const int64_t row0 = (int64_t)blockIdx.y * TOP_DGELU_ROWS + wave;
+  constexpr int NR = TOP_DGELU_ROWS / 4;
+  uint4 raw[NR];
+#pragma unroll
+  for (int i = 0; i < NR; ++i) {
+    const int64_t row = row0 + 4 * i;
+    raw[i] = (ok && row < rows) ? *reinterpret_cast<const uint4*>(u + row * M + c) : make_uint4(0u, 0u, 0u, 0u);
+  }
+  float acc[8], rv[8];
+#pragma unroll
+  for (int k = 0; k < 8; ++k) acc[k] = rv[k] = 0.f;
+  int64_t cur = -1;
+#pragma unroll
+  for (int i = 0; i < NR; ++i) {
+    const int64_t row = row0 + 4 * i;
+    if (!ok || row >= rows) continue;
+    const int64_t b = row / T;
+    if (b != cur) {
+      load8f(r + b * M + c, rv);
+      cur = b;
+    }
+    float uu[8], o[8];
+    unpack8(raw[i], uu);
+#pragma unroll
+    for (int k = 0; k < 8; ++k) {
+      o[k] = rv[k] * dgelu_tanh_fast(uu[k]);
+      acc[k] += o[k];
+    }
+    *reinterpret_cast<uint4*>(du + row * M + c) = pack8(o);
+  }
+#pragma unroll
+  for (int k = 0; k < 8; ++k) red[wave][lane * 8 + k] = acc[k];
+  __syncthreads();
+  for (int i = threadIdx.x; i < 512; i += 256) {
+    const int col = (int)blockIdx.x * 512 + i;
+    if (col < M) partial[(int64_t)blockIdx.y * M + col] = (red[0][i] + red[1][i]) + (red[2][i] + red[3][i]);
+  }
+}
+
+size_t top_dgelu_ws(int64_t rows, int M) { return (size_t)ceil_div(rows, TOP_DGELU_ROWS) * M * sizeof(float); }
+
+int top_dgelu(const float* r, const void* u, void* du, void* ws, int64_t rows, int tokens, int M, float* db1, FoldJob* fold,
+              hipStream_t s) {
+  AVF_REQUIRE(r && u && du && ws && fold && rows > 0 && tokens > 0 && M > 0 && M % 8 == 0, "top_dgelu: bad arguments");
+  AVF_REQUIRE((((uintptr_t)r | (uintptr_t)u | (uintptr_t)du | (uintptr_t)ws) & 15) == 0, "top_dgelu: pointers must be 16-byte aligned");
+  const int64_t nb = ceil_div(rows, TOP_DGELU_ROWS);
+  AVF_REQUIRE(nb <= 65535, "top_dgelu: too many rows");
+  TimingScope ts(KC_OTHER, 0.0, (double)rows * M * 4.0, s, true);
+  launch_in_scope(&ts, top_dgelu_kernel, dim3((unsigned)ceil_div(M, 512), (unsigned)nb), dim3(256), 0, s, r, (const bf16*)u, (bf16*)du,
+                  (float*)ws, rows, tokens, M);
+  AVF_TRY(check_launch("top_dgelu_kernel"));
+  *fold = FoldJob{(const float*)ws, (int)nb, M, M, db1, nullptr, nullptr};
+  return 0;
+}
+
+__global__ __launch_bounds__(256) void top_dw2_kernel(const float* __restrict__ dp, const float* __restrict__ gsum,
+                                                      float* __restrict__ dW2, float* __restrict__ db2, int B, int D, int M,
+                                                      float inv) {
+  const int k = ((int)blockIdx.x * 256 + (int)threadIdx.x) * 4;
+  const int j0 = (int)blockIdx.y * 2;
+  if (k >= M) return;
+  float4 acc[2];
+  acc[0] = acc[1] = make_float4(0.f, 0.f, 0.f, 0.f);
+  float2 ds = make_float2(0.f, 0.f);
+  for (int b = 0; b < B; b += 8) {
+    float4 g[8];
+    float2 dv[8];
+#pragma unroll
+    for (int u = 0; u < 8; ++u) {
+      const int bb = b + u < B ? b + u : B - 1;
+      g[u] = *reinterpret_cast<const float4*>(gsum + (int64_t)bb * M + k);
+      dv[u] = *reinterpret_cast<const float2*>(dp + (int64_t)bb * D + j0);
+      if (b + u >= B) dv[u] = make_float2(0.f, 0.f);
+    }
+#pragma unroll
+    for (int u = 0; u < 8; ++u) {
+      const float d[2] = {bf16_round(dv[u].x * inv), bf16_round(dv[u].y * inv)};
+#pragma unroll
+      for (int q = 0; q < 2; ++q) {
+        acc[q].x = fmaf(d[q], g[u].x, acc[q].x); acc[q].y = fmaf(d[q], g[u].y, acc[q].y);
+        acc[q].z = fmaf(d[q], g[u].z, acc[q].z); acc[q].w = fmaf(d[q], g[u].w, acc[q].w);
+      }
+      if (b + u < B) { ds.x += dv[u].x; ds.y += dv[u].y; }
+    }
+  }
+#pragma unroll
+  for (int q = 0; q < 2; ++q) *reinterpret_cast<float4*>(dW2 + (int64_t)(j0 + q) * M + k) = acc[q];
+  if (k == 0) *reinterpret_cast<float2*>(db2 + j0) = ds;
+}
+
+int top_dw2(const float* dp, const float* gsum, float* dW2, float* db2, int B, int D, int M, float inv, hipStream_t s) {
+  AVF_REQUIRE(dp && gsum && dW2 && db2 && B > 0 && D > 0 && D % 2 == 0 && D / 2 <= 65535 && M > 0 && M % 4 == 0, "top_dw2: bad arguments");
+  AVF_REQUIRE((((uintptr_t)dp | (uintptr_t)gsum | (uintptr_t)dW2 | (uintptr_t)db2) & 15) == 0, "top_dw2: pointers must be 16-byte aligned");
+  TimingScope ts(KC_OTHER, 2.0 * B * D * M, (double)D * M * 4.0, s, true);
+  launch_in_scope(&ts, top_dw2_kernel, dim3((unsigned)ceil_div(M, 1024), (unsigned)(D / 2)), dim3(256), 0, s, dp, gsum, dW2, db2, B, D, M,
+                  inv);
+  return check_launch("top_dw2_kernel");
+}
+
+}
diff --git a/multi-modal-multi-label-facial-action-unit-detection-with-transformer_amd/ops.py b/multi-modal-multi-label-facial-action-unit-detection-with-transformer_amd/ops.py
--- a/multi-modal-multi-label-facial-action-unit-detection-with-transformer_amd/ops.py
+++ b/multi-modal-multi-label-facial-action-unit-detection-with-transformer_amd/ops.py
@@ -1017,6 +1017,69 @@
     return dy, lo, cs
 
 
+def top_pooled(g: torch.Tensor, x_mid: torch.Tensor, w2: torch.Tensor, b2: torch.Tensor):
+    _need_cuda(g, x_mid, w2, b2)
+    assert g.dtype == x_mid.dtype == w2.dtype == torch.bfloat16 and all(t.is_contiguous() for t in (g, x_mid, w2, b2))
+    B, T, M = g.shape
+    D = x_mid.shape[2]
+    assert x_mid.shape[:2] == (B, T) and tuple(w2.shape) == (D, M)
+    pooled = torch.empty((B, D), dtype=torch.float32, device=g.device)
+    gsum = torch.empty((B, M), dtype=torch.float32, device=g.device)
+    xsum = torch.empty((B, D), dtype=torch.float32, device=g.device)
+    _lib.check(_lib.load().avf_top_pooled(_ptr(g), _ptr(x_mid), _ptr(w2), _ptr(b2), _ptr(pooled), _ptr(gsum), _ptr(xsum), B, T, D, M,
+                                          _stream()), "top_pooled")
+    return pooled, gsum, xsum
+
+
+def top_dgelu(d_pooled: torch.Tensor, w2t: torch.Tensor, u: torch.Tensor, du: Optional[torch.Tensor] = None):
+    _need_cuda(d_pooled, w2t, u, du)
+    assert u.dtype == w2t.dtype == torch.bfloat16 and d_pooled.dtype == torch.float32
+    assert all(t.is_contiguous() for t in (d_pooled, w2t, u))
+    B, T, M = u.shape
+    D = d_pooled.shape[1]
+    assert d_pooled.shape[0] == B and tuple(w2t.shape) == (M, D)
+    lib = _lib.load()
+    r = torch.empty((B, M), dtype=torch.float32, device=u.device)
+    if du is None:
+        du = torch.empty_like(u)
+    db1 = torch.empty(M, dtype=torch.float32, device=u.device)
+    ws = _bytes(lib.avf_top_dgelu_workspace_bytes(B * T, M), u.device)
+    _lib.check(lib.avf_top_dgelu(_ptr(d_pooled), _ptr(w2t), _ptr(u), _ptr(r), _ptr(du), _ptr(db1), _ptr(ws), B, T, D, M, _stream()),
+               "top_dgelu")
+    return r, du, db1
+
+
+def top_dw2(d_pooled: torch.Tensor, gsum: torch.Tensor, tokens: int):
+    _need_cuda(d_pooled, gsum)
+    assert d_pooled.dtype == gsum.dtype == torch.float32 and d_pooled.is_contiguous() and gsum.is_contiguous()
+    B, D = d_pooled.shape
+    M = gsum.shape[1]
+    dw2 = torch.empty((D, M), dtype=torch.float32, device=gsum.device)
+    db2 = torch.empty(D, dtype=torch.float32, device=gsum.device)
+    _lib.check(_lib.load().avf_top_dw2(_ptr(d_pooled), _ptr(gsum), _ptr(dw2), _ptr(db2), B, int(tokens), D, M, _stream()), "top_dw2")
+    return dw2, db2
+
+
+def layernorm_bwd_clipres(dy, x, weight, mean, rstd, d_pooled: torch.Tensor, dx: Optional[torch.Tensor] = None):
+    _need_cuda(dy, x, weight, mean, rstd, d_pooled, dx)
+    lib = _lib.load()
+    assert all(t.is_contiguous() and t.shape == x.shape and t.dtype == torch.bfloat16 for t in (dy, x))
+    rows, D = x.shape
+    B = d_pooled.shape[0]
+    tokens = rows // B
+    assert tokens * B == rows and tuple(d_pooled.shape) == (B, D) and d_pooled.dtype == torch.float32 and d_pooled.is_contiguous()
+    dev = x.device
+    if dx is None:
+        dx = torch.empty_like(x)
+    dg = torch.empty(D, dtype=torch.float32, device=dev)
+    db = torch.empty(D, dtype=torch.float32, device=dev)
+    cs = torch.empty(D, dtype=torch.float32, device=dev)
+    ws = _bytes(lib.avf_layernorm_bwd_workspace_bytes(rows, D), dev)
+    _lib.check(lib.avf_layernorm_bwd_clipres(_ptr(dy), _ptr(x), _ptr(weight), _ptr(mean), _ptr(rstd), _ptr(d_pooled), tokens, _ptr(dx),
+                                             _ptr(dg), _ptr(db), _ptr(cs), _ptr(ws), rows, D, _stream()), "layernorm_bwd_clipres")
+    return dx, dg, db, cs
+
+
 def conv_pack_weight(w: torch.Tensor, gamma: torch.Tensor, beta: torch.Tensor, running_mean: torch.Tensor,
                      running_var: torch.Tensor, eps: float = 1e-5):
     _need_cuda(w, gamma, beta, running_mean, running_var)
diff --git a/multi-modal-multi-label-facial-action-unit-detection-with-transformer_amd/transformer.py b/multi-modal-multi-label-facial-action-unit-detection-with-transformer_amd/transformer.py
--- a/multi-modal-multi-label-facial-action-unit-detection-with-transformer_amd/transformer.py
+++ b/multi-modal-multi-label-facial-action-unit-detection-with-transformer_amd/transformer.py
@@ -92,6 +92,11 @@
 def _stack_ends_on(part: str) -> bool:
     v = os.environ.get("AVF_STACK_ENDS", "1").strip()
     return v != "0" and (v in ("", "1") or part in v.split(","))
+
+
+def _stack_top_on(part: str) -> bool:
+    v = os.environ.get("AVF_STACK_TOP", "all").strip()
+    return v != "0" and (v in ("", "all", "1") or part in v.split(","))
 
 
 class _StackFn(torch.autograd.Function):
@@ -147,6 +152,10 @@
         xs = [x0]
         saved = []
         shared = None
+        top_ok = bool(pool and L > 1 and mod._grad_hook is None and lib.avf_layer_top_ok(C.byref(cfgs[L - 1])))
+        top_fwd = top_ok and _stack_top_on("fwd")
+        ctx.top_ok = top_ok
+        ctx.gsum = pooled = None
         for l in range(L):
             pp = mod._param_struct(params, l)
             if need_grad:
@@ -154,6 +163,14 @@
             else:
                 shared = shared if shared is not None else _alloc_bytes(saved_bytes, dev)
                 sv = shared
+            if l == L - 1 and top_fwd:
+                pooled = torch.empty((B, D), dtype=torch.float32, device=dev)
+                ctx.gsum = torch.empty((B, mod.mlp_dim), dtype=torch.float32, device=dev)
+                _lib.check(lib.avf_layer_fwd_top(C.byref(cfgs[l]), C.byref(pp), _ptr(lowps[l]), _ptr(xs[-1]), _ptr(pooled),
+                                                 _ptr(ctx.gsum), _ptr(sv), _ptr(ws), stream), f"layer_fwd_top[{l}]")
+                saved.append(sv)
+                xs.append(None)
+                break
             x_out = torch.empty((B * N, D), dtype=torch.bfloat16 if rs16 else torch.float32, device=dev)
             if l == 0 and embed is not None:
                 _lib.check(lib.avf_layer_fwd_embed(C.byref(cfgs[0]), C.byref(pp), _ptr(lowps[0]), _ptr(embed[0]), _ptr(embed[1]),
@@ -174,6 +191,8 @@
         ctx.lowps = lowps
         ctx.pool = pool
         _check_canaries()
+        if pooled is not None:
+            return pooled
         if pool:
             pooled = torch.empty((B, D), dtype=torch.float32, device=dev)
             fn = lib.avf_token_mean_fwd_bf16 if rs16 else lib.avf_token_mean_fwd
@@ -211,7 +230,17 @@
         if (ctx.fused and ctx.grad_in[2] and not ctx.grad_in[0] and not ctx.grad_in[1] and cfg.grad_stream_bf16
                 and _stack_ends_on("pos") and lib.avf_layer_bwd_pos_ok(C.byref(cfg))):
             d_pos = torch.empty((N, D), dtype=torch.float32, device=dev)
-        if ctx.pool:
+        hook = mod._grad_hook
+        top_bwd = ctx.pool and ctx.top_ok and hook is None and _stack_top_on("bwd")
+        if top_bwd:
+            g = dy.contiguous().to(torch.float32)
+            gsum = ctx.gsum
+            if gsum is None:
+                gsum = torch.empty((B, mod.mlp_dim), dtype=torch.float32, device=dev)
+                _lib.check(lib.avf_layer_top_gsum(C.byref(cfgs[L - 1]), _ptr(ctx.saved_bufs[L - 1]), _ptr(gsum), stream),
+                           "layer_top_gsum")
+            dx = None if d_pos is not None else torch.empty((B * N, D), dtype=torch.float32, device=dev)
+        elif ctx.pool:
             g = dy.contiguous().to(torch.float32)
             have_lo = top_colsum = bf16 and cfg.dropout_p == 0.0
             dx = None if (have_lo and d_pos is not None) else torch.empty((B * N, D), dtype=torch.float32, device=dev)
@@ -221,7 +250,6 @@
                 dx = dx.clone()
         live = mod.flat_parameters()
         sizes = [p.numel() for p in ctx.params[:PARAMS_PER_LAYER]]
-        hook = mod._grad_hook
         groups = mod._dw_plan(lib, cfgs) if (bf16 and hook is None and L > 1) else [1] * L
         per_layer = sum(sizes)
         flat_all = torch.empty(L * per_layer, dtype=torch.float32, device=dev)
@@ -237,7 +265,7 @@
         base = flat_all.data_ptr()
         B2 = PARAMS_PER_LAYER - 1
         gs16 = bool(cfg.grad_stream_bf16)
-        if ctx.pool:
+        if ctx.pool and not top_bwd:
             _lib.check(lib.avf_token_mean_bwd(_ptr(g), None if (gs16 and have_lo) else _ptr(dx),
                                               _ptr(lo_a) if have_lo else None,
                                               _ptr(views[L - 1][B2]) if top_colsum else None, B, N, D, stream),
@@ -266,7 +294,10 @@
                 lead = (C.byref(cfgs[l]), C.byref(pp), _ptr(ctx.lowps[l]), _ptr(ctx.xs[l]),
                         _ptr(ctx.saved_bufs[l]), dx_out_p, _ptr(lo_a) if have_lo else None,
                         _ptr(views[l][B2]) if (l < L - 1 or top_colsum) else None)
-                if l == 0 and d_pos is not None:
+                if l == L - 1 and top_bwd:
+                    args = lead[:5] + (_ptr(g), _ptr(gsum), dx_in_p, _ptr(lo_b), _ptr(views[l - 1][B2]), C.byref(gp), _ptr(ws))
+                    fn, fn_dx, what = lib.avf_layer_bwd_top, lib.avf_layer_bwd_dx_top, "layer_bwd_top"
+                elif l == 0 and d_pos is not None:
                     args = lead + (_ptr(d_pos), C.byref(gp), _ptr(ws))
                     fn, fn_dx, what = lib.avf_layer_bwd_pos, lib.avf_layer_bwd_dx_pos, "layer_bwd_pos"
                 else:
```
